# acoustid/acoustid-index

Measured on AMD Instinct MI355X. Metric: queries/sec + p50 /_search latency, 100M-fp index, 1k-hash queries, higher is better.
Workload: dtype u32

## Files before the change

acoustid-index_amd/csrc/fpx_api.hip:

```cpp
#include <cstdarg>
#include <cstdio>
#include <cstring>
#include <hip/hip_runtime.h>
#include <dlfcn.h>
#include <execinfo.h>
#include <atomic>

#include <algorithm>
#include <new>

#include "fpx_internal.h"

namespace fpx {

static thread_local char g_err[512] = "";

void set_error(const char* fmt, ...)
{
    va_list ap;
    va_start(ap, fmt);
    vsnprintf(g_err, sizeof g_err, fmt, ap);
    va_end(ap);
}

// ... 80 lines not shown
        static const size_t hi = [] { const char* v = getenv("FPX_POISON_MAX"); return v ? (size_t)strtoull(v, nullptr, 0) : ~(size_t)0; }();
        static const uint64_t olo = [] { const char* v = getenv("FPX_POISON_ORD_LO"); return v ? (uint64_t)strtoull(v, nullptr, 0) : (uint64_t)0; }();
        static const uint64_t ohi = [] { const char* v = getenv("FPX_POISON_ORD_HI"); return v ? (uint64_t)strtoull(v, nullptr, 0) : ~(uint64_t)0; }();
        static FILE* const log = [] { const char* v = getenv("FPX_ALLOC_LOG"); return v ? std::fopen(v, "w") : (FILE*)nullptr; }();
        static std::atomic<uint64_t> ordinal{0};
        const uint64_t ord = ordinal.fetch_add(1);
        if (log) {
            void* bt[6];
            const int nb = backtrace(bt, 6);
            Dl_info di{};
            std::fprintf(log, "%llu %zu", (unsigned long long)ord, bytes);
            for (int i = 1; i < nb; ++i)
                if (dladdr(bt[i], &di) && di.dli_fbase) std::fprintf(log, " %s+0x%zx", di.dli_fname ? std::strrchr(di.dli_fname, '/') ? std::strrchr(di.dli_fname, '/') + 1 : di.dli_fname : "?", (size_t)((char*)bt[i] - (char*)di.dli_fbase));
            std::fprintf(log, "\n");
            std::fflush(log);
        }
        if (bytes >= lo && bytes <= hi && ord >= olo && ord <= ohi) { (void)hipMemset(*p, 0xCD, bytes); (void)hipDeviceSynchronize(); }
    }
    return e;
}

thread_local DevArena* tl_arena = nullptr;
thread_local DevArena* tl_scratch = nullptr;
void* arena_take(size_t bytes) { return tl_arena ? tl_arena->take(bytes) : nullptr; }
void* scratch_take(size_t bytes) { return tl_scratch ? tl_scratch->take(bytes) : nullptr; }

hipError_t mem_info(size_t* free_b, size_t* total_b)
{
    const hipError_t e = hipMemGetInfo(free_b, total_b);
    int device = 0;
    if (e == hipSuccess && hipGetDevice(&device) == hipSuccess) *free_b += line_pool_bytes(device);
    return e;
}

Workspace* ws_acquire(Ctx* ctx)
{
    {
        std::lock_guard<std::mutex> g(ctx->mu);
        if (!ctx->free_ws.empty()) {
            Workspace* w = ctx->free_ws.back();
            ctx->free_ws.pop_back();
            return w;
        }
    }
    Workspace* w = new (std::nothrow) Workspace();
    if (!w) { set_error("out of host memory"); return nullptr; }
    bool ok = hipStreamCreateWithFlags(&w->stream, hipStreamNonBlocking) == hipSuccess &&
              hipEventCreate(&w->ev_begin) == hipSuccess && hipEventCreate(&w->ev_probe0) == hipSuccess &&
              hipEventCreate(&w->ev_probe1) == hipSuccess && hipEventCreate(&w->ev_probe2) == hipSuccess &&
              hipEventCreate(&w->ev_end) == hipSuccess &&
              dmalloc(&w->d_counters, COUNTERS_BYTES) == hipSuccess &&
              hipHostMalloc(reinterpret_cast<void**>(&w->h_counters), COUNTERS_BYTES, hipHostMallocMapped) == hipSuccess &&
              hipHostMalloc(reinterpret_cast<void**>(&w->h_cancel), 64, hipHostMallocMapped) == hipSuccess &&
              hipHostGetDevicePointer(reinterpret_cast<void**>(const_cast<uint32_t**>(&w->d_cancel)), w->h_cancel, 0) == hipSuccess;
    if (ok) *w->h_cancel = 0u;
    if (!ok) { set_error("workspace creation failed: %s", hipGetErrorString(hipGetLastError())); ws_destroy(w); return nullptr; }
    ctx->live_ws++;
    return w;
}

constexpr size_t MAX_POOLED = 8;

void ws_release(Ctx* ctx, Workspace* ws)
{
    {
        std::lock_guard<std::mutex> g(ctx->mu);
        if (ctx->free_ws.size() < MAX_POOLED) { ctx->free_ws.push_back(ws); return; }
    }
    ctx->live_ws--;
    ws_destroy(ws);
}

void ws_destroy(Workspace* w)
{
    if (!w) return;
    if (w->stream) (void)hipStreamSynchronize(w->stream);
    if (w->d_qstats) (void)hipFree(w->d_qstats);
    if (w->d_kocnt) (void)hipFree(w->d_kocnt);
    if (w->d_refs) (void)hipFree(w->d_refs);
    if (w->d_cells) (void)hipFree(w->d_cells);
    if (w->h_cells) (void)hipHostFree(w->h_cells);
    void* bufs[] = {w->d_hashes, w->d_offsets, w->d_opts, w->d_keys[0], w->d_keys[1], w->d_hits[0], w->d_hits[1],
                    w->d_cands[0], w->d_cands[1], w->d_temp, w->d_counters, w->d_out, w->d_out_n, w->d_def_list, w->d_def_count, w->d_qrange, w->d_qcand,
                    w->d_binq, w->d_qcursor, w->d_parts, w->d_parts_n};
    for (void* b : bufs) if (b) (void)hipFree(b);
    if (w->h_counters) (void)hipHostFree(w->h_counters);
    if (w->h_stage) (void)hipHostFree(w->h_stage);
    if (w->h_cancel) (void)hipHostFree(w->h_cancel);
    if (w->h_bins) (void)hipHostFree(w->h_bins);
    if (w->h_out) (void)hipHostFree(w->h_out);
    if (w->h_def_count) (void)hipHostFree(w->h_def_count);
    if (w->ev_begin) (void)hipEventDestroy(w->ev_begin);
    if (w->ev_probe0) (void)hipEventDestroy(w->ev_probe0);
    if (w->ev_probe1) (void)hipEventDestroy(w->ev_probe1);
    if (w->ev_probe2) (void)hipEventDestroy(w->ev_probe2);
    if (w->ev_end) (void)hipEventDestroy(w->ev_end);
    if (w->copy_stream) { (void)hipStreamSynchronize(w->copy_stream); (void)hipStreamDestroy(w->copy_stream); }
    for (hipEvent_t& e : w->ev_chunk) if (e) (void)hipEventDestroy(e);
    if (w->stream) (void)hipStreamDestroy(w->stream);
    delete w;
}

static void set_docs(Segment* s, const uint32_t* ids, const uint8_t* alive, uint32_t n)
{
    std::vector<uint64_t> v(n);
    for (uint32_t i = 0; i < n; ++i) v[i] = ((uint64_t)ids[i] << 32) | ((uint64_t)i << 1) | (alive ? (alive[i] ? 1u : 0u) : 1u);
    std::sort(v.begin(), v.end());
    s->doc_ids.clear(); s->doc_alive.clear();
    for (uint32_t i = 0; i < n; ++i) {
        const uint32_t id = (uint32_t)(v[i] >> 32);
        if (i + 1 < n && (uint32_t)(v[i + 1] >> 32) == id) continue;
        s->doc_ids.push_back(id);
        s->doc_alive.push_back((uint8_t)(v[i] & 1u));
    }
}

bool VmBuf::supported(int device)
{
    static std::atomic<int> known[64];
    std::atomic<int>& k = known[(unsigned)device & 63u];
    int v = k.load(std::memory_order_relaxed);
    if (v == 0) {
        const char* e = getenv("FPX_VM");
        int attr = 0;
        v = (e && e[0] == '0') ? 1 : (hipDeviceGetAttribute(&attr, hipDeviceAttributeVirtualMemoryManagementSupported, device) == hipSuccess && attr) ? 2 : 1;
        (void)hipGetLastError();
        k.store(v, std::memory_order_relaxed);
    }
    return v == 2;
}
int VmBuf::reserve(int dev, size_t bytes, size_t piece_bytes)
{
    device = dev; piece = piece_bytes;
    const size_t n = (bytes + piece - 1) / piece;
    void* p = nullptr;
    if (hipMemAddressReserve(&p, n * piece, 0, nullptr, 0) != hipSuccess) { (void)hipGetLastError(); return FPX_E_NOMEM; }
    va = static_cast<uint8_t*>(p); reserved = n * piece;
    handles.assign(n, hipMemGenericAllocationHandle_t{}); mapped.assign(n, 0);
    return FPX_OK;
}
int VmBuf::map_range(size_t lo, size_t hi)
{
    hipMemAllocationProp prop = {};
    prop.type = hipMemAllocationTypePinned; prop.location.type = hipMemLocationTypeDevice; prop.location.id = device;
    hipMemAccessDesc acc = {};
    acc.location = prop.location; acc.flags = hipMemAccessFlagsProtReadWrite;
    for (size_t i = lo / piece; i < handles.size() && i * piece < hi; ++i) {
        if (mapped[i]) continue;
        hipError_t e = hipMemCreate(&handles[i], piece, &prop, 0);
        if (e == hipErrorOutOfMemory) { (void)hipGetLastError(); if (line_pool_flush(device) != 0) e = hipMemCreate(&handles[i], piece, &prop, 0); }
        if (e != hipSuccess) { (void)hipGetLastError(); return FPX_E_NOMEM; }
        if (hipMemMap(va + i * piece, piece, 0, handles[i], 0) != hipSuccess || hipMemSetAccess(va + i * piece, piece, &acc, 1) != hipSuccess) {
            (void)hipGetLastError(); (void)hipMemRelease(handles[i]); return FPX_E_DEVICE;
        }
        mapped[i] = 1;
    }
    return FPX_OK;
}
void VmBuf::release_below(size_t upto)
{
    for (size_t i = 0; i < handles.size() && (i + 1) * piece <= upto; ++i) {
        if (!mapped[i]) continue;
        (void)hipMemUnmap(va + i * piece, piece);
        (void)hipMemRelease(handles[i]);
        mapped[i] = 0;
    }
}
// ... 55 lines not shown
                              unsigned long long* total)
{
    const uint32_t b = blockIdx.x * blockDim.x + threadIdx.x;
    unsigned long long n = 0;
    if (b < num_blocks) {
        const uint8_t* p = blocks + (size_t)b * block_size;
        n = (unsigned long long)p[4] | ((unsigned long long)p[5] << 8);
    }
    for (int d = 32; d > 0; d >>= 1) n += __shfl_down(n, d);
    if ((threadIdx.x & 63) == 0 && n) atomicAdd(total, n);
}

__global__ void k_build_cont(const uint8_t* __restrict__ blocks, uint32_t block_size, uint32_t num_blocks,
                             const uint32_t* __restrict__ block_index, uint32_t* __restrict__ cont)
{
    const uint32_t b = blockIdx.x * blockDim.x + threadIdx.x;
    bool bit = false;
    if (b + 1u < num_blocks)
        bit = *reinterpret_cast<const uint32_t*>(blocks + (size_t)(b + 1u) * block_size) == block_index[b];
    const unsigned long long m = __ballot((int)bit);
    if ((threadIdx.x & 63u) == 0u && b < num_blocks + 64u) {
        cont[(b >> 5)] = (uint32_t)m;
        cont[(b >> 5) + 1u] = (uint32_t)(m >> 32);
    }
}

int finish_file_segment(Segment* s)
{
    if (s->num_blocks == 0) { s->num_buckets = 1; s->bucket_shift = 32; }
    int rc = build_bucket_table(s, 0);
    if (rc) return rc;
    {
        const size_t words = ((size_t)s->num_blocks + 63) / 64 * 2 + 2;
        FPX_HIP(dmalloc(&s->d_cont, words * sizeof(uint32_t)));
        FPX_HIP(hipMemset(s->d_cont, 0, words * sizeof(uint32_t)));
        s->device_bytes += words * sizeof(uint32_t);
        if (s->num_blocks)
            hipLaunchKernelGGL(k_build_cont, dim3((s->num_blocks + 255) / 256), dim3(256), 0, 0,
                               s->d_blocks, s->block_size, s->num_blocks, s->d_block_index, s->d_cont);
    }
    unsigned long long* d_total = nullptr;
    FPX_HIP(dmalloc(&d_total, 8));
    FPX_HIP(hipMemset(d_total, 0, 8));
    if (s->num_blocks)
        hipLaunchKernelGGL(k_count_items, dim3((s->num_blocks + 255) / 256), dim3(256), 0, 0,
                           s->d_blocks, s->block_size, s->num_blocks, d_total);
    unsigned long long total = 0;
    FPX_HIP(hipMemcpy(&total, d_total, 8, hipMemcpyDeviceToHost));
    (void)hipFree(d_total);
    s->num_items = total;
    bool cand = false;
    if ((rc = direct_candidate(s, &cand))) return rc;
    s->candidate = cand;
    if (cand) return FPX_OK;
    if ((rc = build_presence(s))) return rc;
    return decode_small_segment(s);
}

struct OptInfo { const char* name; const char* env; int64_t dflt; int64_t min_set; bool env_once; };
static const OptInfo OPT_TABLE[OPT_COUNT] = {
                 {"direct", "FPX_DIRECT", 1, 0, false},
       {"direct_min_items", "FPX_DIRECT_MIN_ITEMS", 1ll << 20, 0, false},
               {"fuse_min", "FPX_FUSE_MIN", 2, 0, true},
           {"group_packed", "FPX_GROUP_PACKED", -1, -1, false},
     {"presence_min_items", "FPX_PRESENCE_MIN_ITEMS", 1ll << 20, 0, false},
              {"lean_head", "FPX_LEAN_HEAD", 0, 0, true},
                   {"fast", "FPX_FAST", 1, 0, true},
                 {"binned", "FPX_BINNED", 1, 0, true},
                  {"rec32", "FPX_REC32", 1, 0, true},
         {"local_sort_max", "FPX_LOCAL_SORT_MAX", 1ll << 20, 0, true},
        {"order_min_pairs", "FPX_ORDER_MIN_PAIRS", 1ll << 17, 0, true},
               {"lean_min", "FPX_LEAN_MIN", 1ll << 16, 0, true},
        {"sharded_workers", "FPX_SHARDED_WORKERS", 3, 1, true},
               {"hot_refs", "FPX_HOT_REFS", -1, -1, true},
               {"query_wg", "FPX_QUERY_WG", 1, 0, false},
                {"side_wg", "FPX_SIDE_WG", 0, 0, false},
                 {"hot_wg", "FPX_HOT_WG", 0, 0, false},
               {"words_wg", "FPX_WORDS_WG", 0, 0, false},
                 {"low_wg", "FPX_LOW_WG", 0, 0, false},
              {"groups_wg", "FPX_GROUPS_WG", 0, 0, false},
               {"shard_wg", "FPX_SHARD_WG", 0, 0, false},
             {"shard_pack", "FPX_SHARD_PACK", 0, 0, false},
              {"filt_coop", "FPX_FILT_COOP", 0, 0, false},
};

int64_t ctx_opt(const Ctx* c, CtxOpt o)
{
    const OptInfo& t = OPT_TABLE[o];
    if (c) {
        const int64_t v = c->opts[o].load(std::memory_order_relaxed);
        if (v != OPT_UNSET) return v;
    }
    if (t.env_once) {
        static std::atomic<int64_t> cache[OPT_COUNT];
        static std::atomic<uint32_t> have{0};
        if (!(have.load(std::memory_order_acquire) & (1u << o))) {
            const char* e = getenv(t.env);
            cache[o].store(e ? (int64_t)strtoll(e, nullptr, 0) : t.dflt, std::memory_order_relaxed);
            have.fetch_or(1u << o, std::memory_order_release);
        }
        return cache[o].load(std::memory_order_relaxed);
    }
    const char* e = getenv(t.env);
    return e ? (int64_t)strtoll(e, nullptr, 0) : t.dflt;
}

uint32_t ctx_fuse_min(const Ctx* c) { return (uint32_t)std::max<int64_t>(0, ctx_opt(c, OPT_FUSE_MIN)); }

static int settle_in_blocks(Segment* s)
{
    if (s->d_proberec || s->d_small_items || s->settled) return FPX_OK;
    s->settled = true;
    int rc = build_presence(s);
    if (rc) return rc;
    return decode_small_segment(s);
}

int resolve_candidates(Ctx* c, const std::vector<Segment*>& segs)
{
    const uint32_t fuse_min = ctx_fuse_min(c);
    std::vector<Segment*> lone;
    for (const Segment* s : segs)
        if (s->blocks_lost) { set_error("a segment lost its blocks in a group build that failed: it must be created again"); return FPX_E_INVAL; }
    for (Segment* s : segs)
        if (s->kind == 0 && s->ctx == c && !s->home && ((s->candidate && s->d_blocks && !s->settled) || s->direct)) lone.push_back(s);
    std::vector<bool> done(lone.size(), false);
    for (size_t i = 0; fuse_min != 0 && i < lone.size(); ++i) {
        if (done[i]) continue;
        std::vector<Segment*> batch;
        std::vector<size_t> idx;
        for (size_t j = i; j < lone.size() && batch.size() < FUSE_MAX; ++j) {
            if (done[j]) continue;
            const Segment* a = lone[i]; const Segment* b = lone[j];
            if (a->own_flags != b->own_flags || ((a->own_flags & 1u) && a->own_lo != b->own_lo) || ((a->own_flags & 2u) && a->own_hi != b->own_hi)) continue;
            if (a->block_size != b->block_size) continue;
            batch.push_back(lone[j]); idx.push_back(j);
        }
        for (size_t j : idx) done[j] = true;
        if (batch.size() < fuse_min) continue;
        std::shared_ptr<Group> g;
        const int grc = group_segments(c, batch.data(), (uint32_t)batch.size(), &g);
        if (grc == FPX_E_DEVICE || grc == FPX_E_INVAL) return grc;
        if (grc != FPX_OK)
            for (const Segment* b : batch) if (b->blocks_lost) { set_error("a group build failed after its members' blocks had begun to go back: the segments must be created again"); return FPX_E_DEVICE; }
    }
    for (Segment* s : lone) {
        if (s->home || s->direct) continue;
        int rc = build_direct(s);
        if (rc) return rc;
        if (!s->direct && (rc = settle_in_blocks(s))) return rc;
    }
    return FPX_OK;
}

int regroup_segments(Ctx* c, const std::vector<Segment*>& segs, uint32_t* regrouped)
{
    *regrouped = 0;
    if (ctx_fuse_min(c) == 0) return FPX_OK;
    std::vector<Segment*> m;
    for (Segment* s : segs) {
        if (!s || s->kind != 0 || s->ctx != c || s->own_flags) continue;
        if (std::find(m.begin(), m.end(), s) != m.end()) continue;
        if (!m.empty() && s->block_size != m[0]->block_size) continue;
        if (s->home || s->direct || (s->candidate && s->d_blocks && !s->settled)) m.push_back(s);
        if (m.size() == FUSE_MAX) break;
    }
// ... 56 lines not shown
}

using namespace fpx;

extern "C" {

int fpx_version(void) { return 2; }

int fpx_host_alloc(size_t bytes, void** out)
{
    if (!out) { set_error("null out"); return FPX_E_INVAL; }
    *out = nullptr;
    const hipError_t e = hipHostMalloc(out, bytes ? bytes : 1, hipHostMallocDefault);
    if (e != hipSuccess) { *out = nullptr; return hip_fail(e, "hipHostMalloc"); }
    return FPX_OK;
}

void fpx_host_free(void* p) { if (p) (void)hipHostFree(p); }

const char* fpx_last_error(void) { return g_err; }

const char* fpx_strerror(int status)
{
    switch (status) {
        case FPX_OK: return "ok";
        case FPX_E_NOMEM: return "out of memory";
        case FPX_E_TIMEOUT: return "search timeout";
        case FPX_E_DEVICE: return "device error";
        case FPX_E_INVAL: return "invalid argument";
        case FPX_E_NODEVICE: return "no HIP device";
        case FPX_E_AGAIN: return "buffer too small, retry";
        default: return "unknown";
    }
}

int fpx_ctx_create(int device, fpx_ctx** out)
{
    if (!out) { set_error("null out"); return FPX_E_INVAL; }
    *out = nullptr;
    int n = 0;
    hipError_t e = hipGetDeviceCount(&n);
    if (e != hipSuccess || n <= 0) {
        set_error("no HIP device visible (%s): libfpx has no CPU fallback", e == hipSuccess ? "count=0" : hipGetErrorString(e));
        return FPX_E_NODEVICE;
    }
    if (device < 0) { if (hipGetDevice(&device) != hipSuccess) device = 0; }
    if (device >= n) { set_error("device %d out of range (%d visible)", device, n); return FPX_E_INVAL; }
    FPX_HIP(hipSetDevice(device));
    hipDeviceProp_t prop;
    FPX_HIP(hipGetDeviceProperties(&prop, device));
    if (std::strncmp(prop.gcnArchName, "gfx950", 6) != 0) {
        set_error("device %d is %s; libfpx is built for gfx950 only", device, prop.gcnArchName);
        return FPX_E_NODEVICE;
    }
    Ctx* c = new (std::nothrow) Ctx();
    if (!c) return FPX_E_NOMEM;
    c->device = device;
    *out = reinterpret_cast<fpx_ctx*>(c);
    return FPX_OK;
}

int fpx_ctx_device(const fpx_ctx* ctx) { return ctx ? reinterpret_cast<const Ctx*>(ctx)->device : -1; }

static int opt_by_name(const char* name)
{
    if (!name) return -1;
    for (int o = 0; o < OPT_COUNT; ++o) if (!std::strcmp(name, OPT_TABLE[o].name)) return o;
    return -1;
}

int fpx_ctx_set_option(fpx_ctx* ctx, const char* name, int64_t value)
{
    Ctx* c = reinterpret_cast<Ctx*>(ctx);
    const int o = opt_by_name(name);
    if (!c || o < 0) {
        std::string all;
        for (int i = 0; i < OPT_COUNT; ++i) { if (i) all += ", "; all += OPT_TABLE[i].name; }
        set_error("fpx_ctx_set_option: unknown option (%s)", all.c_str());
        return FPX_E_INVAL;
    }
    if (o == OPT_SHARD_WG && value > 2) { set_error("fpx_ctx_set_option: shard_wg is 0, 1 or 2"); return FPX_E_INVAL; }
    if (o == OPT_SHARD_PACK && value > 1) { set_error("fpx_ctx_set_option: shard_pack is 0 or 1"); return FPX_E_INVAL; }
    if (o == OPT_FILT_COOP && value > 1) { set_error("fpx_ctx_set_option: filt_coop is 0 or 1"); return FPX_E_INVAL; }
    c->opts[o].store(value < OPT_TABLE[o].min_set ? OPT_UNSET : value, std::memory_order_relaxed);
    return FPX_OK;
}

int fpx_ctx_get_option(const fpx_ctx* ctx, const char* name, int64_t* value)
{
    const Ctx* c = reinterpret_cast<const Ctx*>(ctx);
    const int o = opt_by_name(name);
    if (!c || o < 0 || !value) { set_error("fpx_ctx_get_option: unknown option"); return FPX_E_INVAL; }
    *value = ctx_opt(c, (CtxOpt)o);
    return FPX_OK;
}

uint64_t fpx_ctx_trim(fpx_ctx* ctx)
{
    Ctx* c = reinterpret_cast<Ctx*>(ctx);
    if (!c) return 0;
    (void)hipSetDevice(c->device);
    return line_pool_flush(c->device);
}

int fpx_ctx_scan_histograms(const fpx_ctx* ctx, fpx_scan_histograms* out, uint64_t* unbucketed)
{
    const Ctx* c = reinterpret_cast<const Ctx*>(ctx);
    if (!c || !out) { set_error("null argument"); return FPX_E_INVAL; }
    uint64_t h[HIST_SLOTS + 1];
    for (uint32_t i = 0; i <= HIST_SLOTS; ++i) h[i] = c->scan_hist[i].load(std::memory_order_relaxed);
    std::memset(out, 0, sizeof *out);
    uint64_t docs_rest = 0, blocks_rest = 0;
    for (uint32_t i = 0; i < 9; ++i) { out->docs_bucket[i + 1] = h[i]; docs_rest += h[i]; }
    for (uint32_t i = 0; i < 3; ++i) { out->blocks_bucket[i + 1] = h[9 + i]; blocks_rest += h[9 + i]; }
    out->count = h[HIST_COUNT]; out->docs_sum = h[HIST_DOCS]; out->blocks_sum = h[HIST_BLOCKS];
    out->docs_bucket[0] = out->count - std::min(out->count, docs_rest);
    out->blocks_bucket[0] = out->count - std::min(out->count, blocks_rest);
    if (unbucketed) *unbucketed = h[HIST_SLOTS];
    return FPX_OK;
}

void fpx_ctx_destroy(fpx_ctx* ctx_)
{
    Ctx* c = reinterpret_cast<Ctx*>(ctx_);
    if (!c) return;
    (void)hipSetDevice(c->device);
    for (Workspace* w : c->free_ws) ws_destroy(w);
    delete c;
}

static int create_file_impl(fpx_ctx* ctx_, const uint8_t* blocks, size_t blocks_len, uint32_t block_size,
                            const uint32_t* block_index, uint32_t num_blocks,
                            uint32_t own_flags, uint32_t own_lo, uint32_t own_hi,
                            uint32_t min_doc_id, uint32_t max_doc_id, uint64_t commit_id,
                            const uint32_t* doc_ids, const uint8_t* doc_alive, uint32_t num_docs,
                            fpx_segment** out)
{
    Ctx* c = reinterpret_cast<Ctx*>(ctx_);
    if (!c || !out || (!blocks && blocks_len) || (!block_index && num_blocks) || (!doc_ids && num_docs)) {
        set_error("null argument"); return FPX_E_INVAL;
    }
    *out = nullptr;
    if (block_size < 64 || block_size > 4096) { set_error("block_size %u outside [64,4096] (src/filefmt.zig:236)", block_size); return FPX_E_INVAL; }
    if (blocks_len < (size_t)num_blocks * block_size) { set_error("blocks_len shorter than num_blocks * block_size"); return FPX_E_INVAL; }
    FPX_HIP(hipSetDevice(c->device));
    Segment* s = new (std::nothrow) Segment();
    if (!s) return FPX_E_NOMEM;
    s->ctx = c; s->kind = 0; s->commit_id = commit_id; s->min_doc_id = min_doc_id; s->max_doc_id = max_doc_id;
    s->block_size = block_size; s->num_blocks = num_blocks;
    s->own_flags = own_flags; s->own_lo = own_lo; s->own_hi = own_hi;
    set_docs(s, doc_ids, doc_alive, num_docs);
    s->blocks_len = ((size_t)num_blocks + 1) * block_size;
    const size_t alloc = s->blocks_len + 16;
    hipError_t e = blocks_alloc(s, alloc);
    if (e == hipSuccess) e = dmalloc(&s->d_block_index, ((size_t)num_blocks + 1) * sizeof(uint32_t));
    if (e != hipSuccess) { segment_free(s); return hip_fail(e, "hipMalloc(segment)"); }
    s->device_bytes = alloc + ((size_t)num_blocks + 1) * sizeof(uint32_t);
    const size_t copy = (size_t)num_blocks * block_size;
    if ((e = hipMemset(s->d_blocks + copy, 0, alloc - copy)) != hipSuccess ||
        (copy && (e = hipMemcpy(s->d_blocks, blocks, copy, hipMemcpyHostToDevice)) != hipSuccess) ||
        (num_blocks && (e = hipMemcpy(s->d_block_index, block_index, (size_t)num_blocks * sizeof(uint32_t), hipMemcpyHostToDevice)) != hipSuccess)) {
        segment_free(s); return hip_fail(e, "segment upload");
    }
    int rc = finish_file_segment(s);
    if (rc) { segment_free(s); return rc; }
    FPX_HIP(hipDeviceSynchronize());
// ... 822 lines not shown
```

acoustid-index_amd/csrc/fpx_internal.h:

```cpp
#pragma once
#include <hip/hip_runtime.h>
#include <stddef.h>
#include <stdint.h>

#include <atomic>
#include <memory>
#include <mutex>
#include <string>
#include <vector>

#include "../../include/fpx.h"

namespace fpx {

struct SegDesc {
    const uint8_t*  blocks;
    const uint32_t* block_index;
    const uint32_t* bucket;
    const uint32_t* dead;
    const uint32_t* cont;
    const uint32_t* dead_bits;
    const uint32_t* proberec;
    const uint2*    blockrec;
    const uint64_t* items;
// ... 177 lines not shown
    uint32_t* d_small_aux = nullptr; uint32_t small_shift = 0, small_cshift = 0;
    const char* why = "";
    bool candidate = false;
    bool settled = false;
    bool direct = false;
    std::shared_ptr<DirectStore> dstore;
    uint32_t* d_drec = nullptr; uint32_t* d_primary = nullptr; uint32_t* d_extras = nullptr;
    std::shared_ptr<Group> home; uint32_t col = 0;
    uint64_t num_distinct = 0, num_positions = 0, extras_words = 0;
    uint32_t first_hash = 0, last_hash = 0, extras_shift = 0;
    uint32_t own_flags = 0, own_lo = 0, own_hi = 0;
    std::mutex dead_mu; std::shared_ptr<DeadSet> last_dead;
    uint64_t num_items = 0;
    uint64_t* d_items = nullptr;
    uint64_t device_bytes = 0;
};

struct Snapshot {
    std::atomic<int> refs{1};
    Ctx* ctx = nullptr;
    std::vector<Segment*> segs;
    std::vector<SegDesc> h_file;
    std::vector<MemDesc> h_mem;
    SegDesc* d_file = nullptr; uint32_t n_file = 0;
    SegDesc* d_lean = nullptr; uint32_t n_lean = 0;
    uint32_t n_lean2 = 0;
    SegDesc* d_gen = nullptr; uint32_t n_gen = 0; bool gen_all_512 = true;
    SegDesc* d_small = nullptr; uint32_t n_small = 0;
    std::vector<SegDesc> h_direct;
    SegDesc* d_direct = nullptr; uint32_t n_direct = 0;
    std::vector<std::shared_ptr<Group>> groups;
    std::vector<GroupDesc> h_group; uint32_t n_group = 0;
    uint32_t max_doc_declared = 0;
    uint32_t rec32_refused = 0;
    uint32_t qs_skip = 0;
    std::vector<std::shared_ptr<DirectStore>> solo_stores;
    SegDesc* d_solo = nullptr; uint32_t n_solo = 0;
    Snapshot* part[2] = {nullptr, nullptr};
    uint32_t max_small_blocks = 0;
    MemDesc* d_mem = nullptr; uint32_t n_mem = 0;
    uint64_t* d_memtab = nullptr; uint32_t* d_membucket = nullptr; uint64_t n_memtab = 0;
    uint32_t* d_membits = nullptr;
    uint64_t mem_items = 0;
    std::vector<std::shared_ptr<DeadSet>> dead_sets;
    std::vector<std::shared_ptr<DeadSet>> direct_dead;
    std::vector<uint32_t> direct_max_doc;
    std::shared_ptr<DeadUnion> dead_union;
    uint32_t max_block_size = 0;
    bool all_512 = true;
};

constexpr size_t COUNTERS_BYTES = (CTR_COUNT + 1) * sizeof(unsigned long long) + 1024 * sizeof(fpx_result);

constexpr size_t STAGE_BYTES = 64 * 1024;

struct Workspace {
    hipStream_t stream = nullptr;
    hipEvent_t ev_begin = nullptr, ev_probe0 = nullptr, ev_probe1 = nullptr, ev_probe2 = nullptr, ev_end = nullptr;
    uint32_t* d_hashes = nullptr; size_t cap_hashes = 0;
    uint64_t* d_offsets = nullptr; size_t cap_queries = 0;
    uint32_t* d_opts = nullptr;
    uint64_t* d_keys[2] = {nullptr, nullptr}; size_t cap_keys = 0;
    uint64_t* d_hits[2] = {nullptr, nullptr}; size_t cap_hits = 0;
    uint64_t* d_cands[2] = {nullptr, nullptr}; size_t cap_cands = 0;
    void* d_temp = nullptr; size_t cap_temp = 0;
    uint64_t* d_qrange = nullptr; size_t cap_qrange = 0;
    uint64_t* d_qcand = nullptr; size_t cap_qcand = 0;
    unsigned long long* d_counters = nullptr;
    uint32_t* d_def_list = nullptr; size_t cap_def = 0;
    unsigned int* d_def_count = nullptr; unsigned int* h_def_count = nullptr; size_t cap_def_segs = 0;
    fpx_result* d_out = nullptr; uint32_t* d_out_n = nullptr; size_t cap_out = 0;
    uint32_t* d_binq = nullptr; unsigned long long* d_qcursor = nullptr; size_t cap_binq = 0; uint32_t* h_bins = nullptr;
    uint8_t* h_out = nullptr; size_t cap_h_out = 0;
    uint4* d_refs = nullptr; size_t cap_refs = 0;
    uint32_t* d_kocnt = nullptr; size_t cap_kocnt = 0;
    unsigned long long* d_qstats = nullptr; size_t cap_qstats = 0;
    uint32_t* d_cells = nullptr; uint32_t* h_cells = nullptr; size_t cap_cells = 0;
    static constexpr uint32_t UP_CHUNKS = 4;
    hipStream_t copy_stream = nullptr; hipEvent_t ev_chunk[UP_CHUNKS] = {nullptr, nullptr, nullptr, nullptr};
    std::vector<uint32_t> h_opts;
    uint32_t hint_def = 0;
    uint64_t hint_misc = 0;
    uint64_t hint_P = 0, hint_H = 0;
    uint32_t fast_penalty = 0;
    fpx_result* d_parts = nullptr; size_t cap_parts = 0;
    uint32_t* d_parts_n = nullptr; size_t cap_parts_n = 0;
    uint64_t batch_hist[HIST_SLOTS + 1] = {};
    unsigned long long* h_counters = nullptr;
    uint8_t* h_stage = nullptr; uint8_t* d_stage = nullptr;
    unsigned long long* d_ret = nullptr;
    uint32_t* h_cancel = nullptr; const uint32_t* d_cancel = nullptr;
};

struct QueryBatch {
    Ctx* ctx = nullptr;
    uint32_t B = 0;
    uint32_t* d_hashes = nullptr;
    uint64_t* d_offsets = nullptr;
    uint32_t* d_opts = nullptr;
    std::vector<uint64_t> offsets;
    std::vector<fpx_opts> opts;
};

enum CtxOpt : int {
    OPT_DIRECT, OPT_DIRECT_MIN_ITEMS, OPT_FUSE_MIN, OPT_GROUP_PACKED,
    OPT_PRESENCE_MIN_ITEMS, OPT_LEAN_HEAD,
    OPT_FAST, OPT_BINNED, OPT_REC32,
    OPT_LOCAL_SORT_MAX, OPT_ORDER_MIN_PAIRS, OPT_LEAN_MIN,
    OPT_SHARDED_WORKERS,
    OPT_HOT_REFS,
    OPT_QUERY_WG,
    OPT_SIDE_WG,
    OPT_HOT_WG,
    OPT_WORDS_WG,
    OPT_LOW_WG,
    OPT_GROUPS_WG,
    OPT_SHARD_WG,
    OPT_SHARD_PACK,
    OPT_FILT_COOP,
    OPT_COUNT
};
constexpr int64_t OPT_UNSET = -2;

struct Ctx {
    int device = 0;
    std::atomic<int64_t> opts[OPT_COUNT];
    Ctx() { for (auto& o : opts) o.store(OPT_UNSET, std::memory_order_relaxed); for (auto& h : scan_hist) h.store(0, std::memory_order_relaxed); }
    std::mutex mu;
    std::mutex group_mu;
    std::vector<Workspace*> free_ws;
    std::atomic<int> live_ws{0};
    std::atomic<int> qs_running{0};
    std::atomic<uint64_t> scan_hist[HIST_SLOTS + 1];
};
void ctx_hist_add(Ctx* c, const uint64_t* slots, uint64_t unbucketed);

int64_t ctx_opt(const Ctx* c, CtxOpt o);
bool ctx_direct_enabled(const Ctx* c);
uint64_t ctx_direct_min_items(const Ctx* c);
uint32_t ctx_fuse_min(const Ctx* c);
int ctx_group_packed(const Ctx* c);
void set_error(const char* fmt, ...);
int  hip_fail(hipError_t e, const char* what);
void*  line_pool_take(int device, size_t bytes, size_t max_bytes, size_t* got);
void   line_pool_put(int device, void* p, size_t bytes);
size_t line_pool_flush(int device);
size_t line_pool_bytes(int device);
hipError_t dmalloc_raw(void** p, size_t bytes);
template <class T> inline hipError_t dmalloc(T** p, size_t bytes) { return dmalloc_raw(reinterpret_cast<void**>(p), bytes); }
hipError_t mem_info(size_t* free_b, size_t* total_b);
struct DevArena {
    uint8_t* base = nullptr;
    size_t cap = 0, used = 0, missed = 0;
    const char* name = "arena";
    std::vector<std::pair<size_t, size_t>> guards;
    static size_t guard_bytes();
    void check_guards();
    ~DevArena() { check_guards(); if (base) (void)hipFree(base); }
    void* take(size_t bytes)
    {
        const size_t g = guard_bytes();
        const size_t body = (bytes + 255u) & ~(size_t)255u, need = body + g;
        if (used + need > cap) { missed += need; return nullptr; }
        void* p = base + used;
        if (g) { (void)hipMemset(base + used + body, 0xA5, g); guards.emplace_back(used + body, bytes); }
        used += need;
        return p;
    }
    void rewind()
    {
        check_guards();
        if (missed) {
            const size_t want = (used + missed) * 5 / 4 + ((size_t)1 << 20);
            if (base) (void)hipFree(base);
            base = nullptr; cap = 0;
            if (dmalloc(&base, want) == hipSuccess) cap = want; else { (void)hipGetLastError(); base = nullptr; }
        }
        used = 0; missed = 0;
    }
};
extern thread_local DevArena* tl_arena;
extern thread_local DevArena* tl_scratch;
void* arena_take(size_t bytes);
void* scratch_take(size_t bytes);
#define FPX_HIP(expr)                                              \
    do {                                                           \
        hipError_t _e = (expr);                                    \
        if (_e != hipSuccess) return ::fpx::hip_fail(_e, #expr);   \
    } while (0)

Workspace* ws_acquire(Ctx* ctx);
void ws_release(Ctx* ctx, Workspace* ws);
void ws_destroy(Workspace* ws);

size_t sort_u64_temp_bytes(size_t n, unsigned begin_bit, unsigned end_bit);
hipError_t sort_u64(void* temp, size_t temp_bytes, uint64_t* buf0, uint64_t* buf1, size_t n,
                    unsigned begin_bit, unsigned end_bit, hipStream_t stream, int* result_in);

size_t select_u64_temp_bytes(size_t n);
hipError_t select_u64(void* temp, size_t temp_bytes, const uint64_t* in, const uint8_t* flags, uint64_t* out,
                      unsigned long long* d_count, size_t n, hipStream_t stream);

// ... 65 lines not shown
```

acoustid-index_amd/csrc/fpx_qsearch.hpp:

```cpp
#pragma once
#include <hip/hip_runtime.h>

#include <cstddef>

#include "fpx_internal.h"

namespace fpx {

#ifndef FPX_QS_WG
#define FPX_QS_WG 256
#endif
#ifndef FPX_QS_WAVES
#define FPX_QS_WAVES 4
#endif
#ifndef FPX_QS_REC_CAP
#define FPX_QS_REC_CAP 8192
#endif
#ifndef FPX_QS_FLOG2
#define FPX_QS_FLOG2 11
#endif
constexpr uint32_t QS_WG = FPX_QS_WG;
constexpr uint32_t QS_REC_CAP = FPX_QS_REC_CAP;
constexpr uint32_t QS_FLOG2 = FPX_QS_FLOG2;
constexpr uint32_t QS_TLOG2 = 8;
constexpr uint32_t QS_MAX_HASHES = QS_REC_CAP >= 8192u ? 4096u : 2048u;
constexpr uint32_t QS_MAX_ROUNDS = 32;
#ifndef FPX_QS_WORDS
#define FPX_QS_WORDS 12
#endif
#ifndef FPX_QS_CH
#define FPX_QS_CH 2
#endif
constexpr uint32_t QS_WORDS = FPX_QS_WORDS;
constexpr uint32_t QS_CH = FPX_QS_CH;
constexpr uint32_t QS_TASKS = (((size_t)2u << QS_FLOG2) + ((size_t)8u << QS_TLOG2)) / 8u;
constexpr uint32_t QS_TASK_WORDS = 8;
constexpr uint32_t QS_TASKS_FILT = QS_TASKS * 8u / 12u;
static_assert(QS_MAX_HASHES * 2u <= QS_REC_CAP, "the dedup set lives where the records will");
static_assert((QS_MAX_HASHES + QS_WG - 1u) / QS_WG <= QS_MAX_ROUNDS, "rounds per query");
static_assert(QS_WORDS % 4 == 0 && QS_WORDS <= 16, "the words are fetched in 16-byte pieces; a lane's masks of them are 16 bits");
#ifndef FPX_QS_DYN
#define FPX_QS_DYN 1
#endif
#ifndef FPX_QS_STAGGER
#define FPX_QS_STAGGER 1
#endif
constexpr uint32_t QS_STAGGER = FPX_QS_STAGGER;
#ifndef FPX_QS_WGS_PER_CU
#define FPX_QS_WGS_PER_CU 4
#endif
constexpr uint32_t QS_WGS_PER_CU = FPX_QS_WGS_PER_CU;
constexpr size_t QS_LDS_BYTES = ((size_t)QS_REC_CAP + 4u) * 4u + ((size_t)2u << QS_FLOG2) + ((size_t)8u << QS_TLOG2) + (size_t)SB_CAND * 8u;

struct QSearchArgs {
    const uint32_t* hashes_base; const uint64_t* offsets;
    const uint32_t* opts;
    uint32_t q_begin, q_end, sb;
    union { uint64_t* cands; uint64_t* bins; };
    union { uint64_t cand_cap; uint64_t bin_cap; };
    uint64_t* qcand;
    union { uint32_t* qcand_n; uint32_t* bin_fill; };
    unsigned long long* counters;
    unsigned long long* stat_sets;
    unsigned long long* qstats;
    const uint32_t* cancel;
    const uint64_t* mem_tab; const uint32_t* mem_bucket; const uint32_t* mem_bits;
    unsigned int* next_q;
    uint32_t stagger;
    union { unsigned long long* redo; const uint32_t* dead_union; };
    union { uint32_t redo_cap; uint32_t bin_rec32; uint32_t dead_union_last; };
};

struct QSKernargs { QSearchArgs a; GroupArgs ga; };
static_assert(sizeof(QSearchArgs) == 160 && offsetof(QSearchArgs, cands) == 40 && offsetof(QSearchArgs, qcand_n) == 64 && offsetof(QSearchArgs, next_q) == 128 &&
              offsetof(QSearchArgs, redo) == 144 && offsetof(QSearchArgs, redo_cap) == 152, "QSearchArgs' layout is the kernels' argument segment: a member is renamed or shared, never moved");
typedef const __attribute__((address_space(4))) QSKernargs* qs_kargs_t;
__device__ __forceinline__ qs_kargs_t qs_cold_args()
{
    qs_kargs_t p = (qs_kargs_t)__builtin_amdgcn_kernarg_segment_ptr();
    asm volatile("" : "+s"(p));
    return p;
}

#define FPX_QS_OCC __attribute__((amdgpu_waves_per_eu(FPX_QS_WAVES)))
#define FPX_LDS __attribute__((address_space(3)))
typedef uint32_t u32x3_t __attribute__((ext_vector_type(3)));
__device__ __forceinline__ uint3 gload_u3(const uint32_t* p)
{
    const u32x3_t v = *(const FPX_GLOBAL u32x3_t*)p;
    return make_uint3(v.x, v.y, v.z);
}
__device__ __forceinline__ uint32_t qs_cell(uint32_t doc) { return (doc ^ (doc >> QS_FLOG2)) & ((1u << QS_FLOG2) - 1u); }
__device__ __forceinline__ unsigned long long qs_task_list(const uint32_t* p, uint32_t chunk)
{
    return ((unsigned long long)p >> 2) | ((unsigned long long)chunk << 57) | (1ull << 63);
}
__device__ __forceinline__ unsigned long long qs_task_words(const uint32_t* p, uint32_t cnt, uint32_t second, uint32_t chunk)
{
    return ((unsigned long long)p >> 2) | ((unsigned long long)(cnt - 1u) << 46) | ((unsigned long long)(second & 0xFFu) << 49) | ((unsigned long long)chunk << 57);
}
__device__ __forceinline__ const uint32_t* qs_task_ptr(unsigned long long e) { return reinterpret_cast<const uint32_t*>((e & ((1ull << 46) - 1ull)) << 2); }
__device__ __forceinline__ uint32_t qs_word_cols(uint32_t pm, uint32_t dm, uint32_t j0, uint32_t cnt)
{
    uint32_t cols = 0, rest = pm, i = 0, w = 0;
    while (rest != 0u && w < j0 + cnt) {
        const uint32_t s = (uint32_t)__builtin_ctz(rest), span = 1u + ((dm >> i) & 1u);
        for (uint32_t t = 0; t < span; ++t, ++w) if (w >= j0 && w < j0 + cnt) cols |= s << (4u * (w - j0));
        ++i; rest &= rest - 1u;
    }
    return cols;
}

template <uint32_t K> __device__ __forceinline__ uint32_t qs_group_bcast(uint32_t v)
{
    return (uint32_t)__builtin_amdgcn_ds_swizzle((int)v, (int)((K << 5) | 0x18u));
}
template <uint32_t K> __device__ __forceinline__ uint32_t qs_from_sub0(uint32_t v)
{
    if constexpr (K == 0u) return v;
    else return (uint32_t)__builtin_amdgcn_update_dpp(0, (int)v, 0x110 | (int)K, 0xF, 0xF, true);
}
template <uint32_t K> __device__ __forceinline__ uint32_t qs_from_sub7(uint32_t v)
{
    if constexpr (K == 7u) return v;
    else return (uint32_t)__builtin_amdgcn_update_dpp(0, (int)v, 0x100 | (int)(7u - K), 0xF, 0xF, true);
}
template <uint32_t K> struct qs_idx { static constexpr uint32_t value = K; };
template <uint32_t K = 0, class F> __device__ __forceinline__ void qs_for8(F&& f)
{
    if constexpr (K < 8u) { f(qs_idx<K>{}); qs_for8<K + 1u>(f); }
}

#ifdef FPX_QS_PROF
#define QS_MARK(i) do { if (tid == 0) { const unsigned long long t_ = clock64(); atomicAdd(&qs_cold_args()->a.counters[CTR_HIST + (i)], t_ - t_prev); t_prev = t_; } } while (0)
#define QS_SUB0() do { if (tid == 0) t_sub = clock64(); } while (0)
#define QS_SUB(i) do { if (tid == 0) { const unsigned long long t_ = clock64(); atomicAdd(&qs_cold_args()->a.counters[CTR_HIST + (i)], t_ - t_sub); t_sub = t_; } } while (0)
#define QS_ARRIVED2(x, y) asm volatile("" :: "v"(x), "v"(y))
#define QS_ARRIVED4(x) asm volatile("" :: "v"((x)[0]), "v"((x)[1]), "v"((x)[2]), "v"((x)[3]))
#else
#define QS_MARK(i) do { } while (0)
#define QS_SUB0() do { } while (0)
#define QS_SUB(i) do { } while (0)
#define QS_ARRIVED2(x, y) do { } while (0)
#define QS_ARRIVED4(x) do { } while (0)
#endif
constexpr uint32_t QS_MAX_CLASSES = 32;
constexpr uint32_t QS_LIST_AHEAD = 8;
__device__ __forceinline__ uint32_t qs_class(uint32_t rec) { return mix32(rec) >> 27; }
static_assert(QS_MAX_CLASSES == 32u, "qs_class gives five bits");
constexpr uint32_t QS_LOW_CHUNK = 8;
constexpr uint32_t QS_SHARE_BQ = 3;
constexpr uint32_t QS_SHARE_STRIDE = 32;
constexpr uint32_t QS_PACK_MAX = 4u * QS_WG;

enum : uint32_t { QS_F_CLS = 1u, QS_F_LOW = 2u, QS_F_NEXT = 4u, QS_F_SHARE = 8u, QS_F_PACK = 16u, QS_F_COOP = 32u };
template <int NS_, bool QS_, bool MEM_, bool FILT_, uint32_t FORM = 0u>
struct qs_variant {
    static constexpr int NS = NS_;
    static constexpr bool QS = QS_, MEM = MEM_, FILT = FILT_;
    static constexpr bool CLS = (FORM & QS_F_CLS) != 0u, LOW = (FORM & QS_F_LOW) != 0u, NEXT = (FORM & QS_F_NEXT) != 0u;
    static constexpr bool SHARE = (FORM & QS_F_SHARE) != 0u, PACK = (FORM & QS_F_PACK) != 0u, COOP = (FORM & QS_F_COOP) != 0u;
    static_assert(NS == 8 || NS == 16, "columns of a line");
    static_assert(!COOP || (FILT && !CLS && !LOW && !NEXT && !SHARE), "the filtered walk eight lanes to a line: k_search_filt only");
    static_assert(!SHARE || (!QS && !CLS && !LOW && !NEXT), "a window's walk for the bin protocol: no per-query statistics, no doc classes, no sorted tail, one group");
    static_assert(!PACK || SHARE, "packed probes: a window's walk only (without a window nearly every hash is a probe)");
    static_assert(!PACK || 2u * QS_PACK_MAX <= QS_REC_CAP, "the packed list and its memory-table bits live at the record array's bottom");
    static_assert(!NEXT || (!CLS && !MEM), "a later group's walk: no doc classes, no memory table (they ride on the first group's launch)");
    static_assert(!(CLS && FILT), "doc classes: the unfiltered walk only");
    static_assert(!LOW || (!CLS && QS_WG == 256u && QS_REC_CAP >= 512u && (QS_REC_CAP & (QS_REC_CAP - 1u)) == 0u),
                  "low floors: no doc classes; the sorted tail's scans are written for 256 lanes and a power-of-two array");
};

template <class V>
__device__ __forceinline__ void qs_body(const QSearchArgs& a, const GroupArgs& ga)
{
    constexpr int NS = V::NS;
    constexpr bool QS = V::QS, MEM = V::MEM, FILT = V::FILT, CLS = V::CLS, LOW = V::LOW, NEXT = V::NEXT, SHARE = V::SHARE, PACK = V::PACK, COOP = V::COOP;
#ifdef FPX_QS_PROF
    unsigned long long t_prev = clock64(), t_sub = 0;
#endif
    constexpr uint32_t HVL = NS == 16 ? 2u : 3u;
    constexpr uint32_t T = 1u << QS_TLOG2, TMASK = T - 1u;
    extern __shared__ __align__(16) uint8_t qs_dyn[];
    uint32_t* const recs = reinterpret_cast<uint32_t*>(qs_dyn);
    uint32_t* const filter = recs + QS_REC_CAP + 4u;
    unsigned long long* const table = reinterpret_cast<unsigned long long*>(filter + (1u << (QS_FLOG2 - 1u)));
    unsigned long long* const tasks = reinterpret_cast<unsigned long long*>(filter);
    constexpr uint32_t TCAP = FILT ? QS_TASKS_FILT : QS_TASKS;
    uint32_t* const tcols = reinterpret_cast<uint32_t*>(tasks + QS_TASKS_FILT);
    uint64_t* const cbuf = reinterpret_cast<uint64_t*>(table + T);
    __shared__ uint32_t s_count, s_ntask, s_over_recs, s_seen_ones, s_cancel, s_claimed, s_full, s_ccnt, s_cshared, s_cbase_lo, s_cbase_hi;
    __shared__ unsigned long long wg_blocks, wg_docs, wg_probes, wg_reads;
    __shared__ uint32_t wg_h[HIST_SLOTS];
    __shared__ uint32_t s_first[FUSE_MAX], s_last[FUSE_MAX];
    __shared__ const uint32_t* s_ext[GROUP_CHUNKS];
    __shared__ uint32_t s_q2;
    __shared__ uint32_t s_dseg[FUSE_MAX];

    const uint32_t tid = threadIdx.x, lane = tid & 63u;
    const GroupDesc* g = &ga.g;
    uint32_t ent = a.q_begin + blockIdx.x;
    uint32_t q = ent, q_recs = 0u;
    uint32_t ncls = 1u;
    auto take_entry = [&]() {
        const unsigned long long e = qs_cold_args()->a.redo[ent];
        q = (uint32_t)__builtin_amdgcn_readfirstlane((int)(uint32_t)e); q_recs = (uint32_t)__builtin_amdgcn_readfirstlane((int)(uint32_t)(e >> 32));
        ncls = 1u;
        while ((unsigned long long)ncls * (QS_REC_CAP / 2u) < (unsigned long long)q_recs) ncls *= 2u;
    };
    if constexpr (CLS) take_entry();
    (void)q_recs;
    uint32_t qn = q + gridDim.x;
    uint32_t n, nn = 0u;
    uint64_t nq_lo = 0;
    const uint32_t* qh;
    if constexpr (CLS) {
        const uint64_t q_lo = a.offsets[q];
        n = (uint32_t)(a.offsets[q + 1] - q_lo);
        qh = a.hashes_base + q_lo;
        qn = 0xFFFFFFFFu;
    } else {
        const uint64_t q_lo = a.offsets[q];
        n = (uint32_t)(a.offsets[q + 1] - q_lo);
        qh = a.hashes_base + q_lo;
        if (qn < a.q_end) { nq_lo = a.offsets[qn]; nn = (uint32_t)(a.offsets[qn + 1] - nq_lo); }
    }
    {
        const qs_kargs_t ka = qs_cold_args();
        if (tid < FUSE_MAX) { s_first[tid] = ka->ga.g.first_hash[tid]; s_last[tid] = ka->ga.g.last_hash[tid]; }
        if (tid < GROUP_CHUNKS) s_ext[tid] = tid < ka->ga.g.nchunks ? ka->ga.g.ext_tab[tid] : nullptr;
        if (FILT && tid < FUSE_MAX) s_dseg[tid] = ka->ga.g.has_dead[tid] != 0u ? ka->ga.g.seg_index[tid] : 0xFFFFFFFFu;
    }
    const uint32_t gmin = (FILT || MEM) ? g->gmin : 0u;
    (void)gmin;
    uint32_t hq[2u * QS_CH];
    uint3 hd[QS_CH];
    auto line_of = [&](uint32_t h) -> const uint32_t* { return g->lines + (size_t)((h >> HVL) - g->line0) * GROUP_LINE_WORDS; };
    auto load_pair = [&](const uint32_t* qh_, uint32_t n_, uint32_t c, uint32_t& h0, uint32_t& h1) {
        uint32_t t = tid;
        if constexpr (COOP) asm volatile("" : "+v"(t));
        const uint32_t i = c * QS_CH * QS_WG + t;
        h0 = i < n_ ? gload_u32(qh_ + i) : 0u;
        h1 = i + QS_WG < n_ ? gload_u32(qh_ + i + QS_WG) : 0u;
    };
    auto issue_heads = [&](bool v0, bool v1) {
        hd[0] = gload_u3(v0 ? line_of(hq[0]) : g->lines);
        hd[1] = gload_u3(v1 ? line_of(hq[1]) : g->lines);
    };
    load_pair(qh, n, 0u, hq[0], hq[1]);
    load_pair(qh, n, 1u, hq[2], hq[3]);
    uint32_t c_host = 0u;
    unsigned long long c_dev = 0ull;
    auto ask_cancel = [&]() {
        const qs_kargs_t ka = qs_cold_args();
        const uint32_t* const cancel = ka->a.cancel;
        if (tid == 0u && cancel != nullptr) {
            if ((blockIdx.x & 63u) == 0u) c_host = __hip_atomic_load(cancel, __ATOMIC_RELAXED, __HIP_MEMORY_SCOPE_SYSTEM);
            c_dev = __hip_atomic_load(&ka->a.counters[CTR_CANCEL], __ATOMIC_RELAXED, __HIP_MEMORY_SCOPE_AGENT);
        }
    };
    ask_cancel();
  if (const uint32_t stagger = qs_cold_args()->a.stagger; !CLS && stagger != 0u && a.q_end - a.q_begin >= 4u * gridDim.x)
      for (uint32_t i = 0; i < ((blockIdx.x >> 8) & 3u) * stagger; ++i) __builtin_amdgcn_s_sleep(127);
  for (;;) {
    if constexpr (CLS) {
        if (ncls > QS_MAX_CLASSES) {
            if (tid == 0) atomicMax(&qs_cold_args()->a.counters[CTR_BINFAIL], 1ull);
            return;
        }
    }
    if constexpr (PACK) {
        if (n > QS_PACK_MAX) {
            if (tid == 0) atomicMax(&qs_cold_args()->a.counters[CTR_BINFAIL], 1ull);
            return;
        }
    }
    const uint32_t rounds = (n + QS_WG - 1u) / QS_WG, nchunks = (rounds + QS_CH - 1u) / QS_CH;
    uint32_t sbits = 8u;
    while ((1u << sbits) < 2u * n) ++sbits;
    if (tid < HIST_SLOTS) wg_h[tid] = 0u;
    for (uint32_t i = tid; i < (1u << sbits); i += QS_WG) recs[i] = 0xFFFFFFFFu;
    if (tid == 0) {
        s_count = 0u; s_ntask = 0u; s_over_recs = 0u; s_seen_ones = 0u; s_ccnt = 0u; s_cshared = 0u;
        if constexpr (PACK) s_claimed = 0u;
        wg_blocks = 0; wg_docs = 0; wg_probes = 0; wg_reads = 0;
        if (c_host != 0u) { atomicExch(&qs_cold_args()->a.counters[CTR_CANCEL], 1ull); c_dev = 1ull; }
        s_cancel = c_dev != 0ull ? 1u : 0u;
    }
    __syncthreads();
    if (s_cancel) return;
    QS_MARK(0);
    uint32_t vmask = 0u;
    uint32_t mmask = 0u;
    uint32_t nx[QS_CH] = {0u, 0u};
    for (uint32_t c = 0; c < nchunks; ++c) {
        uint32_t hc[QS_CH];
        uint32_t mb[QS_CH];
#pragma unroll
        for (uint32_t u = 0; u < QS_CH; ++u) hc[u] = c == 0u ? hq[u] : c == 1u ? hq[QS_CH + u] : nx[u];
        if (c != 0u) { QS_SUB0(); QS_ARRIVED2(hc[0], hc[1]); QS_SUB(6); }
        if (c != 0u && c + 1u < nchunks) load_pair(qh, n, c + 1u, nx[0], nx[1]);
        if constexpr (MEM) {
#pragma unroll
            for (uint32_t u = 0; u < QS_CH; ++u) {
                const uint32_t i = (c * QS_CH + u) * QS_WG + tid;
                mb[u] = (i < n && a.mem_bits != nullptr) ? gload_u32(a.mem_bits + ((hc[u] >> MEMTAB_FILTER_SHIFT) >> 5)) : 0xFFFFFFFFu;
            }
        }
#pragma unroll
        for (uint32_t u = 0; u < QS_CH; ++u) {
            const uint32_t i = (c * QS_CH + u) * QS_WG + tid;
            if (i >= n) continue;
            const uint32_t h = hc[u];
            if constexpr (PACK) { if (h < g->win_lo || h > g->win_hi) continue; }
            bool dup;
            if (h == 0xFFFFFFFFu) dup = atomicExch(&s_seen_ones, 1u) != 0u;
            else {
                uint32_t slot = (h * 0x9E3779B1u) >> (32u - sbits);
                for (;;) {
                    const uint32_t old = atomicCAS(&recs[slot], 0xFFFFFFFFu, h);
                    if (old == 0xFFFFFFFFu) { dup = false; break; }
                    if (old == h) { dup = true; break; }
                    slot = (slot + 1u) & ((1u << sbits) - 1u);
                }
            }
            if (!dup && h >= g->win_lo && h <= g->win_hi) {
                vmask |= 1u << (c * QS_CH + u);
                if constexpr (MEM) mmask |= ((mb[u] >> ((h >> MEMTAB_FILTER_SHIFT) & 31u)) & 1u) << (c * QS_CH + u);
            }
        }
    }
    (void)mmask;
    __syncthreads();
    auto reserve_in = [&](uint32_t* counter, uint32_t cnt) -> uint32_t {
        const uint32_t incl = scan16(cnt);
        const uint32_t r0 = (uint32_t)__builtin_amdgcn_readlane((int)incl, 15), r1 = (uint32_t)__builtin_amdgcn_readlane((int)incl, 31),
                       r2 = (uint32_t)__builtin_amdgcn_readlane((int)incl, 47), r3 = (uint32_t)__builtin_amdgcn_readlane((int)incl, 63);
        const uint32_t total = r0 + r1 + r2 + r3;
        uint32_t wbase = 0;
        if (total != 0u) {
            if (lane == 0u) wbase = atomicAdd(counter, total);
            wbase = (uint32_t)__builtin_amdgcn_readfirstlane((int)wbase);
        }
        const uint32_t row = lane >> 4;
        return wbase + (row >= 1u ? r0 : 0u) + (row >= 2u ? r1 : 0u) + (row >= 3u ? r2 : 0u) + (incl - cnt);
    };
    uint32_t prounds = rounds, pnchunks = nchunks;
    if constexpr (PACK) {
        uint32_t at = reserve_in(&s_claimed, (uint32_t)__popc(vmask));
#pragma unroll
        for (uint32_t r = 0; r < 2u * QS_CH; ++r)
            if (((vmask >> r) & 1u) != 0u) {
                recs[at] = hq[r];
                if constexpr (MEM) recs[QS_PACK_MAX + at] = (mmask >> r) & 1u;
                ++at;
            }
        __syncthreads();
        const uint32_t m = (uint32_t)__builtin_amdgcn_readfirstlane((int)s_claimed);
        vmask = 0u; mmask = 0u;
#pragma unroll
        for (uint32_t r = 0; r < 2u * QS_CH; ++r) {
            const uint32_t i = r * QS_WG + tid;
            const bool has = i < m;
            hq[r] = has ? recs[i] : 0u;
            vmask |= (has ? 1u : 0u) << r;
            if constexpr (MEM) mmask |= (has ? recs[QS_PACK_MAX + i] : 0u) << r;
        }
        prounds = (m + QS_WG - 1u) / QS_WG; pnchunks = (prounds + QS_CH - 1u) / QS_CH;
        __syncthreads();
    }
    QS_MARK(1);

    const uint32_t cmask = ncls - 1u;
// ... 926 lines not shown
            const qs_kargs_t kc = qs_cold_args();
            if (s_full != 0u && tid == 0) atomicMax(&kc->a.counters[CTR_BINFAIL], 1ull);
            const uint32_t gmin_c = kc->ga.g.gmin;
            for (uint32_t s = tid; s < T; s += QS_WG) {
                const unsigned long long e = table[s];
                if (e == 0ull) continue;
                const uint32_t count = (uint32_t)e, doc = gmin_c + (uint32_t)(e >> 32);
                if (count < floor_q) continue;
                if ((uint64_t)count > smax) atomicMax(&kc->a.counters[CTR_MAXSCORE], (unsigned long long)count);
                const uint64_t sc = (uint64_t)count > smax ? smax : (uint64_t)count;
                const uint64_t qpart = sb >= 32u ? 0ull : ((uint64_t)q << (32u + sb));
                const uint64_t key = qpart | ((smax - sc) << 32) | doc;
                const uint32_t at = atomicAdd(&s_ccnt, 1u);
                if (at < SB_CAND) cbuf[at] = key;
                else {
                    const unsigned long long gi = atomicAdd(&kc->a.counters[CTR_CANDS], 1ull);
                    if (gi < kc->a.cand_cap) kc->a.cands[gi] = key;
                    s_cshared = 1u;
                }
            }
            if (pass + 1u < passes) {
                __syncthreads();
                for (uint32_t s = tid; s < T; s += QS_WG) table[s] = 0ull;
                if (tid == 0) { s_claimed = 0u; s_full = 0u; }
                __syncthreads();
            }
        }
    }
  }
    __syncthreads();
    QS_MARK(4);
    const uint32_t cn = min(s_ccnt, SB_CAND);
    (void)cn;
    if constexpr (SHARE) {
    } else if constexpr (NEXT) {
        const qs_kargs_t kh = qs_cold_args();
        if (tid == 0) {
            uint32_t prev = kh->a.qcand_n[q];
            const bool was = prev == QCAND_OVERFLOWED;
            prev = was ? 0u : min(prev, QCAND_SLOTS);
            const bool to_slots = !was && s_cshared == 0u && prev + cn <= QCAND_SLOTS;
            if (!to_slots) {
                if (prev + cn != 0u) {
                    const unsigned long long gi = atomicAdd(&kh->a.counters[CTR_CANDS], (unsigned long long)(prev + cn));
                    s_cbase_lo = (uint32_t)gi; s_cbase_hi = (uint32_t)(gi >> 32);
                }
                if (!was) kh->a.qcand_n[q] = QCAND_OVERFLOWED;
            } else kh->a.qcand_n[q] = prev + cn;
            s_claimed = prev; s_full = to_slots ? 1u : 0u;
        }
        __syncthreads();
        const uint32_t prev = s_claimed;
        const bool to_slots = s_full != 0u;
        const uint64_t base = ((uint64_t)s_cbase_hi << 32) | s_cbase_lo;
        if (tid < cn) {
            const uint64_t key = cbuf[tid];
            if (to_slots) kh->a.qcand[(size_t)q * QCAND_SLOTS + prev + tid] = key;
            else if (base + tid < kh->a.cand_cap) kh->a.cands[base + tid] = key;
        }
        static_assert(SB_CAND + QCAND_SLOTS <= QS_WG, "the carried slots move by lanes of their own");
        if (const uint32_t t = tid - SB_CAND; !to_slots && t < prev) {
            const uint64_t gi = base + cn + t;
            if (gi < kh->a.cand_cap) kh->a.cands[gi] = kh->a.qcand[(size_t)q * QCAND_SLOTS + t];
        }
    } else {
    const bool shared = s_cshared != 0u || cn > QCAND_SLOTS;
    const qs_kargs_t kh = qs_cold_args();
    if (tid == 0) {
        if (shared && cn != 0u) {
            const unsigned long long gi = atomicAdd(&kh->a.counters[CTR_CANDS], (unsigned long long)cn);
            s_cbase_lo = (uint32_t)gi; s_cbase_hi = (uint32_t)(gi >> 32);
        }
        kh->a.qcand_n[q] = shared ? QCAND_OVERFLOWED : cn;
    }
    __syncthreads();
    if (tid < cn) {
        const uint64_t key = cbuf[tid];
        if (!shared) kh->a.qcand[(size_t)q * QCAND_SLOTS + tid] = key;
        else {
            const uint64_t gi = (((uint64_t)s_cbase_hi << 32) | s_cbase_lo) + tid;
            if (gi < kh->a.cand_cap) kh->a.cands[gi] = key;
        }
    }
    }
    QS_MARK(5);
    if constexpr (CLS) {
        ent += gridDim.x;
        if (ent >= a.q_end) break;
        take_entry();
        const uint64_t q_lo = a.offsets[q];
        n = (uint32_t)(a.offsets[q + 1] - q_lo);
        qh = a.hashes_base + q_lo;
        load_pair(qh, n, 0u, hq[0], hq[1]);
        load_pair(qh, n, 1u, hq[2], hq[3]);
        ask_cancel();
    } else {
        if (!has_next) break;
        q = qn; n = nn; qh = a.hashes_base + nq_lo;
        qn = q2; nn = 0u; nq_lo = 0;
        if (has_q2) {
            nq_lo = ((uint64_t)(uint32_t)__builtin_amdgcn_readfirstlane((int)(uint32_t)(o2_lo >> 32)) << 32) | (uint32_t)__builtin_amdgcn_readfirstlane((int)(uint32_t)o2_lo);
            nn = (uint32_t)__builtin_amdgcn_readfirstlane((int)(o2_hi - (uint32_t)o2_lo));
        }
    }
    __syncthreads();
  }
}

template <int NS, bool QS, bool MEM, bool FILT>
__global__ __launch_bounds__(QS_WG) FPX_QS_OCC void k_search_query(QSearchArgs a, GroupArgs ga)
{
    qs_body<qs_variant<NS, QS, MEM, FILT>>(a, ga);
}
template <int NS, bool MEM>
__global__ __launch_bounds__(QS_WG) FPX_QS_OCC void k_search_classes(QSearchArgs a, GroupArgs ga)
{
    qs_body<qs_variant<NS, true, MEM, false, QS_F_CLS>>(a, ga);
}
template <int NS, bool QS, bool MEM>
__global__ __launch_bounds__(QS_WG) FPX_QS_OCC void k_search_low(QSearchArgs a, GroupArgs ga)
{
    qs_body<qs_variant<NS, QS, MEM, false, QS_F_LOW>>(a, ga);
}
template <int NS, bool QS, bool MEM>
__global__ __launch_bounds__(QS_WG) FPX_QS_OCC void k_search_low_filt(QSearchArgs a, GroupArgs ga)
{
    qs_body<qs_variant<NS, QS, MEM, true, QS_F_LOW>>(a, ga);
}
template <int NS, bool QS, bool MEM>
__global__ __launch_bounds__(QS_WG) FPX_QS_OCC void k_search_filt(QSearchArgs a, GroupArgs ga)
{
    qs_body<qs_variant<NS, QS, MEM, true, QS_F_COOP>>(a, ga);
}
template <int NS, bool QS, bool FILT>
__global__ __launch_bounds__(QS_WG) FPX_QS_OCC void k_search_next(QSearchArgs a, GroupArgs ga)
{
    qs_body<qs_variant<NS, QS, false, FILT, QS_F_NEXT>>(a, ga);
}
template <int NS, bool QS, bool FILT>
__global__ __launch_bounds__(QS_WG) FPX_QS_OCC void k_search_low_next(QSearchArgs a, GroupArgs ga)
{
    qs_body<qs_variant<NS, QS, false, FILT, QS_F_LOW | QS_F_NEXT>>(a, ga);
}
template <int NS, bool MEM, bool FILT>
__global__ __launch_bounds__(QS_WG) FPX_QS_OCC void k_search_window(QSearchArgs a, GroupArgs ga)
{
    qs_body<qs_variant<NS, false, MEM, FILT, QS_F_SHARE>>(a, ga);
}
template <int NS, bool MEM, bool FILT>
__global__ __launch_bounds__(QS_WG) FPX_QS_OCC void k_search_packed(QSearchArgs a, GroupArgs ga)
{
    qs_body<qs_variant<NS, false, MEM, FILT, QS_F_SHARE | QS_F_PACK>>(a, ga);
}

__global__ __launch_bounds__(256) void k_qs_zero(unsigned long long* counters, unsigned int* words, uint32_t nwords)
{
    const uint32_t i0 = blockIdx.x * 256u + threadIdx.x;
    if (i0 < CTR_COUNT) counters[i0] = 0ull;
    for (uint32_t i = i0; i < nwords; i += gridDim.x * 256u) words[i] = 0u;
}

}
```

acoustid-index_amd/csrc/fpx_search.hip:

```cpp
#include <cstdio>
#include <cstring>
#include <hip/hip_runtime.h>

#include <algorithm>
#include <chrono>
#include <cstdlib>
#include <thread>
#include <type_traits>
#include <vector>

#include "fpx_internal.h"


#include "fpx_kernels_common.hpp"
#include "fpx_keyorder.hpp"
#include "fpx_probe_generic.hpp"
#include "fpx_probe_lean.hpp"
#include "fpx_direct.hpp"
#include "fpx_group.hpp"
#include "fpx_pgroup.hpp"
#include "fpx_probe_small.hpp"
#include "fpx_score.hpp"
#include "fpx_score_bin.hpp"
#include "fpx_qsearch.hpp"
// ... 38 lines not shown
    uint64_t total = 0, mmax = 0;
    for (const MemDesc& m : sn->h_mem) { total += m.num_items; mmax = std::max<uint64_t>(mmax, m.num_items); }
    if (total == 0) return FPX_OK;
    if (total >= 0xFFFFFFF0ull) { set_error("a snapshot's memory segments hold %llu items: their table's offsets are 32 bits", (unsigned long long)total); return FPX_E_INVAL; }
    uint64_t* buf[2] = {nullptr, nullptr};
    unsigned long long* d_count = nullptr;
    void* d_temp = nullptr;
    uint32_t* d_bucket = nullptr;
    auto fail = [&](int rc) { for (auto* b : buf) if (b) (void)hipFree(b); if (d_count) (void)hipFree(d_count); if (d_temp) (void)hipFree(d_temp); if (d_bucket) (void)hipFree(d_bucket); (void)hipGetLastError(); return rc; };
    const size_t tb = sort_u64_temp_bytes(total, 0, 64);
    if (dmalloc(&buf[0], (total + 1) * 8) != hipSuccess || dmalloc(&buf[1], (total + 1) * 8) != hipSuccess || dmalloc(&d_count, 8) != hipSuccess ||
        dmalloc(&d_temp, tb + 256) != hipSuccess || dmalloc(&d_bucket, ((size_t)(1u << MEMTAB_BITS) + 2) * sizeof(uint32_t)) != hipSuccess)
        return fail(FPX_E_NOMEM);
    hipStream_t st = 0;
    if (hipMemsetAsync(d_count, 0, 8, st) != hipSuccess) return fail(FPX_E_DEVICE);
    const uint32_t gx = (uint32_t)std::min<uint64_t>(std::max<uint64_t>(1, (mmax + WG - 1) / WG), 1024);
    hipLaunchKernelGGL(k_memtab_gather, dim3(gx, sn->n_mem), dim3(WG), 0, st, (const MemDesc*)sn->d_mem, buf[0], d_count);
    unsigned long long n = 0;
    if (hipMemcpyAsync(&n, d_count, 8, hipMemcpyDeviceToHost, st) != hipSuccess || hipStreamSynchronize(st) != hipSuccess) return fail(FPX_E_DEVICE);
    int cur = 0;
    if (n > 1 && sort_u64(d_temp, tb + 256, buf[0], buf[1], n, 0, 64, st, &cur) != hipSuccess) return fail(FPX_E_DEVICE);
    hipLaunchKernelGGL(k_memtab_buckets, dim3(((1u << MEMTAB_BITS) + 256) / 256), dim3(256), 0, st, (const uint64_t*)buf[cur], (uint64_t)n, d_bucket);
    uint32_t* d_bits = nullptr;
    const size_t bits_bytes = ((size_t)1 << (32u - MEMTAB_FILTER_SHIFT)) / 8u;
    if (n != 0 && dmalloc(&d_bits, bits_bytes) == hipSuccess) {
        if (hipMemsetAsync(d_bits, 0, bits_bytes, st) != hipSuccess) { (void)hipFree(d_bits); d_bits = nullptr; }
        else hipLaunchKernelGGL(k_memtab_bits, dim3((uint32_t)std::min<uint64_t>((n + 255) / 256, 4096)), dim3(256), 0, st, (const uint64_t*)buf[cur], (uint64_t)n, d_bits);
    }
    (void)hipGetLastError();
    if (hipGetLastError() != hipSuccess || hipStreamSynchronize(st) != hipSuccess) { if (d_bits) (void)hipFree(d_bits); return fail(FPX_E_DEVICE); }
    sn->d_memtab = buf[cur]; sn->d_membucket = d_bucket; sn->n_memtab = n; sn->d_membits = d_bits;
    (void)hipFree(buf[1 - cur]); (void)hipFree(d_count); (void)hipFree(d_temp);
    return FPX_OK;
}

template <class T>
static int grow(T** p, size_t* cap, size_t need, size_t slack_num = 5, size_t slack_den = 4)
{
    if (need <= *cap) return FPX_OK;
    size_t ncap = need * slack_num / slack_den + 64;
    if (*p) (void)hipFree(*p);
    *p = nullptr; *cap = 0;
    hipError_t e = dmalloc(reinterpret_cast<void**>(p), ncap * sizeof(T));
    if (e != hipSuccess) { set_error("hipMalloc(%zu bytes) failed: %s", ncap * sizeof(T), hipGetErrorString(e)); return FPX_E_NOMEM; }
    *cap = ncap;
    return FPX_OK;
}

static int grow_pair(uint64_t* p[2], size_t* cap, size_t need)
{
    if (need <= *cap) return FPX_OK;
    size_t c0 = *cap, c1 = *cap;
    int rc = grow(&p[0], &c0, need);
    if (rc) return rc;
    rc = grow(&p[1], &c1, need);
    if (rc) return rc;
    *cap = std::min(c0, c1);
    return FPX_OK;
}

static int sort_keys(Workspace* ws, uint64_t* pair[2], uint64_t n, unsigned lo, unsigned hi, hipStream_t st, int* cur)
{
    const size_t tb = sort_u64_temp_bytes(n, lo, hi);
    if (const int rc = grow(reinterpret_cast<uint8_t**>(&ws->d_temp), &ws->cap_temp, tb + 256)) return rc;
    FPX_HIP(sort_u64(ws->d_temp, ws->cap_temp, pair[0], pair[1], n, lo, hi, st, cur));
    return FPX_OK;
}

template <class F> static void with_flags(F&& f) { f(); }
template <class F, class B, class... Bs> static void with_flags(F&& f, B flag, Bs... rest)
{
    static_assert(std::is_same<B, bool>::value, "a kernel's flag is a bool");
    if (flag) with_flags([&](auto... cs) { f(std::true_type{}, cs...); }, rest...);
    else with_flags([&](auto... cs) { f(std::false_type{}, cs...); }, rest...);
}
template <class F, class... Bs> static void with_ns(bool ns8, F&& f, Bs... flags)
{
    if (ns8) with_flags([&](auto... cs) { f(std::integral_constant<int, 8>{}, cs...); }, flags...);
    else with_flags([&](auto... cs) { f(std::integral_constant<int, 16>{}, cs...); }, flags...);
}
#define FPX_LAUNCH(K, grid, wg, lds, st, a0, a1, ns8, ...) \
    with_ns(ns8, [&](auto ns, auto... cs) { hipLaunchKernelGGL((K<decltype(ns)::value, decltype(cs)::value...>), grid, dim3(wg), lds, st, a0, a1); }, __VA_ARGS__)
#define FPX_LAUNCH_QS(K, grid, st, qa, g, ns8, ...) FPX_LAUNCH(K, grid, QS_WG, QS_LDS_BYTES, st, qa, g, ns8, __VA_ARGS__)

static void launch_probe_group(bool packed, bool ns8, bool binned, bool qs, dim3 grid, hipStream_t st, const ProbeArgs& a, const GroupArgs& g)
{
    const size_t stage = (size_t)FSTAGE_CAP * sizeof(uint64_t);
    if (packed) FPX_LAUNCH(k_probe_pgroup, grid, FK_WG, stage + PK_HEAD_LDS, st, a, g, ns8, binned, qs);
    else FPX_LAUNCH(k_probe_group, grid, FK_WG, stage + (binned ? (size_t)FSTAGE_CAP * sizeof(uint16_t) : 0u), st, a, g, ns8, binned, qs);
}

constexpr int FPX_SPLIT = 1;
constexpr int FPX_REDO_QS = 3;
constexpr int FPX_REDO = 2;
constexpr uint32_t QS_REDO_MIN = 4, QS_REDO_SHARE = 8;
constexpr uint32_t qs_redo_limit(uint32_t B) { return B / QS_REDO_SHARE > QS_REDO_MIN ? B / QS_REDO_SHARE : QS_REDO_MIN; }

static unsigned bits_for(uint64_t n)
{
    unsigned b = 0;
    while (b < 64 && (1ull << b) < n) ++b;
    return b;
}

static int ensure_queries(Workspace* ws, size_t B)
{
    if (B + 1 <= ws->cap_queries && ws->d_offsets && ws->d_opts && ws->d_out_n) return FPX_OK;
    const size_t cap = (B + 1) * 5 / 4 + 64;
    if (ws->d_offsets) (void)hipFree(ws->d_offsets);
    if (ws->d_opts) (void)hipFree(ws->d_opts);
    if (ws->d_out_n) (void)hipFree(ws->d_out_n);
    ws->d_offsets = nullptr; ws->d_opts = nullptr; ws->d_out_n = nullptr; ws->cap_queries = 0;
    if (dmalloc(&ws->d_offsets, cap * sizeof(uint64_t)) != hipSuccess ||
        dmalloc(&ws->d_opts, cap * 4 * sizeof(uint32_t)) != hipSuccess ||
        dmalloc(&ws->d_out_n, cap * sizeof(uint32_t)) != hipSuccess) {
        set_error("hipMalloc(query arrays) failed");
        return FPX_E_NOMEM;
    }
    ws->cap_queries = cap;
    return FPX_OK;
}

static uint32_t query_floor(const fpx_opts& o, uint64_t raw_len) { return o.has_min_score ? o.min_score : (uint32_t)((raw_len + 19) / 20); }
static uint32_t min_floor(const uint64_t* offsets, const fpx_opts* opts, uint32_t B)
{
    uint32_t lo = 0xFFFFFFFFu;
    for (uint32_t q = 0; q < B; ++q) lo = std::min(lo, query_floor(opts[q], offsets[q + 1] - offsets[q]));
    return lo;
}

static void fill_opts(std::vector<uint32_t>& h_opts, const fpx_opts* opts, const uint64_t* offsets, uint32_t B)
{
    h_opts.resize((size_t)B * 4);
    for (uint32_t q = 0; q < B; ++q) {
        const uint64_t raw_len = offsets[q + 1] - offsets[q];
        h_opts[q * 4 + 0] = opts[q].max_results;
        h_opts[q * 4 + 1] = query_floor(opts[q], raw_len);
        h_opts[q * 4 + 2] = opts[q].min_score_pct;
        h_opts[q * 4 + 3] = (uint32_t)raw_len;
    }
}

static double now_ms()
{
    using namespace std::chrono;
    return duration<double, std::milli>(steady_clock::now().time_since_epoch()).count();
}

static int sync_deadline(Workspace* ws, double t_start, uint32_t timeout_ms)
{
    hipStream_t st = ws->stream;
    if (timeout_ms == 0) { FPX_HIP(hipStreamSynchronize(st)); return FPX_OK; }
    bool fired = *reinterpret_cast<volatile uint32_t*>(ws->h_cancel) != 0u;
    for (uint32_t spins = 0;; ++spins) {
        const hipError_t e = hipStreamQuery(st);
        if (e == hipSuccess) break;
        if (e != hipErrorNotReady) return hip_fail(e, "hipStreamQuery");
        if (!fired && now_ms() - t_start > (double)timeout_ms) {
            __atomic_store_n(ws->h_cancel, 1u, __ATOMIC_RELEASE);
            fired = true;
        }
        if (spins < 512u) std::this_thread::yield();
        else std::this_thread::sleep_for(std::chrono::microseconds(fired ? 5 : 40));
    }
    if (fired) { set_error("search timeout"); return FPX_E_TIMEOUT; }
    return FPX_OK;
// ... 67 lines not shown
    if (const int rc = ensure_h_out(ws, bytes)) return rc;
    FPX_HIP(hipMemcpyAsync(ws->h_out, ws->d_out_n, (size_t)B * sizeof(uint32_t), hipMemcpyDeviceToHost, st));
    if (out_cap) FPX_HIP(hipMemcpyAsync(ws->h_out + (size_t)B * sizeof(uint32_t), ws->d_out, (size_t)B * out_cap * sizeof(fpx_result), hipMemcpyDeviceToHost, st));
    return FPX_OK;
}
static int staged_targets(Workspace* ws, uint32_t B, uint32_t out_cap, bool* staged, uint32_t** d_n, fpx_result** d_res)
{
    const size_t bytes = (size_t)B * sizeof(uint32_t) + (size_t)B * out_cap * sizeof(fpx_result);
    *staged = bytes <= STAGED_OUT_MAX;
    if (!*staged) return FPX_OK;
    if (const int rc = ensure_h_out(ws, bytes)) return rc;
    uint8_t* d = mapped_address(ws->h_out);
    if (!d) { *staged = false; return FPX_OK; }
    *d_n = reinterpret_cast<uint32_t*>(d);
    *d_res = reinterpret_cast<fpx_result*>(d + (size_t)B * sizeof(uint32_t));
    return FPX_OK;
}
static int deliver_results(Workspace* ws, uint32_t B, uint32_t out_cap, bool staged, fpx_result* out, uint32_t* out_n, hipStream_t st)
{
    if (staged) {
        std::memcpy(out_n, ws->h_out, (size_t)B * sizeof(uint32_t));
        if (out_cap) std::memcpy(out, ws->h_out + (size_t)B * sizeof(uint32_t), (size_t)B * out_cap * sizeof(fpx_result));
        return FPX_OK;
    }
    FPX_HIP(hipMemcpyAsync(out_n, ws->d_out_n, (size_t)B * sizeof(uint32_t), hipMemcpyDeviceToHost, st));
    if (out_cap) FPX_HIP(hipMemcpyAsync(out, ws->d_out, (size_t)B * out_cap * sizeof(fpx_result), hipMemcpyDeviceToHost, st));
    FPX_HIP(hipStreamSynchronize(st));
    return FPX_OK;
}

static uint64_t lean_min_probes(const Ctx* c) { return (uint64_t)std::max<int64_t>(0, ctx_opt(c, OPT_LEAN_MIN)); }

struct Exchange {
    int mode = 0;
    uint32_t world = 1;
    uint64_t* d_records = nullptr; uint64_t cap = 0;
    uint64_t n = 0;
    uint64_t* counts = nullptr;
};

__global__ void k_dest_bounds(const uint64_t* __restrict__ recs, uint64_t n, uint32_t mask, uint32_t world, uint64_t* __restrict__ bounds)
{
    const uint32_t d = blockIdx.x * blockDim.x + threadIdx.x;
    if (d > world) return;
    uint64_t lo = 0, hi = n;
    while (lo < hi) {
        const uint64_t m = (lo + hi) >> 1;
        if (((uint32_t)recs[m] & mask) < d) lo = m + 1; else hi = m;
    }
    bounds[d] = lo;
}

static void gather_hist(uint64_t* dst, const unsigned long long* h_counters, const unsigned long long* sets, uint64_t probes)
{
    for (uint32_t i = 0; i < HIST_SLOTS; ++i) dst[i] = h_counters[CTR_HIST + i];
    dst[HIST_COUNT] += h_counters[CTR_PROBES]; dst[HIST_DOCS] += h_counters[CTR_DOCS]; dst[HIST_BLOCKS] += h_counters[CTR_BLOCKS];
    if (sets) {
        const unsigned long long* hs = sets + (size_t)LEAN_STAT_SETS * 8;
        for (uint32_t k = 0; k < LEAN_STAT_SETS; ++k)
            for (uint32_t i = 0; i < HIST_SLOTS; ++i) dst[i] += hs[(size_t)k * HIST_SLOTS + i];
    }
    dst[HIST_SLOTS] = probes > dst[HIST_COUNT] ? probes - dst[HIST_COUNT] : 0ull;
}
void ctx_hist_add(Ctx* c, const uint64_t* slots, uint64_t unbucketed)
{
    for (uint32_t i = 0; i < HIST_SLOTS; ++i) if (slots[i]) c->scan_hist[i].fetch_add(slots[i], std::memory_order_relaxed);
    if (unbucketed) c->scan_hist[HIST_SLOTS].fetch_add(unbucketed, std::memory_order_relaxed);
}

enum class Try { First, NoQueryWg, GeneralOnly };

struct Batch {
    Snapshot* snap; Workspace* ws; hipStream_t st;
    const QueryBatch* resident; uint32_t q0;
    uint32_t B; uint64_t P, base; unsigned qb;
    const uint32_t* hashes; const uint64_t* offsets; const fpx_opts* opts;
    const uint32_t* d_hashes_base; const uint64_t* d_offsets; const uint32_t* d_opts;
    bool staged_single;
    const uint32_t* cancel; double t_start; uint32_t timeout_ms;
    bool partial; fpx_result* out; uint32_t out_cap; uint32_t* out_n; fpx_stats* stats;
    bool want_q; uint64_t* q_blocks; uint64_t* q_docs;
    size_t def_cap, def_stat_off, def_words;
    uint32_t up_chunks, up_q[Workspace::UP_CHUNKS + 1];
};

struct StatSums { unsigned long long reads = 0, blocks = 0, docs = 0, probes = 0, dreads = 0, bytes_off = 0, pads = 0, records = 0; };
static StatSums sum_stat_sets(const unsigned long long* ls)
{
    StatSums s;
    for (uint32_t i = 0; i < LEAN_STAT_SETS; ++i) {
        s.reads += ls[i * 8 + 0]; s.blocks += ls[i * 8 + 1]; s.docs += ls[i * 8 + 2]; s.probes += ls[i * 8 + 3]; s.dreads += ls[i * 8 + 4];
        s.bytes_off += ls[i * 8 + 5];
        s.pads += ls[i * 8 + 6]; s.records += ls[i * 8 + 7];
    }
    return s;
}
static const unsigned long long* host_stat_sets(const Batch& b) { return reinterpret_cast<const unsigned long long*>(b.ws->h_def_count + b.def_stat_off); }
static unsigned long long* device_stat_sets(const Batch& b) { return reinterpret_cast<unsigned long long*>(b.ws->d_def_count + b.def_stat_off); }
static unsigned long long unspread_fetched_bytes(const Workspace* ws, const Snapshot* snap)
{
    return snap->n_direct ? ws->h_counters[CTR_LEAN_READS] * 64ull + (snap->n_file ? ws->h_counters[CTR_BYTES] : 0ull) : ws->h_counters[CTR_BYTES];
}
static int device_cus(const Ctx* ctx)
{
    static std::atomic<int> cus_of[64];
    int cus = cus_of[(unsigned)ctx->device & 63u].load(std::memory_order_relaxed);
    if (cus == 0) {
        if (hipDeviceGetAttribute(&cus, hipDeviceAttributeMultiprocessorCount, ctx->device) != hipSuccess || cus <= 0) { (void)hipGetLastError(); cus = 256; }
        cus_of[(unsigned)ctx->device & 63u].store(cus, std::memory_order_relaxed);
    }
    return cus;
}
struct CandSlots { uint64_t* qcand = nullptr; uint32_t* qcand_n = nullptr; uint32_t* heavy = nullptr; uint64_t* extra = nullptr; };
static int ensure_cand_slots(Workspace* ws, uint32_t B, size_t extra_words, CandSlots* cs)
{
    const size_t words = (size_t)B * QCAND_SLOTS + 2 * ((size_t)B / 2 + 1);
    if (const int rc = grow(&ws->d_qcand, &ws->cap_qcand, words + extra_words)) return rc;
    cs->qcand = ws->d_qcand;
    cs->qcand_n = reinterpret_cast<uint32_t*>(ws->d_qcand + (size_t)B * QCAND_SLOTS);
    cs->heavy = reinterpret_cast<uint32_t*>(ws->d_qcand + (size_t)B * QCAND_SLOTS + (size_t)B / 2 + 1);
    cs->extra = ws->d_qcand + words;
    const size_t cand_guess0 = std::max<size_t>(1u << 16, (size_t)B * 64);
    return ws->cap_cands < cand_guess0 ? grow_pair(ws->d_cands, &ws->cap_cands, cand_guess0) : FPX_OK;
}
struct ResultsTo { fpx_result* res; uint32_t* n; bool staged; };
static int results_target(Batch& b, ResultsTo* to)
{
    to->res = b.partial ? b.out : b.ws->d_out;
    to->n = b.partial ? b.out_n : b.ws->d_out_n;
    to->staged = false;
    return b.partial ? FPX_OK : staged_targets(b.ws, b.B, b.out_cap, &to->staged, &to->n, &to->res);
}
static void launch_finish(Batch& b, const uint64_t* cands, uint64_t C, uint32_t sb, const CandSlots& cs, fpx_result* d_res, uint32_t* d_res_n, bool count_slots)
{
    hipLaunchKernelGGL(k_finish, dim3((b.B + 127) / 128), dim3(128), 0, b.st,
                       cands, C, b.d_opts, b.B, sb, b.partial ? 1 : 0, d_res, b.out_cap, d_res_n,
                       (const uint64_t*)cs.qcand, (const uint32_t*)cs.qcand_n, count_slots ? b.ws->d_counters : nullptr);
}
static int finish_crowded(Batch& b, uint32_t sb, const CandSlots& cs, const ResultsTo& to, uint64_t Cf)
{
    Workspace* ws = b.ws; int rc, ccur = 0;
    if (Cf != 0 && (rc = sort_keys(ws, ws->d_cands, Cf, 0, 64, b.st, &ccur))) return rc;
    if (b.stats) FPX_HIP(hipMemsetAsync(&ws->d_counters[CTR_SLOTCANDS], 0, sizeof(unsigned long long), b.st));
    launch_finish(b, ws->d_cands[ccur], Cf, sb, cs, to.res, to.n, b.stats != nullptr);
    FPX_HIP(hipGetLastError());
    FPX_HIP(hipMemcpyAsync(&ws->h_counters[CTR_SLOTCANDS], &ws->d_counters[CTR_SLOTCANDS], sizeof(unsigned long long), hipMemcpyDeviceToHost, b.st));
    FPX_HIP(hipEventRecord(ws->ev_end, b.st));
    FPX_SYNC_BATCH(b);
    return FPX_OK;
}
constexpr size_t BINQ_HEAD = 64 / sizeof(uint32_t);
static int publish(Batch& b, bool stat_sets, const uint32_t* b_src = nullptr, uint32_t b_n = 0, uint32_t b_stride = 0)
{
    Workspace* ws = b.ws;
    PublishArgs pa{};
    pa.counters = ws->d_counters; pa.h_counters = mapped_address(ws->h_counters);
    pa.a_src = ws->d_def_count; pa.a_dst = stat_sets ? mapped_address(ws->h_def_count) : nullptr; pa.a_n = stat_sets ? (uint32_t)b.def_words : 0u;
    uint32_t* d_hbins = b_src ? mapped_address(ws->h_bins) : nullptr;
    if (b_src) { pa.b_src = b_src; pa.b_dst = d_hbins + BINQ_HEAD; pa.b_n = b_n; pa.b_stride = b_stride; }
    if (!pa.h_counters || (stat_sets && !pa.a_dst) || (b_src && !d_hbins)) { set_error("page-locked host memory is not mapped into the device"); return FPX_E_DEVICE; }
    hipLaunchKernelGGL(k_publish, dim3(4), dim3(256), 0, b.st, pa);
    FPX_HIP(hipGetLastError());
    return FPX_OK;
}
static bool handed_back(const Workspace* ws, Snapshot* snap)
{
// ... 23 lines not shown
        hipFuncSetAttribute(reinterpret_cast<const void*>(&k_score<32, false>), hipFuncAttributeMaxDynamicSharedMemorySize, 128 * 1024),
        hipFuncSetAttribute(reinterpret_cast<const void*>(&k_score<8, false>), hipFuncAttributeMaxDynamicSharedMemorySize, 128 * 1024),
        hipFuncSetAttribute(reinterpret_cast<const void*>(&k_score<32, true>), hipFuncAttributeMaxDynamicSharedMemorySize, 128 * 1024)};
    (void)lds_attrs;
    *log2f_out = log2f; *log2t_out = log2t;
}
template <int ROWS, bool HEAVY>
static void launch_score(Batch& b, uint32_t grid, size_t lds, const uint64_t* hits, uint32_t sizes, uint32_t sb, const CandSlots& cs)
{
    hipLaunchKernelGGL((k_score<ROWS, HEAVY>), dim3(grid), dim3(WG), lds, b.st, hits, (const uint64_t*)b.ws->d_qrange, b.d_opts, sizes, sb, b.ws->d_cands[0],
                       (uint64_t)b.ws->cap_cands, b.ws->d_counters, (uint64_t)0, cs.qcand, cs.qcand_n, cs.heavy, b.cancel);
}

static int upload_piece(Batch& b, uint32_t c)
{
    Workspace* ws = b.ws;
    const uint64_t h0 = b.offsets[b.up_q[c]] - b.base, h1 = b.offsets[b.up_q[c + 1]] - b.base;
    if (h1 > h0) FPX_HIP(hipMemcpyAsync(ws->d_hashes + h0, b.hashes + b.base + h0, (h1 - h0) * sizeof(uint32_t), hipMemcpyHostToDevice, ws->copy_stream));
    FPX_HIP(hipEventRecord(ws->ev_chunk[c], ws->copy_stream));
    return FPX_OK;
}
static int place_batch(Batch& b, bool query_wg)
{
    Workspace* ws = b.ws; hipStream_t st = b.st; const uint32_t B = b.B; const uint64_t P = b.P, base = b.base; int rc;
    if (b.resident) {
        b.d_hashes_base = b.resident->d_hashes;
        b.d_offsets = b.resident->d_offsets + b.q0;
        b.d_opts = b.resident->d_opts + (size_t)b.q0 * 4;
        return FPX_OK;
    }
    if (B == 1 && 32 + P * sizeof(uint32_t) <= STAGE_BYTES) {
        if (!ws->h_stage) {
            FPX_HIP(hipHostMalloc(reinterpret_cast<void**>(&ws->h_stage), STAGE_BYTES, hipHostMallocMapped));
            FPX_HIP(hipHostGetDevicePointer(reinterpret_cast<void**>(&ws->d_stage), ws->h_stage, 0));
        }
        std::vector<uint32_t> h_opts;
        fill_opts(h_opts, b.opts, b.offsets, 1);
        uint64_t* so = reinterpret_cast<uint64_t*>(ws->h_stage);
        so[0] = 0; so[1] = P;
        std::memcpy(ws->h_stage + 16, h_opts.data(), 16);
        if (P) std::memcpy(ws->h_stage + 32, b.hashes + base, P * sizeof(uint32_t));
        b.d_hashes_base = reinterpret_cast<const uint32_t*>(ws->d_stage + 32);
        b.d_offsets = reinterpret_cast<const uint64_t*>(ws->d_stage);
        b.d_opts = reinterpret_cast<const uint32_t*>(ws->d_stage + 16);
        b.staged_single = true;
        return FPX_OK;
    }
    if ((rc = grow(&ws->d_hashes, &ws->cap_hashes, (size_t)P + 1))) return rc;
    std::vector<uint32_t>& h_opts = ws->h_opts;
    fill_opts(h_opts, b.opts, b.offsets, B);
    if (query_wg && B >= 1024u && P >= (1u << 20)) {
        if (!ws->copy_stream) {
            FPX_HIP(hipStreamCreateWithFlags(&ws->copy_stream, hipStreamNonBlocking));
            for (hipEvent_t& e : ws->ev_chunk) FPX_HIP(hipEventCreateWithFlags(&e, hipEventDisableTiming));
        }
        hipStream_t cs = ws->copy_stream;
        FPX_HIP(hipMemcpyAsync(ws->d_offsets, b.offsets, ((size_t)B + 1) * sizeof(uint64_t), hipMemcpyHostToDevice, cs));
        FPX_HIP(hipMemcpyAsync(ws->d_opts, h_opts.data(), h_opts.size() * sizeof(uint32_t), hipMemcpyHostToDevice, cs));
        b.up_chunks = Workspace::UP_CHUNKS;
        for (uint32_t c = 0; c <= b.up_chunks; ++c) b.up_q[c] = (uint32_t)((uint64_t)B * c / b.up_chunks);
        if ((rc = upload_piece(b, 0u))) return rc;
    } else {
        if (P) FPX_HIP(hipMemcpyAsync(ws->d_hashes, b.hashes + base, P * sizeof(uint32_t), hipMemcpyHostToDevice, st));
        FPX_HIP(hipMemcpyAsync(ws->d_offsets, b.offsets, ((size_t)B + 1) * sizeof(uint64_t), hipMemcpyHostToDevice, st));
        FPX_HIP(hipMemcpyAsync(ws->d_opts, h_opts.data(), h_opts.size() * sizeof(uint32_t), hipMemcpyHostToDevice, st));
        FPX_HIP(hipStreamSynchronize(st));
    }
    b.d_hashes_base = ws->d_hashes - base;
    b.d_offsets = ws->d_offsets;
    b.d_opts = ws->d_opts;
    return FPX_OK;
}
static int ensure_def_lists(Batch& b, bool side_wg)
{
    Snapshot* snap = b.snap; Workspace* ws = b.ws; int rc;
    b.def_cap = std::max<size_t>(4096, (size_t)(b.P / 8));
    if (snap->n_lean || snap->n_direct || side_wg) {
        const size_t need = b.def_cap * std::max(1u, snap->n_lean);
        if ((rc = grow(&ws->d_def_list, &ws->cap_def, need))) return rc;
        if (snap->n_lean > ws->cap_def_segs || !ws->d_def_count) {
            if (ws->d_def_count) (void)hipFree(ws->d_def_count);
            if (ws->h_def_count) (void)hipHostFree(ws->h_def_count);
            ws->d_def_count = nullptr; ws->h_def_count = nullptr; ws->cap_def_segs = 0;
            const size_t nseg = std::max(1u, snap->n_lean);
            const size_t words = nseg * DEF_COUNT_STRIDE + LEAN_STAT_WORDS;
            FPX_HIP(dmalloc(&ws->d_def_count, words * sizeof(unsigned int)));
            FPX_HIP(hipHostMalloc(reinterpret_cast<void**>(&ws->h_def_count), words * sizeof(unsigned int), hipHostMallocMapped));
            ws->cap_def_segs = nseg;
        }
    }
    b.def_stat_off = (size_t)ws->cap_def_segs * DEF_COUNT_STRIDE;
    b.def_words = b.def_stat_off + LEAN_STAT_WORDS;
    return FPX_OK;
}

static bool queries_fit_wg(const uint64_t* offsets, const fpx_opts* opts, uint32_t B, bool low_ok = false, bool* has_low = nullptr)
{
    bool low = false;
    for (uint32_t q = 0; q < B; ++q) {
        const uint64_t raw_len = offsets[q + 1] - offsets[q];
        if (raw_len > QS_MAX_HASHES) return false;
        if (query_floor(opts[q], raw_len) <= 2u) {
            if (!low_ok) return false;
            low = true;
        }
    }
    if (has_low) *has_low = low;
    return true;
}
static bool group_filtered(const GroupDesc& gd) { return gd.any_dead != 0u || gd.active != (gd.nseg >= 32u ? 0xFFFFFFFFu : ((1u << gd.nseg) - 1u)); }

static bool low_floors_ok(const Ctx* ctx, bool filtered)
{
    const int64_t low_wg = ctx_opt(ctx, OPT_LOW_WG);
    return low_wg == 2 || (low_wg == 1 && !filtered);
}
static bool several_groups_ok(const Snapshot* snap)
{
    const int64_t groups_wg = ctx_opt(snap->ctx, OPT_GROUPS_WG);
    if (snap->n_group < 2u || snap->n_group > QS_MAX_GROUPS || (groups_wg != 1 && groups_wg != 2)) return false;
    for (uint32_t i = 0; i < snap->n_group; ++i)
        if (!snap->groups[i]->packed || snap->h_group[i].win_lo != 0u || snap->h_group[i].win_hi != 0xFFFFFFFFu) return false;
    return true;
}
static bool several_groups_low_ok(const Ctx* ctx, bool any_filtered)
{
    return ctx_opt(ctx, OPT_GROUPS_WG) == 2 && low_floors_ok(ctx, any_filtered);
}
static bool takes_query_wg(const Snapshot* snap, const uint64_t* offsets, const fpx_opts* opts, uint32_t B, bool* filt, bool* low)
{
    const int64_t query_wg = ctx_opt(snap->ctx, OPT_QUERY_WG);
    if (!(snap->n_file == 0 && snap->n_solo == 0 && snap->n_group >= 1 && snap->n_direct != 0 &&
          (snap->n_mem == 0 || snap->mem_items == 0 || snap->d_memtab != nullptr) && query_wg != 0)) return false;
    if (snap->n_group != 1) {
        if (!several_groups_ok(snap)) return false;
        *filt = false;
        for (uint32_t i = 0; i < snap->n_group; ++i) *filt = *filt || group_filtered(snap->h_group[i]);
        *low = false;
        return (!*filt || query_wg == 2) && queries_fit_wg(offsets, opts, B, several_groups_low_ok(snap->ctx, *filt), low);
    }
    if (!snap->groups[0]->packed) return false;
    *filt = group_filtered(snap->h_group[0]);
    return (!*filt || query_wg == 2) && queries_fit_wg(offsets, opts, B, low_floors_ok(snap->ctx, *filt), low);
}
static bool takes_side_wg(const Snapshot* snap, const uint64_t* offsets, const fpx_opts* opts, uint32_t B)
{
    if (!(ctx_opt(snap->ctx, OPT_SIDE_WG) == 1 &&
          snap->n_group == 0 && snap->n_lean == 0 && snap->n_gen == 0 && snap->n_file == snap->n_small && snap->n_direct == snap->n_solo &&
          snap->n_small + snap->n_solo != 0 && (snap->n_mem == 0 || snap->mem_items == 0))) return false;
    for (const SegDesc& d : snap->h_file) if (!(d.own_flags == 0u && d.items && d.sbucket && d.sfirst && d.scode)) return false;
    for (const SegDesc& d : snap->h_direct) if (!(d.own_flags == 0u && d.drec && d.primary)) return false;
    return queries_fit_wg(offsets, opts, B);
}
static bool takes_words_wg(const Snapshot* snap, const uint64_t* offsets, const fpx_opts* opts, uint32_t B, bool* filt)
{
    const int64_t words_wg = ctx_opt(snap->ctx, OPT_WORDS_WG);
    if (!(words_wg != 0 && snap->n_group == 1 && !snap->groups[0]->packed && snap->n_file == 0 && snap->n_solo == 0 && snap->n_direct != 0 &&
          (snap->n_mem == 0 || snap->mem_items == 0 || snap->d_memtab != nullptr))) return false;
    *filt = group_filtered(snap->h_group[0]);
    return (!*filt || words_wg == 2) && queries_fit_wg(offsets, opts, B);
}

template <class Args>
static int open_wg_path(Batch& b, size_t extra_words, CandSlots* cs, Args* a)
{
    Workspace* ws = b.ws; int rc;
    if ((rc = ensure_cand_slots(ws, b.B, extra_words, cs))) return rc;
    hipLaunchKernelGGL(k_qs_zero, dim3(8), dim3(256), 0, b.st, ws->d_counters, ws->d_def_count, (uint32_t)b.def_words);
    FPX_HIP(hipEventRecord(ws->ev_probe0, b.st));
    a->hashes_base = b.d_hashes_base; a->offsets = b.d_offsets; a->opts = b.d_opts; a->sb = 32u - b.qb;
    a->cands = ws->d_cands[0]; a->cand_cap = ws->cap_cands; a->qcand = cs->qcand; a->qcand_n = cs->qcand_n;
    a->counters = ws->d_counters; a->stat_sets = device_stat_sets(b);
    a->qstats = b.want_q ? ws->d_qstats : nullptr; a->cancel = b.cancel;
    return FPX_OK;
}
static int close_wg_pass(Batch& b, uint32_t sb, const CandSlots& cs, ResultsTo* to)
{
    Workspace* ws = b.ws; int rc;
    FPX_HIP(hipGetLastError());
    FPX_HIP(hipEventRecord(ws->ev_probe1, b.st));
    if ((rc = results_target(b, to))) return rc;
    launch_finish(b, ws->d_cands[0], 0, sb, cs, to->res, to->n, b.stats != nullptr);
    if ((rc = publish(b, true))) return rc;
    FPX_HIP(hipEventRecord(ws->ev_end, b.st));
    FPX_SYNC_BATCH(b);
    return handed_back(ws, b.snap) ? FPX_REDO_QS : FPX_OK;
}
static int finish_wg_path(Batch& b, const ResultsTo& to, uint64_t Cf, uint32_t path_bits)
{
    Workspace* ws = b.ws; int rc;
    if (!b.partial && (rc = deliver_results(ws, b.B, b.out_cap, to.staged, b.out, b.out_n, b.st))) return rc;
    const unsigned long long* ls = host_stat_sets(b);
    const StatSums s = sum_stat_sets(ls);
    gather_hist(ws->batch_hist, ws->h_counters, ls, s.probes);
    if (fpx_stats* stats = b.stats) {
        float ms = 0.f, total_ms = 0.f;
        (void)hipEventElapsedTime(&ms, ws->ev_probe0, ws->ev_probe1);
        (void)hipEventElapsedTime(&total_ms, ws->ev_begin, ws->ev_end);
        stats->probes += s.probes; stats->scanned_blocks += s.blocks; stats->scanned_docs += s.docs; stats->hits += s.records;
        stats->algorithmic_bytes += s.blocks * 512ull + s.bytes_off;
        stats->candidates += Cf + ws->h_counters[CTR_SLOTCANDS];
        stats->probe_kernel_ms += ms; stats->total_gpu_ms += total_ms; stats->probe_launches += 1;
        stats->probe_kernel_bytes += s.blocks * 512ull + s.bytes_off;
        stats->probe_kernel_fetched_bytes += (s.dreads + 1) / 2 * 128ull;
        stats->path_flags |= 1u | (Cf ? 2u : 0u) | path_bits;
    }
    if ((rc = deliver_qstats(b))) return rc;
    ws->hint_P = b.P; ws->hint_H = std::max<uint64_t>(s.records, 1);
    ws->hint_misc = 0; ws->hint_def = 0;
    return FPX_OK;
}
static int redo_hot_queries(Batch& b, QSearchArgs qa, const GroupArgs& gargs, bool ns8, int cus, uint64_t R)
{
    if (R > qs_redo_limit(b.B) || R > qa.redo_cap) {
        __atomic_store_n(&b.snap->qs_skip, 32u, __ATOMIC_RELAXED);
        return FPX_REDO_QS;
    }
    int rc;
    qa.q_begin = 0u; qa.q_end = (uint32_t)R; qa.next_q = nullptr; qa.stagger = 0u;
    FPX_LAUNCH_QS(k_search_classes, dim3(std::min<uint32_t>((uint32_t)R, (uint32_t)cus * QS_WGS_PER_CU)), b.st, qa, gargs, ns8, qa.mem_tab != nullptr);
    if ((rc = publish(b, true))) return rc;
    FPX_HIP(hipEventRecord(b.ws->ev_end, b.st));
    FPX_SYNC_BATCH(b);
    return handed_back(b.ws, b.snap) ? FPX_REDO_QS : FPX_OK;
}

static_assert(QS_MAX_GROUPS * Workspace::UP_CHUNKS <= DEF_COUNT_STRIDE, "the launches' next_q words -- one per (upload piece, group) -- are the first deferred-list count's line, which k_qs_zero clears");
static int run_query_wg(Batch& b, bool filt, bool low)
{
    Snapshot* snap = b.snap; Workspace* ws = b.ws; hipStream_t st = b.st; const uint32_t B = b.B; int rc;
    const uint32_t ngroups = snap->n_group;
    const bool ns8 = snap->groups[0]->ns == 8u;
    const bool hot_wg = !filt && !low && ngroups == 1u && ctx_opt(snap->ctx, OPT_HOT_WG) == 1;
    if (low) {
        size_t want = 0;
        for (uint32_t q = 0; q < B; ++q) {
            const bool low_q = query_floor(b.opts[q], b.offsets[q + 1] - b.offsets[q]) <= 2u;
            want += low_q ? (size_t)ngroups * (std::min<size_t>(b.opts[q].max_results, QS_REC_CAP) + 32u) : 64u;
        }
        if (ws->cap_cands < want && (rc = grow_pair(ws->d_cands, &ws->cap_cands, want))) return rc;
    }
    CandSlots cs;
    QSearchArgs qa{};
    if ((rc = open_wg_path(b, hot_wg ? (size_t)B : 0, &cs, &qa))) return rc;
    struct Running {
        std::atomic<int>* c; int before;
        explicit Running(std::atomic<int>* c_) : c(c_), before(c_->fetch_add(1)) {}
        ~Running() { c->fetch_sub(1); }
    } running(&snap->ctx->qs_running);
    const bool alone = running.before == 0;
    qa.q_begin = 0u; qa.q_end = B;
    if (snap->n_mem != 0 && snap->mem_items != 0) { qa.mem_tab = snap->d_memtab; qa.mem_bucket = snap->d_membucket; qa.mem_bits = snap->d_membits; }
    if (hot_wg) { qa.redo = reinterpret_cast<unsigned long long*>(cs.extra); qa.redo_cap = B; }
    const bool coop = filt && !low && ngroups == 1u && ctx_opt(snap->ctx, OPT_FILT_COOP) == 1 &&
                      (snap->h_group[0].any_dead == 0u || (snap->dead_union && snap->dead_union->d_bits != nullptr));
    if (coop && snap->h_group[0].any_dead != 0u) {
        qa.dead_union = snap->dead_union->d_bits; qa.dead_union_last = (uint32_t)(snap->dead_union->words - 1u);
    }
    const GroupArgs gargs{snap->h_group[0], snap->d_direct};
    const bool filt0 = group_filtered(snap->h_group[0]), mem = qa.mem_tab != nullptr;
    const int cus = device_cus(snap->ctx);
    const uint32_t up_chunks = b.up_chunks;
    uint32_t next_launches = 0;
    for (uint32_t c = 0; c < std::max(1u, up_chunks); ++c) {
        qa.q_begin = up_chunks ? b.up_q[c] : 0u; qa.q_end = up_chunks ? b.up_q[c + 1] : B;
        if (qa.q_end == qa.q_begin) { if (up_chunks && c + 1u < up_chunks && (rc = upload_piece(b, c + 1u))) return rc; continue; }
        qa.next_q = (FPX_QS_DYN && alone) ? ws->d_def_count + c : nullptr;
        qa.stagger = alone ? QS_STAGGER : 0u;
        if (up_chunks) FPX_HIP(hipStreamWaitEvent(st, ws->ev_chunk[c], 0));
        const dim3 grid(std::min<uint32_t>(qa.q_end - qa.q_begin, (uint32_t)cus * QS_WGS_PER_CU));
        if (low && filt0) FPX_LAUNCH_QS(k_search_low_filt, grid, st, qa, gargs, ns8, b.want_q, mem);
        else if (low) FPX_LAUNCH_QS(k_search_low, grid, st, qa, gargs, ns8, b.want_q, mem);
        else if (coop) FPX_LAUNCH_QS(k_search_filt, grid, st, qa, gargs, ns8, b.want_q, mem);
        else FPX_LAUNCH_QS(k_search_query, grid, st, qa, gargs, ns8, b.want_q, mem, filt0);
        if (ngroups > 1u) {
            QSearchArgs qn = qa;
            qn.mem_tab = nullptr; qn.mem_bucket = nullptr; qn.mem_bits = nullptr;
            for (uint32_t gi = 1; gi < ngroups; ++gi) {
                qn.next_q = qa.next_q ? ws->d_def_count + (size_t)gi * Workspace::UP_CHUNKS + c : nullptr;
                const bool ns8_g = snap->groups[gi]->ns == 8u, filt_g = group_filtered(snap->h_group[gi]);
                const GroupArgs gargs_g{snap->h_group[gi], snap->d_direct};
                if (low) FPX_LAUNCH_QS(k_search_low_next, grid, st, qn, gargs_g, ns8_g, b.want_q, filt_g);
                else FPX_LAUNCH_QS(k_search_next, grid, st, qn, gargs_g, ns8_g, b.want_q, filt_g);
                ++next_launches;
            }
        }
        if (up_chunks && c + 1u < up_chunks && (rc = upload_piece(b, c + 1u))) return rc;
    }
    ResultsTo to;
    if ((rc = close_wg_pass(b, qa.sb, cs, &to)) != FPX_OK && rc != FPX_REDO_QS) return rc;
#ifdef FPX_QS_PROF
    fprintf(stderr, "qs_prof clocks/query: setup %.0f dedup %.0f rounds %.0f tasks %.0f count+exact %.0f handover %.0f", ws->h_counters[CTR_HIST] / (double)B, ws->h_counters[CTR_HIST + 1] / (double)B,
            ws->h_counters[CTR_HIST + 2] / (double)B, ws->h_counters[CTR_HIST + 3] / (double)B, ws->h_counters[CTR_HIST + 4] / (double)B, ws->h_counters[CTR_HIST + 5] / (double)B);
    fprintf(stderr, " | dedup: hash wait %.0f | rounds: hash wait %.0f heads wait %.0f words wait %.0f probe %.0f | next offsets wait %.0f\n", ws->h_counters[CTR_HIST + 6] / (double)B,
            ws->h_counters[CTR_HIST + 7] / (double)B, ws->h_counters[CTR_HIST + 8] / (double)B, ws->h_counters[CTR_HIST + 9] / (double)B, ws->h_counters[CTR_HIST + 10] / (double)B,
            ws->h_counters[CTR_HIST + 11] / (double)B);
#endif
    if (rc) return rc;
    const uint64_t R = hot_wg ? ws->h_counters[CTR_REDO] : 0;
    if (R != 0 && (rc = redo_hot_queries(b, qa, gargs, ns8, cus, R))) return rc;
    uint64_t Cf = 0;
    if (ws->h_counters[CTR_CANDS] != 0 || R != 0) {
        Cf = ws->h_counters[CTR_CANDS];
        if ((rc = finish_crowded(b, qa.sb, cs, to, Cf))) return rc;
    }
    if ((rc = finish_wg_path(b, to, Cf, 4u | 64u | (filt ? 256u : 0u) | (R != 0 ? 1024u : 0u) | (low ? 4096u : 0u) | (ngroups > 1u ? 8192u : 0u) | (coop ? 65536u : 0u)))) return rc;
    if (b.stats) b.stats->probe_launches += next_launches;
    return FPX_OK;
}

static int run_side_wg(Batch& b)
{
    Snapshot* snap = b.snap; const uint32_t B = b.B; int rc;
    CandSlots cs;
    SideArgs sa{};
    if ((rc = open_wg_path(b, 0, &cs, &sa.f))) return rc;
    sa.f.B = B;
    sa.small = snap->d_small; sa.n_small = snap->n_small; sa.solo = snap->d_solo; sa.n_solo = snap->n_solo;
    const int cus = device_cus(snap->ctx);
    hipLaunchKernelGGL(k_search_side, dim3(std::min<uint32_t>(B, (uint32_t)cus * QF_WGS_PER_CU)), dim3(QF_WG), QF_LDS_BYTES, b.st, sa);
    ResultsTo to;
    if ((rc = close_wg_pass(b, sa.f.sb, cs, &to))) return rc;
    const uint64_t Cf = b.ws->h_counters[CTR_CANDS];
    if (Cf != 0 && (rc = finish_crowded(b, sa.f.sb, cs, to, Cf))) return rc;
    return finish_wg_path(b, to, Cf, 512u);
}

static int run_words_wg(Batch& b, bool filt)
{
    Snapshot* snap = b.snap; const uint32_t B = b.B; int rc;
    CandSlots cs;
    WordsArgs wa{};
    if ((rc = open_wg_path(b, 0, &cs, &wa.f))) return rc;
    wa.f.B = B;
    if (snap->n_mem != 0 && snap->mem_items != 0) { wa.mem_tab = snap->d_memtab; wa.mem_bucket = snap->d_membucket; wa.mem_bits = snap->d_membits; }
    const GroupArgs gargs{snap->h_group[0], snap->d_direct};
    const int cus = device_cus(snap->ctx);
    FPX_LAUNCH(k_search_words, dim3(std::min<uint32_t>(B, (uint32_t)cus * QF_WGS_PER_CU)), QF_WG, QF_LDS_BYTES, b.st, wa, gargs,
               snap->groups[0]->ns == 8u, wa.mem_tab != nullptr, filt);
    ResultsTo to;
    if ((rc = close_wg_pass(b, wa.f.sb, cs, &to))) return rc;
    const uint64_t Cf = b.ws->h_counters[CTR_CANDS];
    if (Cf != 0 && (rc = finish_crowded(b, wa.f.sb, cs, to, Cf))) return rc;
    return finish_wg_path(b, to, Cf, 4u | 2048u | (filt ? 256u : 0u));
}

struct Keys { const uint64_t* d_pairs; bool flagged; uint32_t key_skip; };

static int make_keys(Batch& b, bool single_fast, bool score_only, Keys* keys)
{
    Snapshot* snap = b.snap; Workspace* ws = b.ws; hipStream_t st = b.st; const uint64_t* offsets = b.offsets;
    const uint32_t B = b.B; const uint64_t P = b.P, base = b.base; const unsigned qb = b.qb;
    int rc, kcur = 0;
    bool flagged = snap->n_file == 0 && (snap->n_mem == 0 || snap->d_memtab != nullptr) && snap->n_direct != 0 && !score_only;
    for (uint32_t q = 0; q < B && flagged; ++q) flagged = offsets[q + 1] - offsets[q] <= DEDUP_MAX;
    const uint32_t key_skip = flagged ? KEY_SORT_SKIP_DIRECT : KEY_SORT_SKIP;
    const uint64_t local_sort_max = (uint64_t)std::max<int64_t>(0, ctx_opt(snap->ctx, OPT_LOCAL_SORT_MAX));
    bool local_sort = P && !score_only && !single_fast && !flagged && B >= 2u && P <= local_sort_max && snap->n_small == 0;
    if (local_sort)
        for (uint32_t q = 0; q < B && local_sort; ++q) local_sort = offsets[q + 1] - offsets[q] <= QSORT_MAX;
    if (local_sort) {
        hipLaunchKernelGGL(k_make_keys_sorted, dim3(B), dim3(256), 0, st, b.d_hashes_base, b.d_offsets, B, qb, base, ws->d_keys[0],
                           (snap->n_lean || snap->n_direct) ? ws->d_def_count : nullptr, (uint32_t)b.def_words);
        FPX_HIP(hipGetLastError());
    } else if (P && !score_only) {
        const uint64_t order_min = (uint64_t)std::max<int64_t>(0, ctx_opt(snap->ctx, OPT_ORDER_MIN_PAIRS));
        KeyOrder ko{};
        const uint64_t order_max = 1ull << 20;
        const bool own_order = flagged && !single_fast && P >= order_min && P <= order_max;
        if (own_order && (rc = key_order_setup(ws, B, 0u, 32u - key_skip, &ko, nullptr, st, B >= KO_ROWS_MIN_B))) return rc;
        const uint64_t key_base = b.staged_single ? 0ull : base;
        if (flagged)
            hipLaunchKernelGGL(k_make_keys_dedup, dim3(B), dim3(256), 0, st, b.d_hashes_base, b.d_offsets, B, qb, key_base, ws->d_keys[0],
                               single_fast ? ws->d_counters : nullptr, ws->d_def_count, (uint32_t)b.def_words, ko);
        else
            hipLaunchKernelGGL(k_make_keys, dim3(B), dim3(256), 0, st, b.d_hashes_base, b.d_offsets, B, qb, key_base, ws->d_keys[0],
                               single_fast ? ws->d_counters : nullptr, (snap->n_lean || snap->n_direct) ? ws->d_def_count : nullptr, (uint32_t)b.def_words);
        if (own_order) {
            if (ko.qrows) hipLaunchKernelGGL(k_group_hist, dim3((B + KO_GROUP - 1u) / KO_GROUP), dim3(256), 0, st, ko, B);
            hipLaunchKernelGGL(k_bucket_scan, dim3(ko.nb), dim3(256), 0, st, ko, (B + KO_GROUP - 1u) / KO_GROUP);
            hipLaunchKernelGGL(k_scatter_keys, dim3((B + KO_GROUP - 1u) / KO_GROUP), dim3(256), 0, st, ko, (const uint64_t*)ws->d_keys[0], b.d_offsets, key_base, 0u, B, qb,
                               ws->d_keys[1], (unsigned long long*)nullptr);
            FPX_HIP(hipGetLastError());
            kcur = 1;
        } else if (!(flagged && P <= local_sort_max)) {
            if ((rc = sort_keys(ws, ws->d_keys, P, qb + key_skip, 32 + qb, st, &kcur))) return rc;
        }
    }
    keys->d_pairs = ws->d_keys[kcur];
    keys->flagged = flagged;
// ... 474 lines not shown
            gs.probe_kernel_ms = ms;
            gs.probe_aux_ms = 0.f;
            if (pr.used_lean) FPX_HIP(hipEventElapsedTime(&gs.probe_aux_ms, ws->ev_probe1, ws->ev_probe2));
        }
        H = ws->h_counters[CTR_HITS];
        if (pr.used_lean) {
            bool overflow = false;
            for (uint32_t i = 0; i < snap->n_lean; ++i) overflow = overflow || ws->h_def_count[(size_t)i * DEF_COUNT_STRIDE] > b.def_cap;
            if (overflow) {
                if (pr.attempt >= 3) { set_error("deferred list overflow persists"); return FPX_E_DEVICE; }
                pr.force_generic = true;
                continue;
            }
        }
        if (H <= ws->cap_hits) break;
        if (pr.attempt >= 4) { set_error("hit buffer overflow persists (%llu records)", (unsigned long long)H); return FPX_E_DEVICE; }
        if ((rc = grow_pair(ws->d_hits, &ws->cap_hits, (size_t)H + 1024))) return rc;
    }
    const bool spread = pr.spread, used_lean = pr.used_lean;
    if (score_only) {
        H = ex->n;
        if (H > ws->cap_hits && (rc = grow_pair(ws->d_hits, &ws->cap_hits, (size_t)H + 1024))) return rc;
        if (H) FPX_HIP(hipMemcpyAsync(ws->d_hits[0], ex->d_records, H * sizeof(uint64_t), hipMemcpyDeviceToDevice, st));
    }
    if (b.timeout_ms && now_ms() - b.t_start > (double)b.timeout_ms) return FPX_E_TIMEOUT;
    gs.scanned_blocks = ws->h_counters[CTR_BLOCKS] + ws->h_counters[8 + CTR_BLOCKS]; gs.scanned_docs = ws->h_counters[CTR_DOCS] + ws->h_counters[8 + CTR_DOCS];
    gs.algorithmic_bytes = ws->h_counters[CTR_BYTES] + ws->h_counters[8 + CTR_BYTES]; gs.probes = ws->h_counters[CTR_PROBES] + ws->h_counters[8 + CTR_PROBES];
    gs.generic_iters = (uint32_t)ws->h_counters[CTR_GENERIC];
    gs.probe_kernel_bytes = spread ? ws->h_counters[8 + CTR_BYTES] : ws->h_counters[CTR_BYTES];
    gs.probe_kernel_fetched_bytes = spread ? ws->h_counters[CTR_LEAN_READS] * 128ull  : unspread_fetched_bytes(ws, snap);
    gs.hits = H; gs.probe_launches = pr.launches; gs.path_flags = pr.used_fused ? 4u : 0u;
    if (!score_only) gather_hist(ws->batch_hist, ws->h_counters, spread ? host_stat_sets(b) : nullptr, gs.probes);
    auto fill_stats = [&]() {
        if (!b.stats) return;
        (void)hipEventElapsedTime(&gs.total_gpu_ms, ws->ev_begin, ws->ev_end);
        add_stats(b.stats, gs);
    };
    if (probe_only) {
        if ((rc = hand_records_over(b, ex, H))) return rc;
        fill_stats();
        return FPX_OK;
    }
    int ccur = 0;
    const uint32_t sb = 32u - b.qb;
    CandSlots cs;
    if (H && (rc = score_general(b, score_only, H, sb, &cs, &C, &ccur))) return rc;
    if (b.timeout_ms && now_ms() - b.t_start > (double)b.timeout_ms) return FPX_E_TIMEOUT;

    const bool count_slots = b.stats && cs.qcand_n;
    launch_finish(b, ws->d_cands[ccur], C, sb, cs, b.partial ? b.out : ws->d_out, b.partial ? b.out_n : ws->d_out_n, count_slots);
    FPX_HIP(hipGetLastError());
    bool staged = false;
    if (!b.partial && (rc = stage_results(ws, B, b.out_cap, st, &staged))) return rc;
    if (count_slots)
        FPX_HIP(hipMemcpyAsync(&ws->h_counters[CTR_SLOTCANDS], &ws->d_counters[CTR_SLOTCANDS], sizeof(unsigned long long), hipMemcpyDeviceToHost, st));
    FPX_HIP(hipEventRecord(ws->ev_end, st));
    FPX_SYNC_BATCH(b);
    if (b.timeout_ms && now_ms() - b.t_start > (double)b.timeout_ms) return FPX_E_TIMEOUT;
    if (!b.partial && (rc = deliver_results(ws, B, b.out_cap, staged, b.out, b.out_n, st))) return rc;
    gs.candidates = C + (count_slots ? ws->h_counters[CTR_SLOTCANDS] : 0ull);
    fill_stats();
    if ((rc = deliver_qstats(b))) return rc;
    ws->hint_P = P; ws->hint_H = std::max<uint64_t>(H, 1);
    ws->hint_def = 0;
    if (used_lean) for (uint32_t i = 0; i < snap->n_lean; ++i) ws->hint_def = std::max<uint32_t>(ws->hint_def, ws->h_def_count[(size_t)i * DEF_COUNT_STRIDE]);
    return FPX_OK;
}

static int run_batch(Snapshot* snap, Workspace* ws, const QueryBatch* resident, uint32_t q0,
                     const uint32_t* hashes, const uint64_t* offsets, uint32_t B,
                     const fpx_opts* opts, uint32_t timeout_ms, bool partial,
                     fpx_result* out, uint32_t out_cap, uint32_t* out_n, fpx_stats* stats, const Exchange* ex = nullptr,
                     Try mode = Try::First, double t_call = 0.0, uint64_t* q_blocks = nullptr, uint64_t* q_docs = nullptr)
{
    const bool score_only = ex && ex->mode == 2;
    const bool no_fast = mode == Try::GeneralOnly, no_qs = mode != Try::First;
    Batch b{};
    b.snap = snap; b.ws = ws; b.st = ws->stream;
    b.resident = resident; b.q0 = q0; b.hashes = hashes; b.offsets = offsets; b.opts = opts; b.B = B;
    b.t_start = t_call != 0.0 ? t_call : now_ms(); b.timeout_ms = timeout_ms;
    std::memset(ws->batch_hist, 0, sizeof ws->batch_hist);
    __atomic_store_n(ws->h_cancel, 0u, __ATOMIC_RELEASE);
    b.cancel = timeout_ms ? ws->d_cancel : nullptr;
    b.base = offsets[0]; b.P = offsets[B] - b.base; b.qb = bits_for(B);
    b.partial = partial; b.out = out; b.out_cap = out_cap; b.out_n = out_n; b.stats = stats; b.q_blocks = q_blocks; b.q_docs = q_docs;
    const uint64_t P = b.P;
    int rc;
    if ((rc = ensure_queries(ws, B))) return rc;
    if ((rc = grow_pair(ws->d_keys, &ws->cap_keys, (size_t)P + 1))) return rc;
    if (!partial && (rc = grow(&ws->d_out, &ws->cap_out, (size_t)B * out_cap + 1))) return rc;
    static_assert(sizeof(fpx_result) == 8, "fpx_result layout");

    const bool single_fast = B == 1 && !partial && !ex && !no_fast && P != 0 && out_cap <= SINGLE_OUT_MAX &&
                             (snap->n_lean == 0 || P * snap->n_file < lean_min_probes(snap->ctx));
    bool query_wg = false, words_wg = false, side_wg = false, filt = false, low = false;
    if (!ex && !no_fast && !no_qs && !single_fast && B >= 2u && P != 0 && b.qb <= 24u) {
        query_wg = takes_query_wg(snap, offsets, opts, B, &filt, &low);
        words_wg = !query_wg && takes_words_wg(snap, offsets, opts, B, &filt);
        side_wg = !query_wg && !words_wg && takes_side_wg(snap, offsets, opts, B);
        if (query_wg || words_wg || side_wg) {
            const uint32_t skip = __atomic_load_n(&snap->qs_skip, __ATOMIC_RELAXED);
            if (skip != 0u) { __atomic_store_n(&snap->qs_skip, skip - 1u, __ATOMIC_RELAXED); query_wg = words_wg = side_wg = false; }
        }
    }

    if (!single_fast) FPX_HIP(hipEventRecord(ws->ev_begin, b.st));
    if ((rc = place_batch(b, query_wg))) return rc;
    if ((rc = ensure_def_lists(b, side_wg))) return rc;
    Keys keys{};
    if (!query_wg && !words_wg && !side_wg && (rc = make_keys(b, single_fast, score_only, &keys))) return rc;
    b.want_q = (q_blocks || q_docs) && B >= 2u && !score_only;
    if (b.want_q && (rc = grow(&ws->d_qstats, &ws->cap_qstats, (size_t)B + 1))) return rc;
    if (query_wg) return run_query_wg(b, filt, low);
    if (words_wg) return run_words_wg(b, filt);
    if (side_wg) return run_side_wg(b);

    if (ws->cap_hits == 0) {
        size_t want = std::max<size_t>(1u << 20, (size_t)P * std::max<uint32_t>(1u, snap->n_file + snap->n_direct + snap->n_mem));
        if ((rc = grow_pair(ws->d_hits, &ws->cap_hits, want))) return rc;
    }
    bool fast = ctx_opt(snap->ctx, OPT_FAST) != 0 && !ex && !no_fast && !single_fast && B >= 2u && P != 0 && b.qb <= 24u &&
                (1u << level1_bits(b.qb)) <= MAX_BINS && ws->hint_H != 0 && ws->hint_P != 0;
    if (fast && ws->fast_penalty != 0) { ws->fast_penalty -= 1; fast = false; }
    if (fast) return run_device_sized(b, keys);
    if (single_fast) return run_single(b, keys);
    return run_general(b, keys, ex);
}

static bool parts_take(const Snapshot* snap, const uint64_t* offsets, const fpx_opts* opts, uint32_t B)
{
    const int64_t query_wg = ctx_opt(snap->ctx, snap->part[0]->groups[0]->packed ? OPT_QUERY_WG : OPT_WORDS_WG);
    if (query_wg == 0) return false;
    const Snapshot* p0 = snap->part[0];
    bool filtered = false;
    for (uint32_t i = 0; i < p0->n_group; ++i) filtered = filtered || group_filtered(p0->h_group[i]);
    const bool packed = p0->groups[0]->packed;
    if (query_wg != 2 && filtered) return false;
    if (bits_for(B) > 24u || offsets[B] == offsets[0]) return false;
    if (p0->n_group > 1u) return several_groups_ok(p0) && queries_fit_wg(offsets, opts, B, several_groups_low_ok(snap->ctx, filtered));
    return queries_fit_wg(offsets, opts, B, packed && low_floors_ok(snap->ctx, filtered));
}

static int run_with_redos(Snapshot* snap, Workspace* ws, const QueryBatch* resident, uint32_t q0, const uint32_t* hashes, const uint64_t* offsets, uint32_t B,
                          const fpx_opts* opts, uint32_t timeout_ms, bool partial, fpx_result* out, uint32_t out_cap, uint32_t* out_n, fpx_stats* local,
                          double t_call, uint64_t* q_blocks, uint64_t* q_docs)
{
    auto run = [&](Try mode) { return run_batch(snap, ws, resident, q0, hashes, offsets, B, opts, timeout_ms, partial, out, out_cap, out_n, local, nullptr, mode, t_call, q_blocks, q_docs); };
    int rc = run(Try::First);
    if (rc == FPX_REDO_QS) {
        *local = fpx_stats{};
        rc = run(Try::NoQueryWg);
    }
    if (rc == FPX_REDO) {
        *local = fpx_stats{};
        rc = run(Try::GeneralOnly);
    }
    return rc;
}

static int search_parts(Snapshot* snap, const QueryBatch* resident, const uint32_t* hashes, const uint64_t* offsets, uint32_t B,
                        const fpx_opts* opts, uint32_t timeout_ms, fpx_result* out, uint32_t out_cap, uint32_t* out_n, fpx_stats* stats, double t_call,
                        uint64_t* q_blocks, uint64_t* q_docs)
{
    Ctx* ctx = snap->ctx;
    uint32_t cap = 1;
    for (uint32_t q = 0; q < B; ++q) cap = std::max(cap, std::min(opts[q].max_results, out_cap ? out_cap : 1u));
// ... 97 lines not shown
    if (qb->ctx != snap->ctx) { set_error("query batch and snapshot belong to different contexts"); return FPX_E_INVAL; }
    if (stats) std::memset(stats, 0, sizeof *stats);
    for (uint32_t d = 0; d < world; ++d) counts[d] = 0;
    if (qb->B == 0) return FPX_OK;
    FPX_HIP(hipSetDevice(snap->ctx->device));
    Workspace* ws = ws_acquire(snap->ctx);
    if (!ws) return FPX_E_NOMEM;
    Exchange ex;
    ex.mode = 1; ex.world = world; ex.d_records = d_records; ex.cap = records_cap; ex.counts = counts;
    int rc = run_batch(snap, ws, qb, 0, nullptr, qb->offsets.data(), qb->B, qb->opts.data(), timeout_ms, true,
                       nullptr, 0, nullptr, stats, &ex);
    if (rc != FPX_OK) (void)hipStreamSynchronize(ws->stream);
    ws_release(snap->ctx, ws);
    return rc;
}

int score_records_impl(Ctx* ctx, const QueryBatch* qb, const uint64_t* d_records, uint64_t num_records, uint32_t timeout_ms,
                       fpx_result* d_out, uint32_t out_cap, uint32_t* d_out_n)
{
    if (qb->ctx != ctx) { set_error("query batch belongs to a different context"); return FPX_E_INVAL; }
    if (qb->B == 0) return FPX_OK;
    FPX_HIP(hipSetDevice(ctx->device));
    Workspace* ws = ws_acquire(ctx);
    if (!ws) return FPX_E_NOMEM;
    Snapshot none;
    none.ctx = ctx;
    Exchange ex;
    ex.mode = 2; ex.d_records = const_cast<uint64_t*>(d_records); ex.n = num_records;
    int rc = run_batch(&none, ws, qb, 0, nullptr, qb->offsets.data(), qb->B, qb->opts.data(), timeout_ms, true,
                       d_out, out_cap, d_out_n, nullptr, &ex);
    if (rc != FPX_OK) (void)hipStreamSynchronize(ws->stream);
    ws_release(ctx, ws);
    return rc;
}

void query_batch_free(QueryBatch* qb)
{
    if (!qb) return;
    (void)hipSetDevice(qb->ctx->device);
    if (qb->d_hashes) (void)hipFree(qb->d_hashes);
    if (qb->d_offsets) (void)hipFree(qb->d_offsets);
    if (qb->d_opts) (void)hipFree(qb->d_opts);
    delete qb;
}

int query_batch_create_impl(Ctx* ctx, const uint32_t* hashes, const uint64_t* offsets, uint32_t B,
                            const fpx_opts* opts, QueryBatch** out)
{
    *out = nullptr;
    if (!ctx || !offsets || !opts || (B && offsets[B] && !hashes)) { set_error("null argument"); return FPX_E_INVAL; }
    if (offsets[0] != 0) { set_error("offsets[0] must be 0"); return FPX_E_INVAL; }
    for (uint32_t q = 0; q < B; ++q) {
        if (offsets[q + 1] < offsets[q]) { set_error("offsets must be non-decreasing"); return FPX_E_INVAL; }
    }
    FPX_HIP(hipSetDevice(ctx->device));
    QueryBatch* qb = new (std::nothrow) QueryBatch();
    if (!qb) return FPX_E_NOMEM;
    qb->ctx = ctx; qb->B = B;
    qb->offsets.assign(offsets, offsets + B + 1);
    qb->opts.assign(opts, opts + B);
    std::vector<uint32_t> h_opts;
    fill_opts(h_opts, opts, offsets, B);
    const uint64_t P = offsets[B];
    hipError_t e = dmalloc(&qb->d_hashes, (P + 1) * sizeof(uint32_t));
    if (e == hipSuccess) e = dmalloc(&qb->d_offsets, ((size_t)B + 1) * sizeof(uint64_t));
    if (e == hipSuccess) e = dmalloc(&qb->d_opts, ((size_t)B * 4 + 4) * sizeof(uint32_t));
    if (e == hipSuccess && P) e = hipMemcpy(qb->d_hashes, hashes, P * sizeof(uint32_t), hipMemcpyHostToDevice);
    if (e == hipSuccess) e = hipMemcpy(qb->d_offsets, offsets, ((size_t)B + 1) * sizeof(uint64_t), hipMemcpyHostToDevice);
    if (e == hipSuccess && B) e = hipMemcpy(qb->d_opts, h_opts.data(), h_opts.size() * sizeof(uint32_t), hipMemcpyHostToDevice);
    if (e != hipSuccess) { query_batch_free(qb); return hip_fail(e, "query batch upload"); }
    *out = qb;
    return FPX_OK;
}

int merge_partials_impl(Ctx* ctx, const void* d_parts, const void* d_counts, uint32_t world,
                        uint32_t B, uint32_t part_cap, const fpx_opts* opts, const uint64_t* offsets,
                        fpx_result* out, uint32_t out_cap, uint32_t* out_n)
{
    if (!ctx || !d_parts || !d_counts || !opts || !offsets || !out_n) { set_error("null argument"); return FPX_E_INVAL; }
    if (B == 0) return FPX_OK;
    FPX_HIP(hipSetDevice(ctx->device));
    Workspace* ws = ws_acquire(ctx);
    if (!ws) return FPX_E_NOMEM;
    int rc = FPX_OK;
    auto body = [&]() -> int {
        int r;
        if ((r = ensure_queries(ws, B))) return r;
        if ((r = grow(&ws->d_out, &ws->cap_out, (size_t)B * out_cap + 1))) return r;
        std::vector<uint32_t> h_opts;
        fill_opts(h_opts, opts, offsets, B);
        hipStream_t st = ws->stream;
        FPX_HIP(hipMemcpyAsync(ws->d_opts, h_opts.data(), h_opts.size() * sizeof(uint32_t), hipMemcpyHostToDevice, st));
        hipLaunchKernelGGL(k_merge, dim3((B + 127) / 128), dim3(128), 0, st,
                           (const fpx_result*)d_parts, (const uint32_t*)d_counts, world, B, part_cap, ws->d_opts,
                           ws->d_out, out_cap, ws->d_out_n);
        FPX_HIP(hipGetLastError());
        bool staged = false;
        if ((r = stage_results(ws, B, out_cap, st, &staged))) return r;
        FPX_HIP(hipStreamSynchronize(st));
        return deliver_results(ws, B, out_cap, staged, out, out_n, st);
    };
    rc = body();
    ws_release(ctx, ws);
    return rc;
}

constexpr uint32_t SHARD_BQ = 3;
constexpr uint64_t SHARD_NEED_MARK = 0x40000000ull;

template <int QPW, uint32_t CAP>
__global__ __launch_bounds__(QPW == 8 ? 512 : 256) void k_make_keys_window(const uint32_t* __restrict__ hashes_base, const uint64_t* __restrict__ offsets,
                                                          uint32_t B, uint32_t qb, uint64_t* __restrict__ keys, uint32_t stride,
                                                          uint32_t win_lo, uint32_t win_hi, unsigned long long* counters, uint32_t* __restrict__ overflow,
                                                          KeyOrder ko)
{
    static_assert(QPW == 1 || QPW == 8, "a workgroup per query, or a wave per query of a group");
    constexpr uint32_t WG_T = QPW == 8 ? 512u : 256u;
    constexpr uint32_t TEAM = WG_T / QPW;
    constexpr uint32_t UNR = QPW == 8 ? 16u : 4u;
    constexpr uint32_t LIST_CAP = CAP;
    constexpr uint32_t SLOTS = 2u * CAP;
    constexpr uint32_t SLOT_SHIFT = 32u - (CAP == 512u ? 10u : CAP == 1024u ? 11u : 12u);
    static_assert(CAP == 512u || CAP == 1024u || CAP == 2048u, "the hash set's size");
    __shared__ uint32_t s_list[QPW][LIST_CAP];
    __shared__ uint32_t s_tab[QPW][SLOTS];
    __shared__ uint32_t s_hist[KO_MAX_BUCKETS];
    __shared__ uint32_t s_n[QPW], s_out[QPW], s_ones[QPW];
    const uint32_t tid = threadIdx.x, team = tid / TEAM, lt = tid % TEAM, lane = tid & 63u;
    const uint32_t q = blockIdx.x * QPW + team;
    if (blockIdx.x == 0 && tid < CTR_COUNT) counters[tid] = 0ull;
    const bool live = q < B;
    for (uint32_t i = lt; i < SLOTS; i += TEAM) s_tab[team][i] = 0xFFFFFFFFu;
    if (tid < KO_MAX_BUCKETS) s_hist[tid] = 0u;
    if (lt == 0) { s_n[team] = 0u; s_out[team] = 0u; s_ones[team] = 0u; }
    __syncthreads();
    const uint64_t lo = live ? offsets[q] : 0ull, hi = live ? offsets[q + 1] : 0ull;
    const uint64_t below = (1ull << lane) - 1ull;
    uint32_t n = 0;
    for (uint64_t i0 = lo; i0 < hi; i0 += TEAM * UNR) {
        uint32_t h[UNR]; bool in[UNR];
#pragma unroll
        for (uint32_t u = 0; u < UNR; ++u) {
            const uint64_t i = i0 + u * TEAM + lt;
            in[u] = i < hi;
            h[u] = in[u] ? hashes_base[i] : 0u;
        }
#pragma unroll
        for (uint32_t u = 0; u < UNR; ++u) {
            in[u] = in[u] && h[u] >= win_lo && h[u] <= win_hi;
            const uint64_t m = __ballot(in[u]);
            if (m == 0ull) continue;
            uint32_t base = n;
            if constexpr (QPW == 1) {
                if (lane == (uint32_t)__builtin_ctzll(m)) base = atomicAdd(&s_n[team], (uint32_t)__popcll(m));
                base = __shfl(base, __builtin_ctzll(m));
            } else {
                n += (uint32_t)__popcll(m);
            }
            const uint32_t at = base + (uint32_t)__popcll(m & below);
            if (in[u] && at < LIST_CAP) s_list[team][at] = h[u];
        }
    }
    __syncthreads();
    if constexpr (QPW == 1) n = s_n[team];
    if (n > LIST_CAP) { if (lt == 0) *overflow = 1u; n = LIST_CAP; }
    uint64_t* mine = keys + (size_t)q * stride;
// ... 31 lines not shown
                mine[at] = ((uint64_t)h << qb) | q;
                if (ko.nb) atomicAdd(&s_hist[(h >> ko.bshift) & (ko.nb - 1u)], 1u);
            } else {
                *overflow = 1u;
            }
        }
    }
    __syncthreads();
    if constexpr (QPW == 1) n_out = s_out[team];
    if (live && lt == 0 && ko.qn) ko.qn[q] = min(n_out, stride);
    if (ko.nb && tid < ko.nb) {
        const uint32_t G = (B + KO_GROUP - 1u) / KO_GROUP;
        if constexpr (QPW == 8) ko.cnt[(size_t)tid * G + blockIdx.x] = s_hist[tid];
        else if (s_hist[tid] != 0u) atomicAdd(&ko.cnt[(size_t)tid * G + q / KO_GROUP], s_hist[tid]);
    }
}

__global__ void k_cell_counts(const unsigned int* __restrict__ bin_count, uint32_t ncells, uint32_t* __restrict__ out, unsigned long long* __restrict__ counters,
                              uint32_t flag)
{
    const uint32_t c = blockIdx.x * blockDim.x + threadIdx.x;
    if (c >= ncells) return;
    const unsigned int v = bin_count[(size_t)c * BIN_STRIDE];
    out[c] = v | flag;
    atomicMax(&counters[CTR_TOTAL], (unsigned long long)v);
    atomicAdd(&counters[CTR_SLOTCANDS], (unsigned long long)v);
}

static unsigned log2_exact(uint32_t v) { unsigned b = 0; while ((1u << b) < v) ++b; return b; }

static unsigned shard_sort_bits(unsigned win_bits) { return win_bits >= 8u ? 0u : 8u - win_bits; }

static_assert(SHARD_DEDUP_MAX == DEDUP_MAX, "fpx_sharded.hip routes longer queries to the record protocol");
static_assert(QS_SHARE_BQ == SHARD_BQ && QS_SHARE_STRIDE == BIN_STRIDE && DEDUP_MAX <= QS_MAX_HASHES, "k_search_window fills the protocol's bins");
static_assert(QS_PACK_MAX <= DEDUP_MAX, "k_search_packed takes the shorter queries of what k_search_window takes");
bool shard_window_walk_ok(const Snapshot* snap)
{
    const int64_t shard_wg = ctx_opt(snap->ctx, OPT_SHARD_WG);
    if (shard_wg != 1 && shard_wg != 2) return false;
    if (snap->n_group != 1 || snap->n_solo != 0 || snap->n_file != 0 || !snap->groups[0]->packed) return false;
    if (snap->n_mem != 0 && snap->mem_items != 0 && !snap->d_memtab) return false;
    return shard_wg == 2 || !group_filtered(snap->h_group[0]);
}
int shard_bins_per_rank(uint32_t B, uint32_t world)
{
    const uint32_t nb = (B + (1u << SHARD_BQ) - 1u) >> SHARD_BQ;
    return (int)((nb + world - 1u) / world);
}

int shard_probe_impl(Snapshot* snap, const QueryBatch* qb, uint32_t world, uint32_t timeout_ms,
                     uint64_t* d_send, uint64_t cell_cap, uint32_t* d_send_counts, uint64_t* needed_cell_cap, fpx_stats* stats)
{
    if (qb->ctx != snap->ctx) { set_error("query batch and snapshot belong to different contexts"); return FPX_E_INVAL; }
    if (stats) std::memset(stats, 0, sizeof *stats);
    if (needed_cell_cap) *needed_cell_cap = 0;
    const uint32_t B = qb->B;
    if (B == 0) return FPX_OK;
    if (snap->n_group == 0 || snap->n_solo != 0 || snap->n_file != 0 || (snap->n_mem != 0 && !snap->d_memtab && snap->mem_items != 0)) {
        set_error("fpx_shard_probe: the snapshot is not made of groups of direct-addressed segments (and memory segments behind their table) alone (use fpx_probe_resident)"); return FPX_E_INVAL;
    }
    uint32_t win_lo = snap->h_group[0].win_lo, win_hi = snap->h_group[0].win_hi;
    for (const GroupDesc& gd : snap->h_group)
        if (gd.win_lo != win_lo || gd.win_hi != win_hi) { set_error("fpx_shard_probe: the snapshot's groups have different hash windows"); return FPX_E_INVAL; }
    const uint64_t* offsets = qb->offsets.data();
    uint64_t max_len = 0;
    for (uint32_t q = 0; q < B; ++q) max_len = std::max<uint64_t>(max_len, offsets[q + 1] - offsets[q]);
    if (max_len > DEDUP_MAX) { set_error("fpx_shard_probe: queries of more than %u hashes (use fpx_probe_resident)", DEDUP_MAX); return FPX_E_INVAL; }
    for (uint32_t q = 0; q < B; ++q) {
        const fpx_opts& o = qb->opts[q];
        if (query_floor(o, offsets[q + 1] - offsets[q]) <= 2u) {
            set_error("fpx_shard_probe: query %u has a score floor of 1 or 2: this batch takes the record protocol (fpx_probe_resident)", q); return FPX_E_INVAL;
        }
    }
    if (max_len == 0) max_len = 1;
    const unsigned qbits = bits_for(B);
    if (qbits > 24u) { set_error("fpx_shard_probe: at most 2^24 queries"); return FPX_E_INVAL; }
    const uint32_t ncells = (uint32_t)shard_bins_per_rank(B, world) * world;
    if (ncells > (1u << 21)) { set_error("fpx_shard_probe: too many bins"); return FPX_E_INVAL; }
    const double share = ((double)win_hi - (double)win_lo + 1.0) / 4294967296.0;
    const unsigned win_bits = log2_exact(std::max<uint32_t>(1u, (uint32_t)(1.0 / std::max(share, 1e-9) + 0.5)));
    FPX_HIP(hipSetDevice(snap->ctx->device));
    Workspace* ws = ws_acquire(snap->ctx);
    if (!ws) return FPX_E_NOMEM;
    auto body = [&]() -> int {
        int rc;
        hipStream_t st = ws->stream;
        const double t_start = now_ms();
        __atomic_store_n(ws->h_cancel, 0u, __ATOMIC_RELEASE);
        const uint32_t* cancel = timeout_ms ? ws->d_cancel : nullptr;
        const size_t cell_words = (size_t)ncells * BIN_STRIDE, words = cell_words + LEAN_STAT_WORDS + 16;
        if (words > ws->cap_cells) {
            if (ws->d_cells) (void)hipFree(ws->d_cells);
            if (ws->h_cells) (void)hipHostFree(ws->h_cells);
            ws->d_cells = nullptr; ws->h_cells = nullptr; ws->cap_cells = 0;
            FPX_HIP(dmalloc(&ws->d_cells, words * sizeof(uint32_t)));
            FPX_HIP(hipHostMalloc(reinterpret_cast<void**>(&ws->h_cells), (LEAN_STAT_WORDS + 16) * sizeof(uint32_t)));
            ws->cap_cells = words;
        }
        uint32_t* d_stats32 = ws->d_cells + cell_words;
        uint32_t* d_overflow = d_stats32 + LEAN_STAT_WORDS;
        if (ws->cap_hits == 0 && (rc = grow_pair(ws->d_hits, &ws->cap_hits, (size_t)1 << 22))) return rc;
        uint32_t stride = (uint32_t)std::min<uint64_t>(max_len, (uint64_t)((double)max_len * share * 1.25) + 48);
        const bool rec32_enabled = ctx_opt(snap->ctx, OPT_REC32) != 0;
        uint64_t rec_cap = cell_cap;
        bool walk = shard_window_walk_ok(snap), walked = false, packed = false;
        const bool pack = ctx_opt(snap->ctx, OPT_SHARD_PACK) == 1 && max_len <= QS_PACK_MAX;
        if (walk) {
            const uint32_t skip = __atomic_load_n(&snap->qs_skip, __ATOMIC_RELAXED);
            if (skip != 0u) { __atomic_store_n(&snap->qs_skip, skip - 1u, __ATOMIC_RELAXED); walk = false; }
        }
        for (int attempt = 0;; ++attempt) {
            const uint32_t rec32 = rec32_enabled && !__atomic_load_n(&snap->rec32_refused, __ATOMIC_RELAXED) &&
                                   snap->max_doc_declared < (0xFFFFFFFFu >> SHARD_BQ) ? 1u : 0u;
            rec_cap = cell_cap << rec32;
            if (walk) {
                FPX_HIP(hipMemsetAsync(ws->d_cells, 0, words * sizeof(uint32_t), st));
                FPX_HIP(hipMemsetAsync(ws->d_counters, 0, CTR_COUNT * sizeof(unsigned long long), st));
                QSearchArgs qa{};
                qa.hashes_base = qb->d_hashes; qa.offsets = qb->d_offsets; qa.opts = qb->d_opts; qa.q_begin = 0u; qa.q_end = B; qa.sb = 32u - qbits;
                qa.counters = ws->d_counters; qa.stat_sets = reinterpret_cast<unsigned long long*>(d_stats32); qa.qstats = nullptr; qa.cancel = cancel;
                if (snap->n_mem != 0 && snap->mem_items != 0) { qa.mem_tab = snap->d_memtab; qa.mem_bucket = snap->d_membucket; qa.mem_bits = snap->d_membits; }
                qa.bins = d_send; qa.bin_cap = rec_cap; qa.bin_fill = ws->d_cells; qa.bin_rec32 = rec32;
                qa.next_q = FPX_QS_DYN ? d_overflow + 4 : nullptr; qa.stagger = 0u;
                const GroupArgs gargs{snap->h_group[0], snap->d_direct};
                const dim3 grid(std::min<uint32_t>(B, (uint32_t)device_cus(snap->ctx) * QS_WGS_PER_CU));
                FPX_HIP(hipEventRecord(ws->ev_probe0, st));
                const bool ns8 = snap->groups[0]->ns == 8u, mem = qa.mem_tab != nullptr, filt = group_filtered(snap->h_group[0]);
                if (pack) FPX_LAUNCH_QS(k_search_packed, grid, st, qa, gargs, ns8, mem, filt);
                else FPX_LAUNCH_QS(k_search_window, grid, st, qa, gargs, ns8, mem, filt);
                FPX_HIP(hipEventRecord(ws->ev_probe1, st));
                hipLaunchKernelGGL(k_cell_counts, dim3((ncells + 255) / 256), dim3(256), 0, st, (const unsigned int*)ws->d_cells, ncells, d_send_counts, ws->d_counters,
                                   rec32 << 31);
                FPX_HIP(hipGetLastError());
                FPX_HIP(hipMemcpyAsync(ws->h_counters, ws->d_counters, CTR_COUNT * sizeof(unsigned long long), hipMemcpyDeviceToHost, st));
                FPX_HIP(hipMemcpyAsync(ws->h_cells, d_stats32, (LEAN_STAT_WORDS + 16) * sizeof(uint32_t), hipMemcpyDeviceToHost, st));
                FPX_SYNC(ws);
                if (ws->h_counters[CTR_BINFAIL] == 3 && attempt < 3) {
                    __atomic_store_n(&snap->rec32_refused, 1u, __ATOMIC_RELAXED);
                    continue;
                }
                if (ws->h_counters[CTR_BINFAIL] != 0) {
                    __atomic_store_n(&snap->qs_skip, 32u, __ATOMIC_RELAXED);
                    walk = false; attempt = -1;
                    continue;
                }
                walked = true; packed = pack;
                break;
            }
            const uint64_t P = (uint64_t)B * stride;
            if ((rc = grow_pair(ws->d_keys, &ws->cap_keys, (size_t)P + 1))) return rc;
            FPX_HIP(hipMemsetAsync(ws->d_cells, 0, words * sizeof(uint32_t), st));
            KeyOrder ko{};
            unsigned long long* d_P = nullptr;
            if ((rc = key_order_setup(ws, B, win_bits, shard_sort_bits(win_bits), &ko, &d_P, st))) return rc;
            static_assert(KO_GROUP == 8, "k_make_keys_window<8> makes the keys of one group per workgroup");
            if (stride <= 512u)
                hipLaunchKernelGGL((k_make_keys_window<8, 512>), dim3((B + 7u) / 8u), dim3(512), 0, st, (const uint32_t*)qb->d_hashes, (const uint64_t*)qb->d_offsets, B, qbits,
                                   ws->d_keys[0], stride, win_lo, win_hi, ws->d_counters, d_overflow, ko);
            else if (stride <= 1024u)
                hipLaunchKernelGGL((k_make_keys_window<8, 1024>), dim3((B + 7u) / 8u), dim3(512), 0, st, (const uint32_t*)qb->d_hashes, (const uint64_t*)qb->d_offsets, B, qbits,
                                   ws->d_keys[0], stride, win_lo, win_hi, ws->d_counters, d_overflow, ko);
            else
                hipLaunchKernelGGL((k_make_keys_window<1, DEDUP_MAX>), dim3(B), dim3(256), 0, st, (const uint32_t*)qb->d_hashes, (const uint64_t*)qb->d_offsets, B, qbits,
                                   ws->d_keys[0], stride, win_lo, win_hi, ws->d_counters, d_overflow, ko);
            hipLaunchKernelGGL(k_bucket_scan, dim3(ko.nb), dim3(256), 0, st, ko, (B + KO_GROUP - 1u) / KO_GROUP);
            hipLaunchKernelGGL(k_scatter_keys, dim3((B + KO_GROUP - 1u) / KO_GROUP), dim3(256), 0, st, ko, (const uint64_t*)ws->d_keys[0], (const uint64_t*)qb->d_offsets, 0ull, stride, B, qbits,
// ... 29 lines not shown
            else
                hipLaunchKernelGGL(k_bin_each, dim3(64), dim3(256), 0, st, hb, (const uint64_t*)ws->d_hits[1], (const unsigned long long*)&ws->d_counters[CTR_HITS], (uint64_t)ws->cap_hits);
            hipLaunchKernelGGL(k_cell_counts, dim3((ncells + 255) / 256), dim3(256), 0, st, (const unsigned int*)ws->d_cells, ncells, d_send_counts, ws->d_counters,
                               rec32 << 31);
            FPX_HIP(hipGetLastError());
            FPX_HIP(hipMemcpyAsync(ws->h_counters, ws->d_counters, CTR_COUNT * sizeof(unsigned long long), hipMemcpyDeviceToHost, st));
            FPX_HIP(hipMemcpyAsync(ws->h_cells, d_stats32, (LEAN_STAT_WORDS + 16) * sizeof(uint32_t), hipMemcpyDeviceToHost, st));
            FPX_SYNC(ws);
            if (ws->h_cells[LEAN_STAT_WORDS] != 0u && attempt == 0 && stride < max_len) { stride = (uint32_t)max_len; continue; }
            if (ws->h_counters[CTR_BINFAIL] == 3 && attempt < 3) {
                __atomic_store_n(&snap->rec32_refused, 1u, __ATOMIC_RELAXED);
                continue;
            }
            if (ws->h_counters[CTR_HITS] > ws->cap_hits) {
                if (attempt >= 3) { set_error("fpx_shard_probe: misc buffer overflow persists"); return FPX_E_DEVICE; }
                if ((rc = grow_pair(ws->d_hits, &ws->cap_hits, (size_t)ws->h_counters[CTR_HITS] + 1024))) return rc;
                continue;
            }
            break;
        }
        if (ws->h_counters[CTR_TOTAL] > rec_cap) {
            const uint64_t per_cell = rec_cap / std::max<uint64_t>(cell_cap, 1);
            if (needed_cell_cap) *needed_cell_cap = (ws->h_counters[CTR_TOTAL] * 17 / 16 + 128 + per_cell - 1) / std::max<uint64_t>(per_cell, 1);
            set_error("fpx_shard_probe: a bin holds %llu records, the send buffer has room for %llu per bin", (unsigned long long)ws->h_counters[CTR_TOTAL],
                      (unsigned long long)rec_cap);
            return FPX_E_AGAIN;
        }
        {
            const unsigned long long* ls = reinterpret_cast<const unsigned long long*>(ws->h_cells);
            uint64_t hist[HIST_SLOTS + 1];
            gather_hist(hist, ws->h_counters, ls, sum_stat_sets(ls).probes);
            ctx_hist_add(snap->ctx, hist, hist[HIST_SLOTS]);
        }
        if (stats) {
            const StatSums s = sum_stat_sets(reinterpret_cast<const unsigned long long*>(ws->h_cells));
            const unsigned long long blocks = s.blocks, docs = s.docs, probes = s.probes, dreads = s.dreads, bytes_off = s.bytes_off;
            const unsigned long long pads = ws->h_counters[CTR_PADS] + s.pads;
            float ms = 0.f;
            (void)hipEventElapsedTime(&ms, ws->ev_probe0, ws->ev_probe1);
            stats->probes = probes; stats->scanned_blocks = blocks; stats->scanned_docs = docs; stats->hits = ws->h_counters[CTR_SLOTCANDS] - std::min<unsigned long long>(pads, ws->h_counters[CTR_SLOTCANDS]);
            stats->algorithmic_bytes = blocks * 512ull + bytes_off; stats->probe_kernel_bytes = blocks * 512ull + bytes_off;
            stats->probe_kernel_fetched_bytes = dreads * 64ull; stats->probe_kernel_ms = ms; stats->total_gpu_ms = ms; stats->probe_launches = 1;
            stats->path_flags = 1u | 4u | 8u | 16u;
            if (walked) {
                stats->hits = s.records;
                stats->probe_kernel_fetched_bytes = (dreads + 1) / 2 * 128ull;
                stats->path_flags |= 64u | 16384u;
                if (packed) stats->path_flags |= 32768u;
            }
        }
        return FPX_OK;
    };
    const int rc = body();
    if (rc != FPX_OK) (void)hipStreamSynchronize(ws->stream);
    ws_release(snap->ctx, ws);
    return rc;
}

int shard_keys_impl(Ctx* ctx, const QueryBatch* qb, uint32_t world, uint32_t rank, uint32_t B_global,
                    uint64_t* d_keys_send, uint64_t key_cap, unsigned long long* d_key_counts, uint64_t* needed_key_cap)
{
    if (needed_key_cap) *needed_key_cap = 0;
    if (qb->ctx != ctx) { set_error("query batch belongs to a different context"); return FPX_E_INVAL; }
    if (world == 0 || world > KO_MAX_BUCKETS || (world & (world - 1u)) != 0u) { set_error("fpx_shard_keys: the number of ranks must be a power of two <= %u", KO_MAX_BUCKETS); return FPX_E_INVAL; }
    const uint32_t bpr = (uint32_t)shard_bins_per_rank(B_global, world);
    const uint32_t q_lo = std::min<uint64_t>(B_global, (uint64_t)rank * bpr << SHARD_BQ), q_hi = std::min<uint64_t>(B_global, (uint64_t)(rank + 1u) * bpr << SHARD_BQ);
    const uint32_t B = qb->B;
    if (B != q_hi - q_lo) { set_error("fpx_shard_keys: rank %u of %u finishes queries [%u, %u) of the batch of %u: its share must hold exactly those %u (got %u)", rank, world, q_lo, q_hi, B_global, q_hi - q_lo, B); return FPX_E_INVAL; }
    const unsigned qbits = bits_for(B_global);
    if (qbits > 24u) { set_error("fpx_shard_keys: at most 2^24 queries"); return FPX_E_INVAL; }
    FPX_HIP(hipSetDevice(ctx->device));
    if (B == 0) { FPX_HIP(hipMemset(d_key_counts, 0, (size_t)world * sizeof(unsigned long long))); return FPX_OK; }
    const uint64_t* offsets = qb->offsets.data();
    for (uint32_t q = 0; q < B; ++q) {
        const uint64_t len = offsets[q + 1] - offsets[q];
        if (len > DEDUP_MAX) { set_error("fpx_shard_keys: queries of more than %u hashes (use fpx_probe_resident)", DEDUP_MAX); return FPX_E_INVAL; }
        const fpx_opts& o = qb->opts[q];
        if (query_floor(o, len) <= 2u) {
            set_error("fpx_shard_keys: query %u has a score floor of 1 or 2: this batch takes the record protocol (fpx_probe_resident)", q_lo + q); return FPX_E_INVAL;
        }
    }
    Workspace* ws = ws_acquire(ctx);
    if (!ws) return FPX_E_NOMEM;
    auto body = [&]() -> int {
        int rc;
        hipStream_t st = ws->stream;
        const uint64_t P = offsets[B];
        if ((rc = grow_pair(ws->d_keys, &ws->cap_keys, (size_t)P + 1))) return rc;
        KeyOrder ko{};
        if ((rc = key_order_setup(ws, B, 0u, 8u, &ko, nullptr, st, B >= KO_ROWS_MIN_B))) return rc;
        if (ko.nb < world) { set_error("fpx_shard_keys: the batch is too large for %u ranks", world); return FPX_E_INVAL; }
        hipLaunchKernelGGL(k_make_keys_dedup, dim3(B), dim3(256), 0, st, (const uint32_t*)qb->d_hashes, (const uint64_t*)qb->d_offsets, B, qbits, 0ull, ws->d_keys[0],
                           (unsigned long long*)nullptr, (unsigned int*)nullptr, 0u, ko, q_lo);
        if (ko.qrows) hipLaunchKernelGGL(k_group_hist, dim3((B + KO_GROUP - 1u) / KO_GROUP), dim3(256), 0, st, ko, B);
        hipLaunchKernelGGL(k_bucket_scan, dim3(ko.nb), dim3(256), 0, st, ko, (B + KO_GROUP - 1u) / KO_GROUP);
        hipLaunchKernelGGL(k_scatter_keys, dim3((B + KO_GROUP - 1u) / KO_GROUP), dim3(256), 0, st, ko, (const uint64_t*)ws->d_keys[0], (const uint64_t*)qb->d_offsets, 0ull, 0u, B, qbits,
                           d_keys_send, (unsigned long long*)nullptr, ko.nb / world, key_cap, d_key_counts);
        FPX_HIP(hipGetLastError());
        std::vector<unsigned long long> hc(world);
        FPX_HIP(hipMemcpyAsync(hc.data(), d_key_counts, (size_t)world * sizeof(unsigned long long), hipMemcpyDeviceToHost, st));
        FPX_HIP(hipStreamSynchronize(st));
        unsigned long long worst = 0;
        for (unsigned long long c : hc) worst = std::max(worst, c);
        if (worst > key_cap) {
            if (needed_key_cap) *needed_key_cap = worst * 17 / 16 + 256;
            set_error("fpx_shard_keys: a window takes %llu keys, the send buffer has room for %llu per window", worst, (unsigned long long)key_cap);
            return FPX_E_AGAIN;
        }
        return FPX_OK;
    };
    const int rc = body();
    if (rc != FPX_OK) (void)hipStreamSynchronize(ws->stream);
    ws_release(ctx, ws);
    return rc;
}

int shard_probe_keys_impl(Snapshot* snap, const uint64_t* d_keys_recv, uint64_t key_cap, const unsigned long long* d_key_counts, uint32_t world, uint32_t B_global,
                          uint32_t timeout_ms, uint64_t* d_send, uint64_t cell_cap, uint32_t* d_send_counts, uint64_t* needed_cell_cap, fpx_stats* stats)
{
    if (stats) std::memset(stats, 0, sizeof *stats);
    if (needed_cell_cap) *needed_cell_cap = 0;
    const uint32_t B = B_global;
    if (B == 0) return FPX_OK;
    if (snap->n_group == 0 || snap->n_solo != 0 || snap->n_file != 0 || (snap->n_mem != 0 && !snap->d_memtab && snap->mem_items != 0)) {
        set_error("fpx_shard_probe_keys: the snapshot is not made of groups of direct-addressed segments (and memory segments behind their table) alone (use fpx_probe_resident)"); return FPX_E_INVAL;
    }
    const unsigned qbits = bits_for(B);
    if (qbits > 24u) { set_error("fpx_shard_probe_keys: at most 2^24 queries"); return FPX_E_INVAL; }
    const uint32_t ncells = (uint32_t)shard_bins_per_rank(B, world) * world;
    if (ncells > (1u << 21)) { set_error("fpx_shard_probe_keys: too many bins"); return FPX_E_INVAL; }
    FPX_HIP(hipSetDevice(snap->ctx->device));
    Workspace* ws = ws_acquire(snap->ctx);
    if (!ws) return FPX_E_NOMEM;
    auto body = [&]() -> int {
        int rc;
        hipStream_t st = ws->stream;
        const double t_start = now_ms();
        __atomic_store_n(ws->h_cancel, 0u, __ATOMIC_RELEASE);
        const uint32_t* cancel = timeout_ms ? ws->d_cancel : nullptr;
        const size_t cell_words = (size_t)ncells * BIN_STRIDE, words = cell_words + LEAN_STAT_WORDS + 16;
        if (words > ws->cap_cells) {
            if (ws->d_cells) (void)hipFree(ws->d_cells);
            if (ws->h_cells) (void)hipHostFree(ws->h_cells);
            ws->d_cells = nullptr; ws->h_cells = nullptr; ws->cap_cells = 0;
            FPX_HIP(dmalloc(&ws->d_cells, words * sizeof(uint32_t)));
            FPX_HIP(hipHostMalloc(reinterpret_cast<void**>(&ws->h_cells), (LEAN_STAT_WORDS + 16) * sizeof(uint32_t)));
            ws->cap_cells = words;
        }
        uint32_t* d_stats32 = ws->d_cells + cell_words;
        if (ws->cap_hits == 0 && (rc = grow_pair(ws->d_hits, &ws->cap_hits, (size_t)1 << 22))) return rc;
        const bool rec32_enabled = ctx_opt(snap->ctx, OPT_REC32) != 0;
        uint64_t rec_cap = cell_cap;
        for (int attempt = 0;; ++attempt) {
            const uint32_t rec32 = rec32_enabled && !__atomic_load_n(&snap->rec32_refused, __ATOMIC_RELAXED) &&
                                   snap->max_doc_declared < (0xFFFFFFFFu >> SHARD_BQ) ? 1u : 0u;
            rec_cap = cell_cap << rec32;
            FPX_HIP(hipMemsetAsync(ws->d_cells, 0, words * sizeof(uint32_t), st));
            FPX_HIP(hipMemsetAsync(ws->d_counters, 0, CTR_COUNT * sizeof(unsigned long long), st));
            ProbeArgs a;
            a.segs = snap->d_direct; a.P = key_cap; a.qb = qbits; a.ppw = 16u; a.bsp = 0u;
            a.hits = ws->d_hits[1]; a.hit_cap = ws->cap_hits; a.counters = ws->d_counters;
            a.def_list = nullptr; a.def_count = nullptr; a.def_cap = 0; a.ctr_off = 0; a.cancel = cancel;
            a.lean_stats = reinterpret_cast<unsigned long long*>(d_stats32);
            a.key_skip = KEY_SKIP_FLAGGED;
            a.bins = d_send; a.bin_cap = rec_cap; a.bin_count = ws->d_cells; a.bin_shift = SHARD_BQ; a.rec32 = rec32;
            const uint64_t wgs = (key_cap + FK_WG - 1) / FK_WG;
            a.rounds = (uint32_t)std::max<uint64_t>(1, std::min<uint64_t>(4, wgs * world / 8192));
            const uint64_t per_wg = (uint64_t)FK_WG * a.rounds;
            FPX_HIP(hipEventRecord(ws->ev_probe0, st));
            a.pairs = d_keys_recv; a.slot_stride = key_cap; a.P_dev = d_key_counts;
            for (const GroupDesc& gd : snap->h_group) {
                const GroupArgs gargs{gd, snap->d_direct};
                const dim3 grid((uint32_t)((key_cap + per_wg - 1) / per_wg), world);
                const Group* grp = snap->groups[&gd - snap->h_group.data()].get();
                launch_probe_group(grp->packed, grp->ns == 8u, true, false, grid, st, a, gargs);
            }
            if (snap->n_mem && snap->d_memtab)
                hipLaunchKernelGGL(k_probe_memtab, dim3(memtab_grid(key_cap), world), dim3(WG), 0, st, (const uint64_t*)snap->d_memtab, (const uint32_t*)snap->d_membucket,
                                   d_keys_recv, key_cap, qbits, KEY_SKIP_FLAGGED, ws->d_hits[1], (uint64_t)ws->cap_hits, ws->d_counters, d_key_counts, key_cap, (const uint32_t*)snap->d_membits);
            FPX_HIP(hipEventRecord(ws->ev_probe1, st));
            BinArgs hb{};
            hb.bins = d_send; hb.bin_cap = rec_cap; hb.bin_count = ws->d_cells; hb.shift = SHARD_BQ; hb.nbins = std::min<uint32_t>(ncells, MAX_SBINS);
            hb.rec32 = rec32; hb.counters = ws->d_counters;
            if (ncells <= MAX_SBINS)
                hipLaunchKernelGGL(k_bin, dim3(64), dim3(256), 0, st, hb, (const uint64_t*)ws->d_hits[1], (const unsigned long long*)&ws->d_counters[CTR_HITS], (uint64_t)ws->cap_hits);
            else
                hipLaunchKernelGGL(k_bin_each, dim3(64), dim3(256), 0, st, hb, (const uint64_t*)ws->d_hits[1], (const unsigned long long*)&ws->d_counters[CTR_HITS], (uint64_t)ws->cap_hits);
            hipLaunchKernelGGL(k_cell_counts, dim3((ncells + 255) / 256), dim3(256), 0, st, (const unsigned int*)ws->d_cells, ncells, d_send_counts, ws->d_counters,
                               rec32 << 31);
            FPX_HIP(hipGetLastError());
            FPX_HIP(hipMemcpyAsync(ws->h_counters, ws->d_counters, CTR_COUNT * sizeof(unsigned long long), hipMemcpyDeviceToHost, st));
            FPX_HIP(hipMemcpyAsync(ws->h_cells, d_stats32, (LEAN_STAT_WORDS + 16) * sizeof(uint32_t), hipMemcpyDeviceToHost, st));
            FPX_SYNC(ws);
            if (ws->h_counters[CTR_BINFAIL] == 3 && attempt < 3) { __atomic_store_n(&snap->rec32_refused, 1u, __ATOMIC_RELAXED); continue; }
            if (ws->h_counters[CTR_HITS] > ws->cap_hits) {
                if (attempt >= 3) { set_error("fpx_shard_probe_keys: misc buffer overflow persists"); return FPX_E_DEVICE; }
                if ((rc = grow_pair(ws->d_hits, &ws->cap_hits, (size_t)ws->h_counters[CTR_HITS] + 1024))) return rc;
                continue;
            }
            break;
        }
        if (ws->h_counters[CTR_TOTAL] > rec_cap) {
            const uint64_t per_cell = rec_cap / std::max<uint64_t>(cell_cap, 1);
            if (needed_cell_cap) *needed_cell_cap = (ws->h_counters[CTR_TOTAL] * 17 / 16 + 128 + per_cell - 1) / std::max<uint64_t>(per_cell, 1);
            set_error("fpx_shard_probe_keys: a bin holds %llu records, the send buffer has room for %llu per bin", (unsigned long long)ws->h_counters[CTR_TOTAL],
                      (unsigned long long)rec_cap);
            return FPX_E_AGAIN;
        }
        {
            const unsigned long long* ls = reinterpret_cast<const unsigned long long*>(ws->h_cells);
            uint64_t hist[HIST_SLOTS + 1];
            gather_hist(hist, ws->h_counters, ls, sum_stat_sets(ls).probes);
            ctx_hist_add(snap->ctx, hist, hist[HIST_SLOTS]);
        }
        if (stats) {
            const StatSums s = sum_stat_sets(reinterpret_cast<const unsigned long long*>(ws->h_cells));
            const unsigned long long blocks = s.blocks, docs = s.docs, probes = s.probes, dreads = s.dreads, bytes_off = s.bytes_off;
            const unsigned long long pads = ws->h_counters[CTR_PADS] + s.pads;
            float ms = 0.f;
            (void)hipEventElapsedTime(&ms, ws->ev_probe0, ws->ev_probe1);
            stats->probes = probes; stats->scanned_blocks = blocks; stats->scanned_docs = docs; stats->hits = ws->h_counters[CTR_SLOTCANDS] - std::min<unsigned long long>(pads, ws->h_counters[CTR_SLOTCANDS]);
            stats->algorithmic_bytes = blocks * 512ull + bytes_off; stats->probe_kernel_bytes = blocks * 512ull + bytes_off;
            stats->probe_kernel_fetched_bytes = dreads * 64ull; stats->probe_kernel_ms = ms; stats->total_gpu_ms = ms; stats->probe_launches = 1;
            stats->path_flags = 1u | 4u | 8u | 16u;
        }
        return FPX_OK;
    };
    const int rc = body();
    if (rc != FPX_OK) (void)hipStreamSynchronize(ws->stream);
    ws_release(snap->ctx, ws);
    return rc;
}

int shard_score_impl(Ctx* ctx, const QueryBatch* qb, uint32_t world, uint32_t rank, const uint64_t* d_recv, uint64_t cell_cap, const uint32_t* d_recv_counts,
                     uint32_t timeout_ms, fpx_result* out, uint32_t out_cap, uint32_t* out_n, uint32_t* first_query, uint32_t* num_queries,
                     uint64_t* needed_cell_cap, uint32_t B_global)
{
    if (needed_cell_cap) *needed_cell_cap = 0;
    if (qb->ctx != ctx) { set_error("query batch belongs to a different context"); return FPX_E_INVAL; }
    const uint32_t B = B_global ? B_global : qb->B;
    const uint32_t bpr = (uint32_t)shard_bins_per_rank(B, world);
    const uint32_t q_lo = std::min<uint64_t>(B, (uint64_t)rank * bpr << SHARD_BQ), q_hi = std::min<uint64_t>(B, (uint64_t)(rank + 1u) * bpr << SHARD_BQ);
    if (first_query) *first_query = q_lo;
    if (num_queries) *num_queries = q_hi - q_lo;
    if (B_global && qb->B != q_hi - q_lo) { set_error("fpx_shard_score_share: the share holds %u queries, rank %u of %u finishes %u", qb->B, rank, world, q_hi - q_lo); return FPX_E_INVAL; }
    if (q_hi == q_lo) {
        const size_t ncounts = (size_t)world * bpr;
        if (d_recv_counts && ncounts) {
            FPX_HIP(hipSetDevice(ctx->device));
            std::vector<uint32_t> h(ncounts);
            FPX_HIP(hipMemcpy(h.data(), d_recv_counts, ncounts * sizeof(uint32_t), hipMemcpyDeviceToHost));
            uint64_t need = 0;
            for (uint32_t c : h) if (((uint64_t)c & 0x7FFFFFFFull) >= SHARD_NEED_MARK) need = std::max<uint64_t>(need, (uint64_t)c & (SHARD_NEED_MARK - 1u));
            if (need) {
                if (needed_cell_cap) *needed_cell_cap = need;
                set_error("fpx_shard_score: a sender's bins need %llu cells, the exchange ran with %llu: redo the step", (unsigned long long)need, (unsigned long long)cell_cap);
                return FPX_E_AGAIN;
            }
        }
        return FPX_OK;
    }
    const uint32_t* d_opts_b = B_global ? qb->d_opts - (size_t)q_lo * 4 : qb->d_opts;
    const uint32_t nq = q_hi - q_lo;
    const unsigned qbits = bits_for(B);
    FPX_HIP(hipSetDevice(ctx->device));
    Workspace* ws = ws_acquire(ctx);
    if (!ws) return FPX_E_NOMEM;
    auto body = [&]() -> int {
        int rc;
        hipStream_t st = ws->stream;
        const double t_start = now_ms();
        __atomic_store_n(ws->h_cancel, 0u, __ATOMIC_RELEASE);
        const uint32_t* cancel = timeout_ms ? ws->d_cancel : nullptr;
        if ((rc = ensure_queries(ws, B))) return rc;
        if ((rc = grow(&ws->d_out, &ws->cap_out, (size_t)B * out_cap + 1))) return rc;
        if ((rc = grow(&ws->d_qcand, &ws->cap_qcand, (size_t)B * QCAND_SLOTS + 2 * ((size_t)B / 2 + 1) + bpr))) return rc;
        uint64_t* d_qcand = ws->d_qcand;
        uint32_t* d_qcand_n = reinterpret_cast<uint32_t*>(ws->d_qcand + (size_t)B * QCAND_SLOTS);
        uint32_t* d_bin_n = reinterpret_cast<uint32_t*>(ws->d_qcand + (size_t)B * QCAND_SLOTS + (size_t)B / 2 + 1);
        const size_t cand_guess = std::max<size_t>(1u << 16, (size_t)nq * 64);
        if (ws->cap_cands < cand_guess && (rc = grow_pair(ws->d_cands, &ws->cap_cands, cand_guess))) return rc;
        const uint32_t sbf = 32u - qbits;
        auto finish = [&](const uint64_t* cands, uint64_t C) {
            hipLaunchKernelGGL(k_finish, dim3((nq + 127) / 128), dim3(128), 0, st, cands, C, (const uint32_t*)d_opts_b, nq, sbf, 0,
                               ws->d_out, out_cap, ws->d_out_n, (const uint64_t*)(d_qcand + (size_t)q_lo * QCAND_SLOTS), (const uint32_t*)(d_qcand_n + q_lo),
                               (unsigned long long*)nullptr, q_lo);
        };
        bool staged = false;
        for (int attempt = 0;; ++attempt) {
        FPX_HIP(hipMemsetAsync(ws->d_counters, 0, CTR_COUNT * sizeof(unsigned long long), st));
        FPX_HIP(hipMemsetAsync(d_qcand_n, 0, (size_t)B * sizeof(uint32_t), st));
        ScoreBinArgs sa{};
        sa.bins = d_recv; sa.bin_cap = cell_cap; sa.rec_mode = 2u; sa.bin_count = d_recv_counts; sa.nsrc = world; sa.src_stride = (uint64_t)bpr * cell_cap;
        sa.count_stride = bpr; sa.count_step = 1u; sa.bq = SHARD_BQ; sa.bin_base = rank * bpr; sa.B = B;
        sa.opts = d_opts_b; sa.sb = sbf; sa.cands = ws->d_cands[0]; sa.cand_cap = ws->cap_cands; sa.counters = ws->d_counters;
        sa.qcand = d_qcand; sa.qcand_n = d_qcand_n; sa.bin_n = d_bin_n; sa.cancel = cancel;
        const size_t sb_lds = ((size_t)8u << SB_TABLE_LOG2) + ((size_t)2u << SB_FILTER_LOG2) + ((size_t)SB_CAND << SHARD_BQ) * 8u;
        const uint32_t my_bins = (nq + (1u << SHARD_BQ) - 1u) >> SHARD_BQ;
        hipLaunchKernelGGL(k_score_bin<false>, dim3(my_bins), dim3(SB_WG), sb_lds, st, sa);
        finish(ws->d_cands[0], 0);
        FPX_HIP(hipGetLastError());
        if ((rc = stage_results(ws, nq, out_cap, st, &staged))) return rc;
        FPX_HIP(hipMemcpyAsync(ws->h_counters, ws->d_counters, CTR_COUNT * sizeof(unsigned long long), hipMemcpyDeviceToHost, st));
        FPX_SYNC(ws);
        if (ws->h_counters[CTR_BINFAIL] == 2 && (ws->h_counters[CTR_TOTAL] & SHARD_NEED_MARK) != 0) {
            if (needed_cell_cap) *needed_cell_cap = ws->h_counters[CTR_TOTAL] & (SHARD_NEED_MARK - 1u);
            set_error("fpx_shard_score: a sender's bins need %llu cells, the exchange ran with %llu: redo the step", (unsigned long long)(ws->h_counters[CTR_TOTAL] & (SHARD_NEED_MARK - 1u)),
                      (unsigned long long)cell_cap);
            return FPX_E_AGAIN;
        }
        if (ws->h_counters[CTR_CANDS] > ws->cap_cands && attempt < 3) {
            if ((rc = grow_pair(ws->d_cands, &ws->cap_cands, (size_t)ws->h_counters[CTR_CANDS] + 1024))) return rc;
            continue;
        }
        if (ws->h_counters[CTR_BINFAIL] != 0 || ws->h_counters[CTR_MAXSCORE] != 0 || ws->h_counters[CTR_CANDS] > ws->cap_cands) {
            set_error("fpx_shard_score: a bin could not be scored in place (%s): use smaller batches or the record protocol (fpx_score_partial)",
                      ws->h_counters[CTR_BINFAIL] == 2 ? "a received bin overflowed" : ws->h_counters[CTR_MAXSCORE] ? "a score does not fit the candidate key" : "too many candidates");
            return FPX_E_INVAL;
        }
        break;
        }
        if (ws->h_counters[CTR_CANDS] != 0) {
            const uint64_t Cf = ws->h_counters[CTR_CANDS];
            int ccur = 0;
            if ((rc = sort_keys(ws, ws->d_cands, Cf, 0, 64, st, &ccur))) return rc;
            finish(ws->d_cands[ccur], Cf);
            FPX_HIP(hipGetLastError());
            if ((rc = stage_results(ws, nq, out_cap, st, &staged))) return rc;
            FPX_SYNC(ws);
        }
        return deliver_results(ws, nq, out_cap, staged, out, out_n, st);
    };
    const int rc = body();
    if (rc != FPX_OK) (void)hipStreamSynchronize(ws->stream);
    ws_release(ctx, ws);
    return rc;
}

__global__ __launch_bounds__(256) void k_bw_stream(const uint4* __restrict__ src, size_t n16, unsigned long long* sink)
{
    uint32_t acc = 0;
    for (size_t i = (size_t)blockIdx.x * blockDim.x + threadIdx.x; i < n16; i += (size_t)gridDim.x * blockDim.x) {
        uint4 v = src[i];
        acc ^= v.x ^ v.y ^ v.z ^ v.w;
    }
    if (acc == 0x9e3779b9u) atomicAdd(sink, 1ull);
}

__global__ __launch_bounds__(256) void k_bw_random(const uint8_t* __restrict__ src, uint64_t nblocks, uint32_t block_size,
                                                   uint32_t steps, unsigned long long* sink)
// ... 147 lines not shown
```

Baseline: 28.61 million.

## Fuse per-query finish and host publication into the query search kernel's last workgroup

In the single-group query search path, each workgroup now sorts its candidate slots and writes final results per query directly in the kernel. The last workgroup, chosen by an atomic ticket, copies counters, stat words and results into mapped host memory and resets them. This removes the separate finish kernel, the zeroing kernel on clean workspaces, and the device-to-host result transfers, cutting launches and host syncs per batch. The cost is more complexity, a serial tail in the last workgroup, and dependence on clean-state tracking across calls.

```diff
diff --git a/acoustid-index_amd/csrc/fpx_api.hip b/acoustid-index_amd/csrc/fpx_api.hip
--- a/acoustid-index_amd/csrc/fpx_api.hip
+++ b/acoustid-index_amd/csrc/fpx_api.hip
@@ -186,7 +186,7 @@
     if (w->h_cells) (void)hipHostFree(w->h_cells);
     void* bufs[] = {w->d_hashes, w->d_offsets, w->d_opts, w->d_keys[0], w->d_keys[1], w->d_hits[0], w->d_hits[1],
                     w->d_cands[0], w->d_cands[1], w->d_temp, w->d_counters, w->d_out, w->d_out_n, w->d_def_list, w->d_def_count, w->d_qrange, w->d_qcand,
-                    w->d_binq, w->d_qcursor, w->d_parts, w->d_parts_n};
+                    w->d_binq, w->d_qcursor, w->d_parts, w->d_parts_n, w->d_fin};
     for (void* b : bufs) if (b) (void)hipFree(b);
     if (w->h_counters) (void)hipHostFree(w->h_counters);
     if (w->h_stage) (void)hipHostFree(w->h_stage);
@@ -408,6 +408,7 @@
                {"shard_wg", "FPX_SHARD_WG", 0, 0, false},
              {"shard_pack", "FPX_SHARD_PACK", 0, 0, false},
               {"filt_coop", "FPX_FILT_COOP", 0, 0, false},
+              {"wg_finish", "FPX_WG_FINISH", 1, 0, false},
 };
 
 int64_t ctx_opt(const Ctx* c, CtxOpt o)
@@ -630,6 +631,7 @@
     if (o == OPT_SHARD_WG && value > 2) { set_error("fpx_ctx_set_option: shard_wg is 0, 1 or 2"); return FPX_E_INVAL; }
     if (o == OPT_SHARD_PACK && value > 1) { set_error("fpx_ctx_set_option: shard_pack is 0 or 1"); return FPX_E_INVAL; }
     if (o == OPT_FILT_COOP && value > 1) { set_error("fpx_ctx_set_option: filt_coop is 0 or 1"); return FPX_E_INVAL; }
+    if (o == OPT_WG_FINISH && value > 1) { set_error("fpx_ctx_set_option: wg_finish is 0 or 1"); return FPX_E_INVAL; }
     c->opts[o].store(value < OPT_TABLE[o].min_set ? OPT_UNSET : value, std::memory_order_relaxed);
     return FPX_OK;
 }
diff --git a/acoustid-index_amd/csrc/fpx_internal.h b/acoustid-index_amd/csrc/fpx_internal.h
--- a/acoustid-index_amd/csrc/fpx_internal.h
+++ b/acoustid-index_amd/csrc/fpx_internal.h
@@ -283,6 +283,8 @@
     uint32_t hint_def = 0;
     uint64_t hint_misc = 0;
     uint64_t hint_P = 0, hint_H = 0;
+    bool qs_clean = false; size_t qs_clean_words = 0;
+    uint8_t* d_fin = nullptr; size_t cap_fin = 0;
     uint32_t fast_penalty = 0;
     fpx_result* d_parts = nullptr; size_t cap_parts = 0;
     uint32_t* d_parts_n = nullptr; size_t cap_parts_n = 0;
@@ -319,6 +321,7 @@
     OPT_SHARD_WG,
     OPT_SHARD_PACK,
     OPT_FILT_COOP,
+    OPT_WG_FINISH,
     OPT_COUNT
 };
 constexpr int64_t OPT_UNSET = -2;
diff --git a/acoustid-index_amd/csrc/fpx_qsearch.hpp b/acoustid-index_amd/csrc/fpx_qsearch.hpp
--- a/acoustid-index_amd/csrc/fpx_qsearch.hpp
+++ b/acoustid-index_amd/csrc/fpx_qsearch.hpp
@@ -71,7 +71,16 @@
     union { uint32_t redo_cap; uint32_t bin_rec32; uint32_t dead_union_last; };
 };
 
+struct QSFinishArgs {
+    fpx_result* fin_res; uint32_t* fin_n; uint32_t fin_stride;
+    uint32_t pub_nwords;
+    unsigned int* pub_ticket; unsigned long long* pub_counters; unsigned int* pub_words; unsigned int* pub_words_host;
+    const uint4* pub_res; uint4* pub_res_host; uint32_t pub_res_n16;
+};
 struct QSKernargs { QSearchArgs a; GroupArgs ga; };
+struct QSKernargsFin { QSearchArgs a; GroupArgs ga; QSFinishArgs fa; };
+static_assert(sizeof(GroupArgs) % 8 == 0 && offsetof(QSKernargsFin, fa) == sizeof(QSearchArgs) + sizeof(GroupArgs) && offsetof(QSKernargsFin, ga) == offsetof(QSKernargs, ga),
+              "the third parameter lies right behind the second");
 static_assert(sizeof(QSearchArgs) == 160 && offsetof(QSearchArgs, cands) == 40 && offsetof(QSearchArgs, qcand_n) == 64 && offsetof(QSearchArgs, next_q) == 128 &&
               offsetof(QSearchArgs, redo) == 144 && offsetof(QSearchArgs, redo_cap) == 152, "QSearchArgs' layout is the kernels' argument segment: a member is renamed or shared, never moved");
 typedef const __attribute__((address_space(4))) QSKernargs* qs_kargs_t;
@@ -81,6 +90,8 @@
     asm volatile("" : "+s"(p));
     return p;
 }
+typedef const __attribute__((address_space(4))) QSFinishArgs* qs_fargs_t;
+__device__ __forceinline__ qs_fargs_t qs_fin_args() { return &((const __attribute__((address_space(4))) QSKernargsFin*)qs_cold_args())->fa; }
 
 #define FPX_QS_OCC __attribute__((amdgpu_waves_per_eu(FPX_QS_WAVES)))
 #define FPX_LDS __attribute__((address_space(3)))
@@ -196,6 +207,7 @@
     __shared__ const uint32_t* s_ext[GROUP_CHUNKS];
     __shared__ uint32_t s_q2;
     __shared__ uint32_t s_dseg[FUSE_MAX];
+    constexpr bool WGF = !CLS && !NEXT && !SHARE;
 
     const uint32_t tid = threadIdx.x, lane = tid & 63u;
     const GroupDesc* g = &ga.g;
@@ -288,7 +300,7 @@
         s_cancel = c_dev != 0ull ? 1u : 0u;
     }
     __syncthreads();
-    if (s_cancel) return;
+    if (s_cancel) { if constexpr (WGF) break; else return; }
     QS_MARK(0);
     uint32_t vmask = 0u;
     uint32_t mmask = 0u;
@@ -1381,6 +1393,42 @@
             if (gi < kh->a.cand_cap) kh->a.cands[gi] = key;
         }
     }
+    if constexpr (WGF) {
+        const qs_fargs_t kfin = qs_fin_args();
+        if (kfin->fin_n != nullptr && !shared) {
+          if (tid == 0u) {
+            uint32_t qv = q, cv = cn;
+            asm volatile("" : "+v"(qv), "+v"(cv));
+            uint64_t k[QCAND_SLOTS];
+#pragma unroll
+            for (uint32_t i = 0; i < QCAND_SLOTS; ++i) { const uint64_t e = cbuf[i]; k[i] = i < cv ? e : ~0ull; }
+#pragma unroll
+            for (uint32_t i = 0; i + 1 < QCAND_SLOTS; ++i)
+#pragma unroll
+                for (uint32_t j = 0; j + 1 < QCAND_SLOTS - i; ++j) {
+                    const uint64_t lo = k[j + 1] < k[j] ? k[j + 1] : k[j], hi = k[j + 1] < k[j] ? k[j] : k[j + 1];
+                    k[j] = lo; k[j + 1] = hi;
+                }
+            const uint4 ov = *reinterpret_cast<const uint4*>(kh->a.opts + (size_t)qv * 4u);
+            uint32_t width = kfin->fin_stride, fsb = kh->a.sb;
+            asm volatile("" : "+v"(width), "+v"(fsb));
+            const uint64_t fmax = fsb >= 32u ? 0xFFFFFFFFull : ((1ull << fsb) - 1ull);
+            fpx_result* const row = kfin->fin_res + (size_t)qv * width;
+            uint32_t min_score = ov.y, nres = 0u;
+            bool alive = true;
+#pragma unroll
+            for (uint32_t i = 0; i < QCAND_SLOTS; ++i) {
+                const uint32_t score = (uint32_t)(fmax - ((k[i] >> 32) & fmax));
+                alive = alive && i < cv && i != ov.x && score >= min_score;
+                if (i == 0u) min_score = alive ? max(min_score, rel_floor(score, ov.z)) : min_score;
+                if (alive && i < width) { row[i].id = (uint32_t)k[i]; row[i].score = score; }
+                nres += alive ? 1u : 0u;
+            }
+            kfin->fin_n[qv] = min(nres, width);
+            if (cv != 0u) atomicAdd(&kh->a.counters[CTR_SLOTCANDS], (unsigned long long)cv);
+          }
+        }
+    }
     }
     QS_MARK(5);
     if constexpr (CLS) {
@@ -1404,10 +1452,45 @@
     }
     __syncthreads();
   }
+    if constexpr (WGF) {
+        const qs_kargs_t kf = qs_cold_args();
+        const qs_fargs_t kfin = qs_fin_args();
+        unsigned int* const ticket = kfin->pub_ticket;
+        if (ticket != nullptr) {
+            __threadfence();
+            __syncthreads();
+            if (tid == 0u) s_cbase_lo = atomicAdd(ticket, 1u);
+            __syncthreads();
+            if (s_cbase_lo == gridDim.x - 1u) {
+                __threadfence();
+                unsigned long long* const ctr = kf->a.counters; unsigned long long* const ctr_host = kfin->pub_counters;
+                for (uint32_t i = tid; i < (uint32_t)CTR_COUNT; i += QS_WG) {
+                    ctr_host[i] = __hip_atomic_load(&ctr[i], __ATOMIC_RELAXED, __HIP_MEMORY_SCOPE_AGENT);
+                    __hip_atomic_store(&ctr[i], 0ull, __ATOMIC_RELAXED, __HIP_MEMORY_SCOPE_AGENT);
+                }
+                unsigned int* const words = kfin->pub_words; unsigned int* const words_host = kfin->pub_words_host;
+                const uint32_t nwords = kfin->pub_nwords;
+                for (uint32_t i = tid; i < nwords; i += QS_WG) {
+                    words_host[i] = __hip_atomic_load(&words[i], __ATOMIC_RELAXED, __HIP_MEMORY_SCOPE_AGENT);
+                    __hip_atomic_store(&words[i], 0u, __ATOMIC_RELAXED, __HIP_MEMORY_SCOPE_AGENT);
+                }
+                const uint4* const res = kfin->pub_res; uint4* const res_host = kfin->pub_res_host;
+                const uint32_t n16 = kfin->pub_res_n16;
+                for (uint32_t i = tid; i < n16; i += QS_WG * 8u) {
+                    uint4 v[8];
+#pragma unroll
+                    for (uint32_t u = 0; u < 8u; ++u) v[u] = i + u * QS_WG < n16 ? res[i + u * QS_WG] : make_uint4(0u, 0u, 0u, 0u);
+#pragma unroll
+                    for (uint32_t u = 0; u < 8u; ++u) if (i + u * QS_WG < n16) res_host[i + u * QS_WG] = v[u];
+                }
+                if (tid == 0u) __hip_atomic_store(ticket, 0u, __ATOMIC_RELAXED, __HIP_MEMORY_SCOPE_AGENT);
+            }
+        }
+    }
 }
 
 template <int NS, bool QS, bool MEM, bool FILT>
-__global__ __launch_bounds__(QS_WG) FPX_QS_OCC void k_search_query(QSearchArgs a, GroupArgs ga)
+__global__ __launch_bounds__(QS_WG) FPX_QS_OCC void k_search_query(QSearchArgs a, GroupArgs ga, QSFinishArgs)
 {
     qs_body<qs_variant<NS, QS, MEM, FILT>>(a, ga);
 }
@@ -1417,17 +1500,17 @@
     qs_body<qs_variant<NS, true, MEM, false, QS_F_CLS>>(a, ga);
 }
 template <int NS, bool QS, bool MEM>
-__global__ __launch_bounds__(QS_WG) FPX_QS_OCC void k_search_low(QSearchArgs a, GroupArgs ga)
+__global__ __launch_bounds__(QS_WG) FPX_QS_OCC void k_search_low(QSearchArgs a, GroupArgs ga, QSFinishArgs)
 {
     qs_body<qs_variant<NS, QS, MEM, false, QS_F_LOW>>(a, ga);
 }
 template <int NS, bool QS, bool MEM>
-__global__ __launch_bounds__(QS_WG) FPX_QS_OCC void k_search_low_filt(QSearchArgs a, GroupArgs ga)
+__global__ __launch_bounds__(QS_WG) FPX_QS_OCC void k_search_low_filt(QSearchArgs a, GroupArgs ga, QSFinishArgs)
 {
     qs_body<qs_variant<NS, QS, MEM, true, QS_F_LOW>>(a, ga);
 }
 template <int NS, bool QS, bool MEM>
-__global__ __launch_bounds__(QS_WG) FPX_QS_OCC void k_search_filt(QSearchArgs a, GroupArgs ga)
+__global__ __launch_bounds__(QS_WG) FPX_QS_OCC void k_search_filt(QSearchArgs a, GroupArgs ga, QSFinishArgs)
 {
     qs_body<qs_variant<NS, QS, MEM, true, QS_F_COOP>>(a, ga);
 }
@@ -1452,10 +1535,11 @@
     qs_body<qs_variant<NS, false, MEM, FILT, QS_F_SHARE | QS_F_PACK>>(a, ga);
 }
 
-__global__ __launch_bounds__(256) void k_qs_zero(unsigned long long* counters, unsigned int* words, uint32_t nwords)
+__global__ __launch_bounds__(256) void k_qs_zero(unsigned long long* counters, unsigned int* words, uint32_t nwords, unsigned int* ticket = nullptr)
 {
     const uint32_t i0 = blockIdx.x * 256u + threadIdx.x;
     if (i0 < CTR_COUNT) counters[i0] = 0ull;
+    if (i0 == 0u && ticket != nullptr) *ticket = 0u;
     for (uint32_t i = i0; i < nwords; i += gridDim.x * 256u) words[i] = 0u;
 }
 
diff --git a/acoustid-index_amd/csrc/fpx_search.hip b/acoustid-index_amd/csrc/fpx_search.hip
--- a/acoustid-index_amd/csrc/fpx_search.hip
+++ b/acoustid-index_amd/csrc/fpx_search.hip
@@ -144,6 +144,8 @@
 #define FPX_LAUNCH(K, grid, wg, lds, st, a0, a1, ns8, ...) \
     with_ns(ns8, [&](auto ns, auto... cs) { hipLaunchKernelGGL((K<decltype(ns)::value, decltype(cs)::value...>), grid, dim3(wg), lds, st, a0, a1); }, __VA_ARGS__)
 #define FPX_LAUNCH_QS(K, grid, st, qa, g, ns8, ...) FPX_LAUNCH(K, grid, QS_WG, QS_LDS_BYTES, st, qa, g, ns8, __VA_ARGS__)
+#define FPX_LAUNCH_QS_FIN(K, grid, st, qa, g, fa, ns8, ...) \
+    with_ns(ns8, [&](auto ns, auto... cs) { hipLaunchKernelGGL((K<decltype(ns)::value, decltype(cs)::value...>), grid, dim3(QS_WG), QS_LDS_BYTES, st, qa, g, fa); }, __VA_ARGS__)
 
 static void launch_probe_group(bool packed, bool ns8, bool binned, bool qs, dim3 grid, hipStream_t st, const ProbeArgs& a, const GroupArgs& g)
 {
@@ -377,6 +379,7 @@
     bool want_q; uint64_t* q_blocks; uint64_t* q_docs;
     size_t def_cap, def_stat_off, def_words;
     uint32_t up_chunks, up_q[Workspace::UP_CHUNKS + 1];
+    bool ws_clean;
 };
 
 struct StatSums { unsigned long long reads = 0, blocks = 0, docs = 0, probes = 0, dreads = 0, bytes_off = 0, pads = 0, records = 0; };
@@ -566,6 +569,7 @@
             if (ws->d_def_count) (void)hipFree(ws->d_def_count);
             if (ws->h_def_count) (void)hipHostFree(ws->h_def_count);
             ws->d_def_count = nullptr; ws->h_def_count = nullptr; ws->cap_def_segs = 0;
+            b.ws_clean = false;
             const size_t nseg = std::max(1u, snap->n_lean);
             const size_t words = nseg * DEF_COUNT_STRIDE + LEAN_STAT_WORDS;
             FPX_HIP(dmalloc(&ws->d_def_count, words * sizeof(unsigned int)));
@@ -645,12 +649,13 @@
     return (!*filt || words_wg == 2) && queries_fit_wg(offsets, opts, B);
 }
 
+static unsigned int* wg_ticket(const Workspace* ws) { return reinterpret_cast<unsigned int*>(ws->d_counters + CTR_COUNT + 1); }
 template <class Args>
-static int open_wg_path(Batch& b, size_t extra_words, CandSlots* cs, Args* a)
+static int open_wg_path(Batch& b, size_t extra_words, CandSlots* cs, Args* a, bool clean = false)
 {
     Workspace* ws = b.ws; int rc;
     if ((rc = ensure_cand_slots(ws, b.B, extra_words, cs))) return rc;
-    hipLaunchKernelGGL(k_qs_zero, dim3(8), dim3(256), 0, b.st, ws->d_counters, ws->d_def_count, (uint32_t)b.def_words);
+    if (!clean) hipLaunchKernelGGL(k_qs_zero, dim3(8), dim3(256), 0, b.st, ws->d_counters, ws->d_def_count, (uint32_t)b.def_words, wg_ticket(ws));
     FPX_HIP(hipEventRecord(ws->ev_probe0, b.st));
     a->hashes_base = b.d_hashes_base; a->offsets = b.d_offsets; a->opts = b.d_opts; a->sb = 32u - b.qb;
     a->cands = ws->d_cands[0]; a->cand_cap = ws->cap_cands; a->qcand = cs->qcand; a->qcand_n = cs->qcand_n;
@@ -670,10 +675,10 @@
     FPX_SYNC_BATCH(b);
     return handed_back(ws, b.snap) ? FPX_REDO_QS : FPX_OK;
 }
-static int finish_wg_path(Batch& b, const ResultsTo& to, uint64_t Cf, uint32_t path_bits)
+static int finish_wg_path(Batch& b, const ResultsTo& to, uint64_t Cf, uint32_t path_bits, bool delivered = false)
 {
     Workspace* ws = b.ws; int rc;
-    if (!b.partial && (rc = deliver_results(ws, b.B, b.out_cap, to.staged, b.out, b.out_n, b.st))) return rc;
+    if (!b.partial && !delivered && (rc = deliver_results(ws, b.B, b.out_cap, to.staged, b.out, b.out_n, b.st))) return rc;
     const unsigned long long* ls = host_stat_sets(b);
     const StatSums s = sum_stat_sets(ls);
     gather_hist(ws->batch_hist, ws->h_counters, ls, s.probes);
@@ -694,6 +699,44 @@
     ws->hint_misc = 0; ws->hint_def = 0;
     return FPX_OK;
 }
+struct WgFinish {
+    bool on = false; uint32_t width = 0;
+    int aim(Batch& b, QSFinishArgs* fa)
+    {
+        Workspace* ws = b.ws; int rc;
+        fa->pub_counters = mapped_address(ws->h_counters); fa->pub_words = ws->d_def_count; fa->pub_words_host = mapped_address(ws->h_def_count);
+        fa->pub_nwords = (uint32_t)b.def_words;
+        if (!fa->pub_counters || !fa->pub_words_host) return FPX_OK;
+        width = std::min<uint32_t>(b.out_cap, QCAND_SLOTS);
+        const size_t bytes = (((size_t)b.B * sizeof(uint32_t) + (size_t)b.B * width * sizeof(fpx_result)) + 15u) & ~(size_t)15u;
+        if ((rc = ensure_h_out(ws, bytes))) return rc;
+        if ((rc = grow(&ws->d_fin, &ws->cap_fin, bytes))) return rc;
+        uint8_t* h = mapped_address(ws->h_out);
+        if (!h) return FPX_OK;
+        fa->fin_n = reinterpret_cast<uint32_t*>(ws->d_fin); fa->fin_res = reinterpret_cast<fpx_result*>(ws->d_fin + (size_t)b.B * sizeof(uint32_t)); fa->fin_stride = width;
+        fa->pub_res = reinterpret_cast<const uint4*>(ws->d_fin); fa->pub_res_host = reinterpret_cast<uint4*>(h); fa->pub_res_n16 = (uint32_t)(bytes / 16u);
+        on = true;
+        return FPX_OK;
+    }
+    void deliver(Batch& b) const
+    {
+        const Workspace* ws = b.ws;
+        const uint32_t* n = reinterpret_cast<const uint32_t*>(ws->h_out);
+        const fpx_result* rows = reinterpret_cast<const fpx_result*>(ws->h_out + (size_t)b.B * sizeof(uint32_t));
+        std::memcpy(b.out_n, n, (size_t)b.B * sizeof(uint32_t));
+        for (uint32_t q = 0; q < b.B; ++q)
+            for (uint32_t i = 0, c = std::min(n[q], width); i < c; ++i) b.out[(size_t)q * b.out_cap + i] = rows[(size_t)q * width + i];
+    }
+};
+static int close_wg_finish(Batch& b)
+{
+    Workspace* ws = b.ws;
+    FPX_HIP(hipGetLastError());
+    FPX_HIP(hipEventRecord(ws->ev_probe1, b.st));
+    FPX_HIP(hipEventRecord(ws->ev_end, b.st));
+    FPX_SYNC_BATCH(b);
+    return handed_back(ws, b.snap) ? FPX_REDO_QS : FPX_OK;
+}
 static int redo_hot_queries(Batch& b, QSearchArgs qa, const GroupArgs& gargs, bool ns8, int cus, uint64_t R)
 {
     if (R > qs_redo_limit(b.B) || R > qa.redo_cap) {
@@ -726,7 +769,14 @@
     }
     CandSlots cs;
     QSearchArgs qa{};
-    if ((rc = open_wg_path(b, hot_wg ? (size_t)B : 0, &cs, &qa))) return rc;
+    QSFinishArgs fa{};
+    ResultsTo to;
+    WgFinish wf;
+    if (!b.partial && ngroups == 1u && !hot_wg && ctx_opt(snap->ctx, OPT_WG_FINISH) == 1) {
+        if ((rc = results_target(b, &to))) return rc;
+        if ((rc = wf.aim(b, &fa))) return rc;
+    }
+    if ((rc = open_wg_path(b, hot_wg ? (size_t)B : 0, &cs, &qa, wf.on && b.ws_clean && ws->qs_clean_words == b.def_words))) return rc;
     struct Running {
         std::atomic<int>* c; int before;
         explicit Running(std::atomic<int>* c_) : c(c_), before(c_->fetch_add(1)) {}
@@ -746,17 +796,20 @@
     const int cus = device_cus(snap->ctx);
     const uint32_t up_chunks = b.up_chunks;
     uint32_t next_launches = 0;
+    uint32_t last_c = 0;
+    for (uint32_t c = 0; c < up_chunks; ++c) if (b.up_q[c + 1] != b.up_q[c]) last_c = c;
     for (uint32_t c = 0; c < std::max(1u, up_chunks); ++c) {
         qa.q_begin = up_chunks ? b.up_q[c] : 0u; qa.q_end = up_chunks ? b.up_q[c + 1] : B;
+        fa.pub_ticket = wf.on && c == last_c ? wg_ticket(ws) : nullptr;
         if (qa.q_end == qa.q_begin) { if (up_chunks && c + 1u < up_chunks && (rc = upload_piece(b, c + 1u))) return rc; continue; }
         qa.next_q = (FPX_QS_DYN && alone) ? ws->d_def_count + c : nullptr;
         qa.stagger = alone ? QS_STAGGER : 0u;
         if (up_chunks) FPX_HIP(hipStreamWaitEvent(st, ws->ev_chunk[c], 0));
         const dim3 grid(std::min<uint32_t>(qa.q_end - qa.q_begin, (uint32_t)cus * QS_WGS_PER_CU));
-        if (low && filt0) FPX_LAUNCH_QS(k_search_low_filt, grid, st, qa, gargs, ns8, b.want_q, mem);
-        else if (low) FPX_LAUNCH_QS(k_search_low, grid, st, qa, gargs, ns8, b.want_q, mem);
-        else if (coop) FPX_LAUNCH_QS(k_search_filt, grid, st, qa, gargs, ns8, b.want_q, mem);
-        else FPX_LAUNCH_QS(k_search_query, grid, st, qa, gargs, ns8, b.want_q, mem, filt0);
+        if (low && filt0) FPX_LAUNCH_QS_FIN(k_search_low_filt, grid, st, qa, gargs, fa, ns8, b.want_q, mem);
+        else if (low) FPX_LAUNCH_QS_FIN(k_search_low, grid, st, qa, gargs, fa, ns8, b.want_q, mem);
+        else if (coop) FPX_LAUNCH_QS_FIN(k_search_filt, grid, st, qa, gargs, fa, ns8, b.want_q, mem);
+        else FPX_LAUNCH_QS_FIN(k_search_query, grid, st, qa, gargs, fa, ns8, b.want_q, mem, filt0);
         if (ngroups > 1u) {
             QSearchArgs qn = qa;
             qn.mem_tab = nullptr; qn.mem_bucket = nullptr; qn.mem_bits = nullptr;
@@ -771,8 +824,7 @@
         }
         if (up_chunks && c + 1u < up_chunks && (rc = upload_piece(b, c + 1u))) return rc;
     }
-    ResultsTo to;
-    if ((rc = close_wg_pass(b, qa.sb, cs, &to)) != FPX_OK && rc != FPX_REDO_QS) return rc;
+    if ((rc = wf.on ? close_wg_finish(b) : close_wg_pass(b, qa.sb, cs, &to)) != FPX_OK && rc != FPX_REDO_QS) return rc;
 #ifdef FPX_QS_PROF
     fprintf(stderr, "qs_prof clocks/query: setup %.0f dedup %.0f rounds %.0f tasks %.0f count+exact %.0f handover %.0f", ws->h_counters[CTR_HIST] / (double)B, ws->h_counters[CTR_HIST + 1] / (double)B,
             ws->h_counters[CTR_HIST + 2] / (double)B, ws->h_counters[CTR_HIST + 3] / (double)B, ws->h_counters[CTR_HIST + 4] / (double)B, ws->h_counters[CTR_HIST + 5] / (double)B);
@@ -788,8 +840,12 @@
         Cf = ws->h_counters[CTR_CANDS];
         if ((rc = finish_crowded(b, qa.sb, cs, to, Cf))) return rc;
     }
-    if ((rc = finish_wg_path(b, to, Cf, 4u | 64u | (filt ? 256u : 0u) | (R != 0 ? 1024u : 0u) | (low ? 4096u : 0u) | (ngroups > 1u ? 8192u : 0u) | (coop ? 65536u : 0u)))) return rc;
+    const bool finished = wf.on && Cf == 0;
+    if (finished) wf.deliver(b);
+    if ((rc = finish_wg_path(b, to, Cf, 4u | 64u | (filt ? 256u : 0u) | (R != 0 ? 1024u : 0u) | (low ? 4096u : 0u) | (ngroups > 1u ? 8192u : 0u) | (coop ? 65536u : 0u) |
+                                        (finished ? 131072u : 0u), finished))) return rc;
     if (b.stats) b.stats->probe_launches += next_launches;
+    if (finished) { ws->qs_clean = true; ws->qs_clean_words = b.def_words; }
     return FPX_OK;
 }
 
@@ -1430,6 +1486,7 @@
     std::memset(ws->batch_hist, 0, sizeof ws->batch_hist);
     __atomic_store_n(ws->h_cancel, 0u, __ATOMIC_RELEASE);
     b.cancel = timeout_ms ? ws->d_cancel : nullptr;
+    b.ws_clean = ws->qs_clean; ws->qs_clean = false;
     b.base = offsets[0]; b.P = offsets[B] - b.base; b.qb = bits_for(B);
     b.partial = partial; b.out = out; b.out_cap = out_cap; b.out_n = out_n; b.stats = stats; b.q_blocks = q_blocks; b.q_docs = q_docs;
     const uint64_t P = b.P;
@@ -1693,6 +1750,7 @@
     FPX_HIP(hipSetDevice(ctx->device));
     Workspace* ws = ws_acquire(ctx);
     if (!ws) return FPX_E_NOMEM;
+    ws->qs_clean = false;
     int rc = FPX_OK;
     auto body = [&]() -> int {
         int r;
@@ -1890,6 +1948,7 @@
     FPX_HIP(hipSetDevice(snap->ctx->device));
     Workspace* ws = ws_acquire(snap->ctx);
     if (!ws) return FPX_E_NOMEM;
+    ws->qs_clean = false;
     auto body = [&]() -> int {
         int rc;
         hipStream_t st = ws->stream;
@@ -2085,6 +2144,7 @@
     }
     Workspace* ws = ws_acquire(ctx);
     if (!ws) return FPX_E_NOMEM;
+    ws->qs_clean = false;
     auto body = [&]() -> int {
         int rc;
         hipStream_t st = ws->stream;
@@ -2135,6 +2195,7 @@
     FPX_HIP(hipSetDevice(snap->ctx->device));
     Workspace* ws = ws_acquire(snap->ctx);
     if (!ws) return FPX_E_NOMEM;
+    ws->qs_clean = false;
     auto body = [&]() -> int {
         int rc;
         hipStream_t st = ws->stream;
@@ -2269,6 +2330,7 @@
     FPX_HIP(hipSetDevice(ctx->device));
     Workspace* ws = ws_acquire(ctx);
     if (!ws) return FPX_E_NOMEM;
+    ws->qs_clean = false;
     auto body = [&]() -> int {
         int rc;
         hipStream_t st = ws->stream;
```

New measurement: 17.76 million. -37.9%, worse.
